# Fastaxx/Penguin.jl

Hardware: AMD Instinct MI355X
Metric: time-steps/sec + SpMV GB/s (% HBM roofline), 3D mono diffusion 512^3 (higher is better)
Workload: dtype f64

## Files before the change

include/penguin_hip.h:

```cpp
#ifndef PENGUIN_HIP_H
#define PENGUIN_HIP_H

#include <stddef.h>
#include <stdint.h>

#ifdef __cplusplus
extern "C" {
#endif

typedef struct pg_mesh pg_mesh;
typedef struct pg_capacity pg_capacity;
typedef struct pg_diffops pg_diffops;
typedef struct pg_solver pg_solver;
typedef struct pg_streamvort pg_streamvort;

enum { PG_BODY_BALL = 1, PG_BODY_MULTIBALL = 2, PG_BODY_HALFSPACE = 3, PG_BODY_ELLIPSOID = 4, PG_BODY_PLANE = 5 };
enum { PG_FLAG_COMPLEMENT = 1, PG_FLAG_NO_CENTROIDS = 2 };
enum { PG_CAP_V = 0, PG_CAP_GAMMA = 1, PG_CAP_CELL_TYPES = 2, PG_CAP_A = 3, PG_CAP_B = 4,
       PG_CAP_W = 5, PG_CAP_C_OMEGA = 6, PG_CAP_C_GAMMA = 7,
       PG_CAP_ST_V0 = 8, PG_CAP_ST_V1 = 9, PG_CAP_ST_CT_OMEGA = 10, PG_CAP_ST_CT_GAMMA = 11 };
enum { PG_OP_G = 0, PG_OP_H = 1, PG_OP_WINV = 2,
       PG_OP_C0 = 3 , PG_OP_K0 = 6  };
enum { PG_BC_NONE = 0, PG_BC_DIRICHLET = 1, PG_BC_NEUMANN = 2, PG_BC_ROBIN = 3, PG_BC_PERIODIC = 4 };
enum { PG_KEY_LEFT = 0 , PG_KEY_RIGHT = 1 , PG_KEY_BOTTOM = 2 ,
// ... 38 lines not shown
enum { PG_PRECOND_MG_CELL = -3 };
enum { PG_PRECOND_POLY_EST = -4 };
#define PG_SPECEST_MARGIN 0.0205

typedef struct {
  int32_t steps;
  int32_t admitted;
  int32_t gershgorin_admits;
  int32_t reserved;
  double g_ritz;
  double g_used;
  double margin;
  double gershgorin;
  double ritz_re_min, ritz_re_max, ritz_im_max;
  double estimate_ms;
} pg_specest_info;

#define PG_MG_MAX_LEVELS 16
typedef struct {
  int32_t levels;
  int32_t tail_level;
  int64_t rows[PG_MG_MAX_LEVELS];
  int64_t nnz[PG_MG_MAX_LEVELS];
  double setup_ms;
  int64_t bytes;
} pg_mg_info;

typedef struct {
  int32_t iters;
  int32_t converged;
  double resnorm;
  double bnorm;
  double extremum;
  double time;
} pg_step_info;

typedef struct {
  int64_t steps;
  int64_t total_iters;
  double t_final;
  double extremum;
  double solve_ms;
  double spmv_ms_total;
  int64_t spmv_launches;
  int64_t unconverged_steps;
  double worst_relres;
  double spmv_lean_ms_total;
  int64_t spmv_lean_launches;
  int64_t poly_degree;
  int64_t half_exits;
  int64_t poly_xspace;
  int64_t products;
  int64_t guess_states_read;
} pg_run_info;

typedef struct {
  int64_t n_own;
  int64_t nnz;
  int64_t n_ghost;
  int64_t n_omega;
  int64_t n_gamma;
  int64_t M_global;
  int64_t spmv_bytes;
  int64_t spmv_slices;
  int64_t rows_uniform;
  int64_t rows_pattern;
  int64_t rows_irregular;
  int64_t neumann_ok;
  double gershgorin;
  int64_t spmv_units;
  int64_t rows_marched;
  int64_t rows_matrix;
  int64_t n_ghost_loop;
  int64_t loop_is_compact;
  int64_t rows_edge;
} pg_system_info;

typedef struct {
  int64_t steps;
  int64_t psi_iters;
  int64_t omega_iters;
  int64_t psi_products;
  int64_t omega_products;
  int64_t unconverged;
  double worst_relres;
  double t_final;
  double total_ms;
  double psi_ms;
  double velocity_ms;
  double build_ms;
  double omega_ms;
} pg_streamvort_run_info;

int32_t pg_last_error(char* buf, size_t n);
int32_t pg_init(int32_t device_id);
int32_t pg_get_unique_id(void* out128);
int32_t pg_init_distributed(int32_t device_id, int32_t rank, int32_t nranks, const void* unique_id128);
int32_t pg_finalize(void);
int32_t pg_device_synchronize(void);
int32_t pg_set_profiling(int32_t on);
int32_t pg_device_name(char* buf, size_t n);
int32_t pg_config_string(char* buf, size_t n);

int32_t pg_mesh_create(int32_t N, const int64_t* n, const double* L, const double* x0, pg_mesh** out);
int32_t pg_mesh_destroy(pg_mesh* m);
int32_t pg_mesh_get_centers(const pg_mesh* m, int32_t d, double* out, int64_t len);
// ... 76 lines not shown

int32_t pg_streamvort_create(pg_capacity* c, pg_diffops* o, const double* nu, double dt, const pg_bc_desc* bc_stream,
                             const pg_bc_desc* bc_vorticity, const pg_border_desc* borders_stream, int32_t nborders_stream,
                             const pg_border_desc* borders_vorticity, int32_t nborders_vorticity, const double* psi0,
                             const double* omega0, pg_streamvort** out);
int32_t pg_streamvort_destroy(pg_streamvort* sv);
int32_t pg_streamvort_set_omega(pg_streamvort* sv, const double* omega);
int32_t pg_streamvort_set_source(pg_streamvort* sv, const double* f_n , const double* f_np1 );
int32_t pg_streamvort_set_interface_values(pg_streamvort* sv, int32_t which, const double* g_n , const double* g_np1 );
int32_t pg_streamvort_set_border_values(pg_streamvort* sv, int32_t which, const double* values );
int32_t pg_streamvort_solve_stream(pg_streamvort* sv, const pg_krylov_opts* opts, pg_step_info* info);
int32_t pg_streamvort_step(pg_streamvort* sv, int32_t scheme, const pg_krylov_opts* opts, pg_step_info* info_psi,
                           pg_step_info* info_omega);
int32_t pg_streamvort_run(pg_streamvort* sv, int64_t steps, int32_t scheme, const pg_krylov_opts* opts, int32_t save_every,
                          pg_streamvort_run_info* info);
int32_t pg_streamvort_get(const pg_streamvort* sv, int32_t field, int64_t state_index, double* out, int64_t len);
int32_t pg_streamvort_num_states(const pg_streamvort* sv, int64_t* out);
int32_t pg_streamvort_time(const pg_streamvort* sv, int64_t state_index, double* out);
int32_t pg_streamvort_solver(pg_streamvort* sv, int32_t which, pg_solver** borrowed);

int32_t pg_solver_set_source(pg_solver* s, int32_t phase, const double* f_n , const double* f_np1 );
int32_t pg_solver_set_interface_value(pg_solver* s, const double* g_n , const double* g_np1 );
int32_t pg_solver_set_border_values(pg_solver* s, const double* values );

int32_t pg_solver_initial_solve(pg_solver* s, const pg_krylov_opts* opts, pg_step_info* info);
int32_t pg_solver_step(pg_solver* s, int32_t scheme, const pg_krylov_opts* opts, pg_step_info* info);
int32_t pg_solver_run(pg_solver* s, double Tend, int32_t scheme, const pg_krylov_opts* opts, int32_t do_initial,
                      int64_t max_steps, int32_t save_every, pg_run_info* info);
int32_t pg_solver_num_states(const pg_solver* s, int64_t* out);
int32_t pg_solver_get_state(const pg_solver* s, int64_t state_index, double* x, int64_t len);
int32_t pg_solver_system_info(const pg_solver* s, int32_t which, pg_system_info* out);
int32_t pg_solver_get_system_csr(const pg_solver* s, int32_t which, int64_t* rowptr, int64_t* col, double* val,
                                 double* b, int64_t* idx);
int32_t pg_solver_get_row_scaling(const pg_solver* s, int32_t which, double* ds);
int32_t pg_solver_mg_info(const pg_solver* s, pg_mg_info* out);
int32_t pg_solver_mg_info_for(const pg_solver* s, int32_t precond, pg_mg_info* out);
int32_t pg_solver_spectral_estimate(pg_solver* s, int32_t which, pg_specest_info* out);
int32_t pg_solver_time_spmv(pg_solver* s, int32_t which, int32_t reps, double* avg_ms);

int32_t pg_partition_planes(const int64_t* weight, int64_t nplanes, int32_t nranks, int64_t* bounds);
int32_t pg_slab_numbering_host(int32_t K, int64_t plane, int64_t nplanes, int64_t p0, int64_t p1, const uint8_t* active,
                               int64_t* out);

int32_t pg_debug_spmv_compare(pg_solver* s, int32_t which, int32_t variant_a, int32_t variant_b, double* max_abs_diff,
                              double* max_abs);
int32_t pg_debug_spmv_mode_compare(pg_solver* s, int32_t which, int32_t mode, double* max_abs_diff, double* max_abs,
                                   double* max_dot_rel);
int32_t pg_debug_spmv_sizes(pg_solver* s, int32_t which, int64_t* n, int64_t* n_vec, int64_t* nnz, int32_t* grid);
#define PG_DEBUG_SPMV_SENTINEL 0x7FF8C0DE5EED0BADull
int32_t pg_debug_spmv_apply(pg_solver* s, int32_t which, int32_t variant, int32_t mode, const double* x, const double* aux,
                            const double* dotx, const double* base, double pc0, double pc1, double pc2, int32_t fold,
                            int32_t done, int32_t repeat, double* y, double* partials, double* slot_sums, double* folded,
                            int64_t* ticket);
int32_t pg_debug_read_probe(int64_t bytes, int32_t elem_bytes, int32_t nt, int32_t blocks, int32_t reps, double* gbs);
int32_t pg_debug_run_virtual_ranks(int32_t nranks, int32_t N, const int64_t* n, const double* L, int32_t body_kind,
                                   const double* params, int32_t nparams, double interface_value, double border_value,
                                   int32_t nkeys, const int32_t* keys, double dt, int32_t scheme_ctor, int32_t scheme_run,
                                   int64_t steps, double* x_out, int64_t* n_own_out, int64_t* nnz_out,
                                   int64_t* n_ghost_out, int64_t* iters_out);
int32_t pg_debug_set_virtual_rank_method(int32_t method, int32_t restart);
int32_t pg_debug_set_virtual_rank_precond(int32_t precond);
int32_t pg_debug_set_virtual_rank_ramp(double ramp);
int32_t pg_debug_set_virtual_rank_kick(int64_t step, double factor);
int32_t pg_debug_virtual_rank_info(int32_t rank, int64_t* full_rows, int64_t* loop_rows, int64_t* loop_bytes,
                                   int64_t* loop_ghosts);
int32_t pg_debug_scale_diagonal_rows(pg_solver* s, double factor);
int32_t pg_debug_set_poly_give_up(int32_t iterations);

int32_t pg_debug_mg_aggregates(pg_solver* s, int32_t level, int64_t* n, int32_t* agg);
int32_t pg_debug_mg_level_csr(pg_solver* s, int32_t level, int64_t* n, int64_t* nnz, int64_t* rowptr, int64_t* col, double* val);
int32_t pg_debug_mg_apply(pg_solver* s, const double* r, double* z);
int32_t pg_debug_mg_aggregates_for(pg_solver* s, int32_t precond, int32_t level, int64_t* n, int32_t* agg);
int32_t pg_debug_mg_level_csr_for(pg_solver* s, int32_t precond, int32_t level, int64_t* n, int64_t* nnz, int64_t* rowptr, int64_t* col,
                                  double* val);
int32_t pg_debug_mg_apply_for(pg_solver* s, int32_t precond, const double* r, double* z);

int32_t pg_debug_specest_hessenberg(pg_solver* s, int32_t which, int32_t* steps, double* H);

int32_t pg_solver_guess_info(pg_solver* s, int32_t* kept, int32_t* nstates, int32_t* offsets , double* coef ,
                             double* rr_plain, double* rr_taken);

#ifdef __cplusplus
}
#endif
#endif
```

penguin/jl_amd/_lib.py:

```python
from __future__ import annotations

import ctypes as C
import os
import re
from pathlib import Path

import numpy as np

_HERE = Path(__file__).resolve().parent
LIB_PATH = Path(os.environ["PG_LIB_PATH"]) if os.environ.get("PG_LIB_PATH") else _HERE / "lib" / "libpenguin_hip.so"
HEADER_PATH = _HERE.parent.parent / "include" / "penguin_hip.h"


class PenguinHipError(RuntimeError):
    pass


PG_BODY_BALL, PG_BODY_MULTIBALL, PG_BODY_HALFSPACE, PG_BODY_ELLIPSOID, PG_BODY_PLANE = 1, 2, 3, 4, 5
PG_FLAG_COMPLEMENT, PG_FLAG_NO_CENTROIDS = 1, 2
PG_CAP_V, PG_CAP_GAMMA, PG_CAP_CELL_TYPES, PG_CAP_A, PG_CAP_B, PG_CAP_W, PG_CAP_C_OMEGA, PG_CAP_C_GAMMA = range(8)
PG_CAP_ST_V0, PG_CAP_ST_V1, PG_CAP_ST_CT_OMEGA, PG_CAP_ST_CT_GAMMA = 8, 9, 10, 11
PG_OP_G, PG_OP_H, PG_OP_WINV = 0, 1, 2
PG_OP_C0, PG_OP_K0 = 3, 6
PG_BC_NONE, PG_BC_DIRICHLET, PG_BC_NEUMANN, PG_BC_ROBIN, PG_BC_PERIODIC = 0, 1, 2, 3, 4
PG_KEY = {"left": 0, "right": 1, "bottom": 2, "top": 3, "backward": 4, "forward": 5}
PG_SCHEME = {"BE": 0, "CN": 1, "STEADY": 2}
PG_METHOD = {"bicgstab": 0, "cg": 1, "gmres": 2, "bicgstabl": 3}
PG_SV_PSI, PG_SV_OMEGA, PG_SV_U, PG_SV_V = 0, 1, 2, 3
PG_PRECOND_MG = -2
PG_PRECOND_MG_CELL = -3
PG_PRECOND_POLY_EST = -4
PG_SPECEST_MARGIN = 0.0205
PG_MG_MAX_LEVELS = 16

c_double_p = C.POINTER(C.c_double)
c_i64_p = C.POINTER(C.c_int64)
c_i32_p = C.POINTER(C.c_int32)


class pg_bc_desc(C.Structure):
    _fields_ = [("kind", C.c_int32), ("alpha", C.c_double), ("beta", C.c_double), ("value", C.c_double),
                ("value_array", c_double_p)]


class pg_border_desc(C.Structure):
    _fields_ = [("key", C.c_int32), ("kind", C.c_int32), ("value", C.c_double)]


class pg_jump_desc(C.Structure):
    _fields_ = [("alpha1", C.c_double), ("alpha2", C.c_double), ("g", C.c_double), ("beta1", C.c_double),
                ("beta2", C.c_double), ("h", C.c_double), ("g_array", c_double_p), ("h_array", c_double_p)]


class pg_motion_desc(C.Structure):
    _fields_ = [("body_kind", C.c_int32), ("flags", C.c_int32), ("axis", C.c_int32), ("nq", C.c_int32), ("sign", C.c_double),
                ("t0", C.c_double), ("t1", C.c_double), ("nodes", c_double_p), ("body0", C.c_double * 4),
                ("body1", C.c_double * 4)]


class pg_krylov_opts(C.Structure):
    _fields_ = [("method", C.c_int32), ("reltol", C.c_double), ("abstol", C.c_double), ("maxiter", C.c_int32),
                ("check_every", C.c_int32), ("warm_start", C.c_int32), ("restart", C.c_int32), ("precond", C.c_int32)]


class pg_step_info(C.Structure):
    _fields_ = [("iters", C.c_int32), ("converged", C.c_int32), ("resnorm", C.c_double), ("bnorm", C.c_double),
                ("extremum", C.c_double), ("time", C.c_double)]


class pg_run_info(C.Structure):
    _fields_ = [("steps", C.c_int64), ("total_iters", C.c_int64), ("t_final", C.c_double), ("extremum", C.c_double),
                ("solve_ms", C.c_double), ("spmv_ms_total", C.c_double), ("spmv_launches", C.c_int64),
                ("unconverged_steps", C.c_int64), ("worst_relres", C.c_double), ("spmv_lean_ms_total", C.c_double),
                ("spmv_lean_launches", C.c_int64), ("poly_degree", C.c_int64), ("half_exits", C.c_int64),
                ("poly_xspace", C.c_int64), ("products", C.c_int64), ("guess_states_read", C.c_int64)]


class pg_system_info(C.Structure):
    _fields_ = [("n_own", C.c_int64), ("nnz", C.c_int64), ("n_ghost", C.c_int64), ("n_omega", C.c_int64),
                ("n_gamma", C.c_int64), ("M_global", C.c_int64), ("spmv_bytes", C.c_int64), ("spmv_slices", C.c_int64),
                ("rows_uniform", C.c_int64), ("rows_pattern", C.c_int64), ("rows_irregular", C.c_int64),
                ("neumann_ok", C.c_int64), ("gershgorin", C.c_double), ("spmv_units", C.c_int64),
                ("rows_marched", C.c_int64), ("rows_matrix", C.c_int64), ("n_ghost_loop", C.c_int64),
                ("loop_is_compact", C.c_int64), ("rows_edge", C.c_int64)]


class pg_streamvort_run_info(C.Structure):
    _fields_ = [("steps", C.c_int64), ("psi_iters", C.c_int64), ("omega_iters", C.c_int64), ("psi_products", C.c_int64),
                ("omega_products", C.c_int64), ("unconverged", C.c_int64), ("worst_relres", C.c_double), ("t_final", C.c_double),
                ("total_ms", C.c_double), ("psi_ms", C.c_double), ("velocity_ms", C.c_double), ("build_ms", C.c_double),
                ("omega_ms", C.c_double)]


class pg_mg_info(C.Structure):
    _fields_ = [("levels", C.c_int32), ("tail_level", C.c_int32), ("rows", C.c_int64 * PG_MG_MAX_LEVELS),
                ("nnz", C.c_int64 * PG_MG_MAX_LEVELS), ("setup_ms", C.c_double), ("bytes", C.c_int64)]


class pg_specest_info(C.Structure):
    _fields_ = [("steps", C.c_int32), ("admitted", C.c_int32), ("gershgorin_admits", C.c_int32), ("reserved", C.c_int32),
                ("g_ritz", C.c_double), ("g_used", C.c_double), ("margin", C.c_double), ("gershgorin", C.c_double),
                ("ritz_re_min", C.c_double), ("ritz_re_max", C.c_double), ("ritz_im_max", C.c_double), ("estimate_ms", C.c_double)]


def declared_symbols() -> list[str]:
    txt = HEADER_PATH.read_text()
    return sorted(set(re.findall(r"\bint32_t\s+(pg_[a-z0-9_]+)\s*\(", txt)))


_lib = None
hip_runtime_source = "system"


def _share_the_hip_runtime_with_torch() -> None:
    global hip_runtime_source
    import sys

    if "torch" in sys.modules:
        hip_runtime_source = "already mapped by torch"
        return
    if os.environ.get("PG_HIP_RUNTIME", "auto") == "system":
        return
    import importlib.util

    try:
        spec = importlib.util.find_spec("torch")
    except (ImportError, ValueError):
        spec = None
# ... 123 lines not shown
    return {k: getattr(info, k) for k, _ in pg_specest_info._fields_ if k != "reserved"}


def debug_specest_hessenberg(handle, which: int = 0, run: bool = True) -> np.ndarray:
    w = C.c_int32(which | (0 if run else 4))
    k = C.c_int32(0)
    check(lib().pg_debug_specest_hessenberg(handle, w, C.byref(k), None))
    H = np.zeros((k.value + 1) * max(k.value, 1))
    check(lib().pg_debug_specest_hessenberg(handle, w, C.byref(k), dptr(H)))
    return H[: (k.value + 1) * k.value].reshape((k.value + 1, k.value), order="F")


DEBUG_SPMV_SENTINEL = 0x7FF8C0DE5EED0BAD
DEBUG_SPMV_GUARD = 64


def debug_spmv_sizes(handle, which: int) -> tuple[int, int, int, int]:
    n, nv, nnz, grid = C.c_int64(0), C.c_int64(0), C.c_int64(0), C.c_int32(0)
    check(lib().pg_debug_spmv_sizes(handle, C.c_int32(which), C.byref(n), C.byref(nv), C.byref(nnz), C.byref(grid)))
    return n.value, nv.value, nnz.value, grid.value


def loop_system_csr(handle, which: int):
    n, _, nnz, _ = debug_spmv_sizes(handle, which)
    rowptr, col, val = np.zeros(n + 1, dtype=np.int64), np.zeros(max(nnz, 1), dtype=np.int64), np.zeros(max(nnz, 1))
    check(lib().pg_solver_get_system_csr(handle, C.c_int32(which), iptr(rowptr), iptr(col), dptr(val), None, None))
    return rowptr, col[:nnz], val[:nnz]


def debug_spmv_apply(handle, which: int, variant: int, mode: int, x, aux=None, dotx=None, base=None, pc=(0.0, 0.0, 0.0),
                     fold: int = 0, done: int = 0, repeat: int = 1) -> dict:
    n, nv, _, grid = debug_spmv_sizes(handle, which)

    def arr(a, length, name):
        if a is None:
            return None, None
        a = np.ascontiguousarray(a, dtype=np.float64)
        if a.size != length:
            raise ValueError(f"debug_spmv_apply: {name} has {a.size} entries, the matrix needs {length}")
        return a, dptr(a)

    xs, xp = arr(x, nv, "x")
    auxs, auxp = arr(aux, n, "aux")
    dots, dotp = arr(dotx, n, "dotx")
    bases, basep = arr(base, n, "base")
    y = np.zeros(n + DEBUG_SPMV_GUARD)
    partials = np.zeros((5, grid))
    sums, folded = np.zeros(5), np.zeros(5)
    ticket = C.c_int64(-1)
    check(lib().pg_debug_spmv_apply(handle, C.c_int32(which), C.c_int32(variant), C.c_int32(mode), xp, auxp, dotp, basep,
                                    C.c_double(pc[0]), C.c_double(pc[1]), C.c_double(pc[2]), C.c_int32(fold), C.c_int32(done),
                                    C.c_int32(repeat), dptr(y), dptr(partials), dptr(sums), dptr(folded), C.byref(ticket)))
    return {"y": y, "partials": partials, "slot_sums": sums, "folded": folded, "ticket": ticket.value, "grid": grid, "n": n}
```

penguin/jl_amd/csrc/pg_common.h:

```cpp
#pragma once
#include <hip/hip_runtime.h>
#include "pg_rccl.h"

#include <chrono>
#include <cstdint>
#include <cstdio>
#include <cstring>
#include <stdexcept>
#include <string>
#include <vector>

#include "../../../include/penguin_hip.h"

namespace pg {

using i64 = int64_t;
using i32 = int32_t;

struct Error : std::runtime_error {
  using std::runtime_error::runtime_error;
};

void set_last_error(const std::string& msg);

#define PG_HIP(expr)                                                                              \
  do {                                                                                            \
    hipError_t _e = (expr);                                                                       \
    if (_e != hipSuccess)                                                                         \
      throw pg::Error(std::string("HIP error: ") + hipGetErrorString(_e) + " at " + __FILE__ + ":" + \
                      std::to_string(__LINE__) + " (" #expr ")");                                 \
  } while (0)

#define PG_NCCL(expr)                                                                             \
  do {                                                                                            \
    ncclResult_t _e = (expr);                                                                     \
    if (_e != ncclSuccess)                                                                        \
      throw pg::Error(std::string("RCCL error: ") + pg::rccl::api().GetErrorString(_e) + " at " + __FILE__ + ":" + \
                      std::to_string(__LINE__) + " (" #expr ")");                                 \
  } while (0)

#define PG_REQUIRE(cond, msg)                                   \
  do {                                                          \
    if (!(cond)) throw pg::Error(std::string(msg));             \
  } while (0)

#define PG_API_BEGIN try {
#define PG_API_END                                  \
  return 0;                                         \
  }                                                 \
  catch (const std::exception& e) {                 \
    pg::set_last_error(e.what());                   \
    return 1;                                       \
  }                                                 \
  catch (...) {                                     \
    pg::set_last_error("unknown exception");        \
    return 2;                                       \
  }

struct Config {
  bool debug = false;
  int alloc_poison = 0;
  int async_alloc = 0;
  int alloc_guard = 0;
  long long pool_limit_mb = 0;
  bool poly = true;
  int poly_degree = 6;
  bool poly_adapt = true;
  double poly_margin = 1.0;
  double poly_slack = -1.0;
  int poly_hist = 3;
  bool poly_trend = true;
  int poly_maxdeg = 0;
  int poly_mindeg = 4;
  int profile_sample = 3;
  bool gamma_elim = true;
  bool diag_elim = true;
  double diag_elim_frac = 0.0005;
  int spmv_variant = 70;
  int spmv_xcd = 1;
  int spmv_strip = 16;
  int spmv_march_k = 0;
  int spmv_minrun = 24;
  bool spmv_march = true;
  bool spmv_edges = true;
  int spmv_tile_units = 0;
  int spmv_blocks_per_cu = 0;
  bool halo_overlap = true;
  int guess_n = 4;
  int guess_depth = 7;
  bool guess_defer = true;
  bool guess_always = false;
  int guess_monitor = 256;
  double guess_pass_cost = 0.34;
  double guess_gain = 0.8;
  bool speculate_product = true;
  int mg_tail_rows = 2048;
  int unit_order = 0;
};
const Config& config();

struct LocalComm;

struct Context {
  bool inited = false;
  LocalComm* local = nullptr;
  int device = 0;
  hipStream_t stream = nullptr;
  hipStream_t comm_stream = nullptr;
  hipEvent_t ev_fork = nullptr, ev_join = nullptr;
  int rank = 0, nranks = 1;
  ncclComm_t comm = nullptr;
  ncclComm_t comm_halo = nullptr;
  bool profiling = false;
  std::string device_name;
};
Context& ctx();
void require_init();
void set_thread_context(Context* c);
Context* thread_context();
LocalComm* local_comm_create(int nranks);
void local_comm_destroy(LocalComm* c);
void comm_allreduce_sum_f64(double* dev, int count, hipStream_t st);
void comm_allreduce_max_f64(double* dev, int count, hipStream_t st);
void comm_allreduce_sum_u64(unsigned long long* dev, i64 count, hipStream_t st);

void* dev_alloc(size_t bytes);
// ... 150 lines not shown
```

penguin/jl_amd/csrc/pg_context.hip:

```cpp
#include "pg_common.h"

#include <cxxabi.h>
#include <execinfo.h>

#include <atomic>
#include <map>
#include <mutex>
#include <unordered_map>
#include <unordered_set>
#include "pg_host_algos.h"

#include <algorithm>
#include <array>
#include <memory>
#include <set>

namespace pg {

static thread_local std::string g_last_error;
void set_last_error(const std::string& msg) { g_last_error = msg; }

Context& ctx() {
  static Context c;
  Context* t = thread_context();
  return t ? *t : c;
}

const Config& config() {
  static const Config c = [] {
    Config k;
    auto geti = [](const char* name, long long dflt) { const char* v = getenv(name); return v ? atoll(v) : dflt; };
    auto getd = [](const char* name, double dflt) { const char* v = getenv(name); return v ? atof(v) : dflt; };
    k.debug = getenv("PG_DEBUG") != nullptr;
    k.alloc_poison = (int)geti("PG_ALLOC_POISON", 0);
    k.async_alloc = (int)geti("PG_ASYNC_ALLOC", 0);
    k.alloc_guard = (int)geti("PG_ALLOC_GUARD", 0);
    k.pool_limit_mb = geti("PG_POOL_LIMIT_MB", 0);
    k.poly = geti("PG_POLY", 1) != 0;
    k.poly_degree = (int)geti("PG_POLY_DEGREE", 6);
    k.poly_adapt = geti("PG_POLY_ADAPT", getenv("PG_POLY_DEGREE") ? 0 : 1) != 0;
    k.poly_margin = getd("PG_POLY_MARGIN", 1.0);
    k.poly_slack = getd("PG_POLY_SLACK", -1.0);
    k.poly_hist = (int)std::max<long long>(1, std::min<long long>(3, geti("PG_POLY_HIST", 3)));
    k.poly_maxdeg = (int)geti("PG_POLY_MAXDEG", 0);
    k.poly_mindeg = (int)std::max<long long>(2, std::min<long long>(8, geti("PG_POLY_MINDEG", 4)));
    k.poly_trend = geti("PG_POLY_TREND", 1) != 0;
    k.profile_sample = (int)std::max<long long>(1, geti("PG_PROFILE_SAMPLE", 3));
    k.gamma_elim = geti("PG_GAMMA_ELIM", 1) != 0;
    k.diag_elim = geti("PG_DIAG_ELIM", 1) != 0;
    k.diag_elim_frac = getd("PG_DIAG_ELIM_FRAC", 0.0005);
    k.spmv_variant = (int)geti("PG_SPMV_VARIANT", 70);
    k.spmv_xcd = (int)geti("PG_SPMV_XCD", 1);
    k.spmv_strip = (int)geti("PG_SPMV_STRIP", 16);
    k.spmv_march_k = (int)geti("PG_SPMV_MARCH_K", 0);
    k.spmv_minrun = (int)geti("PG_SPMV_MINRUN", 24);
    k.spmv_march = geti("PG_SPMV_MARCH", 1) != 0;
    k.spmv_edges = geti("PG_SPMV_EDGES", 1) != 0;
    k.spmv_tile_units = (int)geti("PG_SPMV_TILE_UNITS", 0);
    k.spmv_blocks_per_cu = (int)geti("PG_SPMV_BLOCKS_PER_CU", 0);
    k.halo_overlap = geti("PG_HALO_OVERLAP", 1) != 0;
    k.speculate_product = geti("PG_SPECULATE", 1) != 0;
    k.guess_n = (int)std::max<long long>(0, std::min<long long>(4, geti("PG_GUESS_STATES", 4)));
    k.guess_depth = (int)std::max<long long>(1, std::min<long long>(7, geti("PG_GUESS_DEPTH", 7)));
    k.mg_tail_rows = (int)std::max<long long>(0, geti("PG_MG_TAIL_ROWS", 2048));
    k.guess_monitor = (int)std::max<long long>(1, geti("PG_GUESS_MONITOR", 256));
    k.guess_pass_cost = getd("PG_GUESS_PASS_COST", 0.34);
    k.guess_always = geti("PG_GUESS_ALWAYS", 0) != 0;
    k.guess_defer = geti("PG_GUESS_DEFER", 1) != 0;
    k.guess_gain = getd("PG_GUESS_GAIN", 0.8);
    k.unit_order = (int)geti("PG_SPMV_UNIT_ORDER", 0);
    return k;
  }();
  return c;
}

void require_init() {
  if (!ctx().inited)
    throw Error("penguin_hip: not initialised (call pg_init / pg_init_distributed first)");
}

static void init_device(int device_id) {
  Context& c = ctx();
  int ndev = 0;
  hipError_t e = hipGetDeviceCount(&ndev);
  if (e != hipSuccess || ndev <= 0)
    throw Error("penguin_hip: no HIP device visible -- this library has no CPU fallback");
  PG_REQUIRE(device_id >= 0 && device_id < ndev, "penguin_hip: device id out of range");
  PG_HIP(hipSetDevice(device_id));
  hipDeviceProp_t prop;
  PG_HIP(hipGetDeviceProperties(&prop, device_id));
  c.device = device_id;
  c.device_name = std::string(prop.name) + " (" + prop.gcnArchName + ")";
  if (!c.stream) PG_HIP(hipStreamCreateWithFlags(&c.stream, hipStreamNonBlocking));
  if (!c.comm_stream) PG_HIP(hipStreamCreateWithFlags(&c.comm_stream, hipStreamNonBlocking));
  c.inited = true;
}

}

// ... 215 lines not shown
      split_ok = R.CommSplit(c.comm, 0, rank, &c.comm_halo, nullptr) == ncclSuccess && c.comm_halo != nullptr;
      if (!split_ok) c.comm_halo = nullptr;
    }
    if (!split_ok) {
      ncclUniqueId id2;
      if (rank == 0) PG_NCCL(R.GetUniqueId(&id2));
      DevBuf<char> buf((i64)sizeof(id2));
      if (rank == 0) buf.upload(reinterpret_cast<const char*>(&id2), (i64)sizeof(id2));
      PG_NCCL(R.Broadcast(buf.p, buf.p, sizeof(id2), ncclChar, 0, c.comm, c.stream));
      buf.download(reinterpret_cast<char*>(&id2), (i64)sizeof(id2));
      PG_NCCL(R.CommInitRank(&c.comm_halo, nranks, id2, rank));
    }
  }
  PG_API_END
}

int32_t pg_finalize(void) {
  PG_API_BEGIN
  Context& c = ctx();
  if (c.inited) {
    (void)hipDeviceSynchronize();
    if (c.comm_halo) { (void)rccl::api().CommDestroy(c.comm_halo); c.comm_halo = nullptr; }
    if (c.comm) { (void)rccl::api().CommDestroy(c.comm); c.comm = nullptr; }
    dev_cache_release();
    if (c.stream) { (void)hipStreamDestroy(c.stream); c.stream = nullptr; }
    if (c.comm_stream) { (void)hipStreamDestroy(c.comm_stream); c.comm_stream = nullptr; }
    if (c.ev_fork) { (void)hipEventDestroy(c.ev_fork); c.ev_fork = nullptr; }
    if (c.ev_join) { (void)hipEventDestroy(c.ev_join); c.ev_join = nullptr; }
    c.inited = false;
  }
  PG_API_END
}

int32_t pg_device_synchronize(void) {
  PG_API_BEGIN
  require_init();
  PG_HIP(hipDeviceSynchronize());
  PG_API_END
}

int32_t pg_set_profiling(int32_t on) {
  PG_API_BEGIN
  ctx().profiling = on != 0;
  PG_API_END
}

int32_t pg_config_string(char* buf, size_t n) {
  PG_API_BEGIN
  const Config& k = config();
  char tmp[1024];
  snprintf(tmp, sizeof(tmp),
           "spmv_variant=%d spmv_xcd=%d spmv_strip=%d spmv_unit_order=%d spmv_march=%d spmv_edges=%d spmv_march_k=%d spmv_minrun=%d spmv_tile_units=%d "
           "spmv_blocks_per_cu=%d halo_overlap=%d speculate=%d poly=%d poly_degree=%d poly_adapt=%d "
           "poly_margin=%g poly_slack=%g poly_hist=%d poly_trend=%d poly_maxdeg=%d gamma_elim=%d diag_elim=%d "
           "guess_states=%d guess_depth=%d guess_defer=%d async_alloc=%d cache_limit_mb=%lld alloc_poison=%d alloc_guard=%d profile_sample=%d debug=%d",
           k.spmv_variant, k.spmv_xcd, k.spmv_strip, k.unit_order, (int)k.spmv_march, (int)k.spmv_edges, k.spmv_march_k, k.spmv_minrun, k.spmv_tile_units,
           k.spmv_blocks_per_cu, (int)k.halo_overlap, (int)k.speculate_product, (int)k.poly, k.poly_degree, (int)k.poly_adapt,
           k.poly_margin, k.poly_slack, k.poly_hist, (int)k.poly_trend, k.poly_maxdeg,
           (int)k.gamma_elim, (int)k.diag_elim, k.guess_n, k.guess_depth, (int)k.guess_defer, k.async_alloc, k.pool_limit_mb, k.alloc_poison, k.alloc_guard, k.profile_sample, (int)k.debug);
  if (buf && n > 0) {
    std::strncpy(buf, tmp, n - 1);
    buf[n - 1] = 0;
  }
  PG_API_END
}

int32_t pg_device_name(char* buf, size_t n) {
  PG_API_BEGIN
  require_init();
  if (buf && n > 0) {
    std::strncpy(buf, ctx().device_name.c_str(), n - 1);
    buf[n - 1] = 0;
  }
  PG_API_END
}

int32_t pg_mesh_create(int32_t N, const int64_t* n, const double* L, const double* x0, pg_mesh** out) {
  PG_API_BEGIN
  PG_REQUIRE(N >= 1 && N <= 3, "pg_mesh_create: N must be 1, 2 or 3");
  PG_REQUIRE(out != nullptr, "pg_mesh_create: out is NULL");
  PG_REQUIRE(n != nullptr && L != nullptr, "pg_mesh_create: n / L is NULL");
  std::unique_ptr<pg_mesh> guard(new pg_mesh());
  pg_mesh* m = guard.get();
  m->N = N;
  for (int d = 0; d < N; ++d) {
    PG_REQUIRE(n[d] >= 1, "pg_mesh_create: n_d must be >= 1");
    m->n[d] = n[d];
    m->L[d] = L[d];
    m->x0[d] = x0 ? x0[d] : 0.0;
    const double h = L[d] / static_cast<double>(n[d]);
    m->centers[d].resize(n[d]);
    m->nodes[d].resize(n[d] + 1);
    for (i64 j = 0; j < n[d]; ++j) m->centers[d][j] = m->x0[d] + static_cast<double>(j) * h;
    for (i64 j = 0; j <= n[d]; ++j) m->nodes[d][j] = m->x0[d] + (static_cast<double>(j) + 0.5) * h;
  }
  if (ctx().inited) {
    for (int d = 0; d < N; ++d) {
      m->d_nodes[d].alloc(n[d] + 1);
      m->d_nodes[d].upload(m->nodes[d].data(), n[d] + 1);
    }
  }
  *out = guard.release();
  PG_API_END
}

int32_t pg_mesh_destroy(pg_mesh* m) {
  PG_API_BEGIN
  delete m;
  PG_API_END
}

// ... 133 lines not shown
```

penguin/jl_amd/csrc/pg_host_algos.h:

```cpp
#pragma once
#include <algorithm>
#include <cmath>
#include <cstdint>
#include <vector>

namespace pghost {

inline void partition_planes(const int64_t* weight, int64_t nplanes, int nranks, int64_t* bounds) {
  std::vector<double> cum(nplanes + 1, 0.0);
  for (int64_t k = 0; k < nplanes; ++k) cum[k + 1] = cum[k] + static_cast<double>(weight[k]) + 1.0;
  const double total = cum[nplanes];
  bounds[0] = 0;
  for (int r = 1; r < nranks; ++r) {
    const double target = total * r / nranks;
    int64_t k = std::lower_bound(cum.begin(), cum.end(), target) - cum.begin();
    if (k > 0 && (target - cum[k - 1]) < (cum[k] - target)) --k;
    const int64_t lo = bounds[r - 1] + 1;
    const int64_t hi = nplanes - (nranks - r);
    bounds[r] = std::min(std::max(k, lo), hi);
  }
  bounds[nranks] = nplanes;
}

constexpr int SLAB_MAX_KINDS = 4;
// ... 498 lines not shown

PGHOST_HD inline int bicgstabl_small_solve(const double* G, int l, double* gamma) {
  for (int i = 0; i <= BL_MAX_L; ++i) gamma[i] = 0.0;
  if (l < 1 || l > BL_MAX_L) return 0;
  double M[BL_MAX_L][BL_MAX_L], c[BL_MAX_L], d0[BL_MAX_L], y[BL_MAX_L];
  int perm[BL_MAX_L];
  for (int k = l; k >= 1; --k) {
    for (int i = 0; i < k; ++i) {
      for (int j = 0; j < k; ++j) M[i][j] = G[(i + 1) * BL_LD + (j + 1)];
      c[i] = G[(i + 1) * BL_LD];
      d0[i] = M[i][i];
      perm[i] = i;
    }
    bool ok = true;
    for (int s = 0; s < k && ok; ++s) {
      int p = s;
      for (int q = s + 1; q < k; ++q)
        if (M[q][q] > M[p][p]) p = q;
      if (p != s) {
        for (int j = 0; j < k; ++j) { const double t = M[s][j]; M[s][j] = M[p][j]; M[p][j] = t; }
        for (int i = 0; i < k; ++i) { const double t = M[i][s]; M[i][s] = M[i][p]; M[i][p] = t; }
        { const double t = c[s]; c[s] = c[p]; c[p] = t; }
        { const double t = d0[s]; d0[s] = d0[p]; d0[p] = t; }
        { const int t = perm[s]; perm[s] = perm[p]; perm[p] = t; }
      }
      const double piv = M[s][s];
      if (!(piv > BL_PIV_TOL * d0[s]) || !bl_finite(piv)) { ok = false; break; }
      const double root = sqrt(piv);
      M[s][s] = root;
      c[s] = c[s] / root;
      for (int q = s + 1; q < k; ++q) M[q][s] = M[q][s] / root;
      for (int q = s + 1; q < k; ++q) {
        for (int t = s + 1; t <= q; ++t) {
          M[q][t] -= M[q][s] * M[t][s];
          M[t][q] = M[q][t];
        }
        c[q] -= M[q][s] * c[s];
      }
    }
    if (!ok) continue;
    for (int s = k - 1; s >= 0; --s) {
      double v = c[s];
      for (int q = s + 1; q < k; ++q) v -= M[q][s] * y[q];
      y[s] = v / M[s][s];
      if (!bl_finite(y[s])) ok = false;
    }
    if (!ok) continue;
    for (int s = 0; s < k; ++s) gamma[1 + perm[s]] = y[s];
    return k;
  }
  return 0;
}

}
```

penguin/jl_amd/csrc/pg_krylov.h:

```cpp
#pragma once
#include <functional>

#include "pg_system.h"

namespace pg {

struct MgHierarchy;

struct XGuess {
  const double* zbase = nullptr;
  const double* zr[8] = {nullptr, nullptr, nullptr, nullptr, nullptr, nullptr, nullptr, nullptr};
  const double* coef = nullptr;
};

struct KrylovWork {
  i64 n = 0, nvec = 0;
  DevBuf<double> r, rhat, p, v, t;
  DevBuf<double> partials;
  DevBuf<double> sc;
  double* h_sc = nullptr;
  int grid = 1;
  DevBuf<unsigned> ticket;
  double last_rate2 = 0.0;
  int last_iters = 0;
  const void* adapt_matrix = nullptr;
  int adapt_m = 0, adapt_h = 0;
  const void* need_matrix = nullptr;
  double need_hist[3] = {0.0, 0.0, 0.0};
  const void* fail_matrix = nullptr;
  int fail_deg = 0, good_deg = 0;
  double fail_L = 0.0;
  int fail_wait = 0, fail_backoff = 1;
  const int* scatter = nullptr;
  MgHierarchy* mg = nullptr;
  XGuess xguess;
  bool p_in_rhat = false;
  bool start_folded = false;
  const int* moved_flag = nullptr;
  int moved_stamp = 0;
  DevBuf<double> ya, yb, wa, wb;
  DevBuf<double> gm_basis, gm, gm_partials;
  int gm_m = -1;
  DevBuf<double> bl_vecs, bl, bl_partials;
  int bl_l = -1;
  i64 bl_stride = 0;
  std::function<void()> after_first_batch;
  hipEvent_t ev_poll = nullptr;
  void init(i64 n_own, i64 n_vec);
  ~KrylovWork();
};

struct SolveStats {
  int iters = 0;
  int converged = 0;
  double resnorm = 0.0, bnorm = 0.0;
  double spmv_ms = 0.0, spmv_lean_ms = 0.0;
  i64 spmv_launches = 0, spmv_lean_launches = 0;
  int poly_degree = 0;
  int half_exit = 0;
  int poly_xspace = 0;
  i64 products = 0;
  int polls = 0;
};

void halo_exchange(const Numbering& nb, const Slab& slab, double* vec, hipStream_t st);
void halo_begin(const Numbering& nb, const Slab& slab, double* vec, hipStream_t st);
void halo_end(hipStream_t st);
void spmv(const CsrMatrix& A, const double* x, double* y, hipStream_t st);
void spmv_halo(const CsrMatrix& A, const Numbering& nb, const Slab& slab, double* x, double* y, hipStream_t st);
void krylov_solve(const CsrMatrix& A, const Numbering& nb, const Slab& slab, const double* b, double* x,
                  KrylovWork& w, const pg_krylov_opts& opts, SolveStats& stats, const double* x0 = nullptr,
                  const double* Ax0 = nullptr, bool preinit = false);

bool krylov_uses_polynomial(const CsrMatrix& A, const pg_krylov_opts& opts);

extern int g_poly_give_up;

void gmres_solve(const CsrMatrix& A, const Numbering& nb, const Slab& slab, const double* b, double* x, KrylovWork& w,
                 const pg_krylov_opts& opts, SolveStats& stats);

void bicgstabl_solve(const CsrMatrix& A, const Numbering& nb, const Slab& slab, const double* b, double* x, KrylovWork& w,
                     const pg_krylov_opts& opts, SolveStats& stats);
const char* krylov_method_refusal(int method);

}
```

penguin/jl_amd/csrc/pg_krylov.hip:

```cpp
#include "pg_krylov.h"
#include "pg_multigrid.h"
#include "pg_spmv.h"
#include "pg_specest.h"

using namespace pg;

namespace pg { extern double g_host_wait_us; }

namespace {


__global__ __launch_bounds__(BLOCK) void k_bicg_init(i64 n, i64 nvec, const double* __restrict__ b,
                                                     const double* x0, const double* __restrict__ Ax0,
                                                     double* x, double* __restrict__ r,
                                                     double* __restrict__ rhat, double* __restrict__ p,
                                                     double* __restrict__ v, double* __restrict__ partials,
                                                     const double* __restrict__ ds) {
  __shared__ double s_red[BLOCK / 64];
  double acc = 0.0, accb = 0.0, accw = 0.0;
  for (i64 i = blockIdx.x * (i64)BLOCK + threadIdx.x; i < nvec; i += (i64)gridDim.x * BLOCK) {
    if (i < n) {
      const double bi = b[i];
      const double ri = x0 ? bi - Ax0[i] : bi;
      const double d = ds ? ds[i] : 1.0;
      x[i] = x0 ? x0[i] : 0.0;
      r[i] = ri; rhat[i] = ri; p[i] = ri; v[i] = 0.0;
      acc += ri * ri;
      accb += (d * bi) * (d * bi);
      accw += (d * ri) * (d * ri);
    } else {
      x[i] = 0.0; p[i] = 0.0;
    }
  }
  const double t = block_sum(acc, s_red);
  if (threadIdx.x == 0) partials[blockIdx.x] = t;
  const double tb = block_sum(accb, s_red);
  if (threadIdx.x == 0) partials[gridDim.x + blockIdx.x] = tb;
  const double tw = block_sum(accw, s_red);
  if (threadIdx.x == 0) partials[2 * (size_t)gridDim.x + blockIdx.x] = tw;
}

__global__ __launch_bounds__(BLOCK) void k_bicg_s(i64 n, double* __restrict__ sc, const double* __restrict__ v,
                                                  const double* __restrict__ rhat, double* __restrict__ r,
                                                  double* __restrict__ partials, const double* __restrict__ ds,
                                                  unsigned* __restrict__ ticket, int r_in_rhat) {
  __shared__ double s_red[BLOCK / 64];
  if (sc[S_DONE] != 0.0) return;
  const double alpha = sc[S_ALPHA];
  const bool rrhat = r_in_rhat != 0 && sc[S_ITERS] == 0.0;
  double a0 = 0.0, a1 = 0.0, aw = 0.0;
  for (i64 i = blockIdx.x * (i64)BLOCK + threadIdx.x; i < n; i += (i64)gridDim.x * BLOCK) {
    const double rh = rhat[i];
// ... 254 lines not shown
  if (threadIdx.x == 0) derive(phase, sc);
}

__global__ void k_derive(int phase, double* sc, int check_done) {
  if (check_done && sc[S_DONE] != 0.0) return;
  derive(phase, sc);
}

__global__ __launch_bounds__(BLOCK) void k_start_sums_moved(int grid, const double* __restrict__ partials, double* __restrict__ sc,
                                                            const int* __restrict__ flag, int stamp) {
  __shared__ double s_red[BLOCK / 64];
  for (int s = 0; s < 3; ++s) {
    double a = 0.0;
    for (int i = threadIdx.x; i < grid; i += BLOCK) a += partials[(size_t)s * grid + i];
    const double t = block_sum(a, s_red);
    if (threadIdx.x == 0) sc[S_RED0 + s] = t;
  }
  if (threadIdx.x == 0) sc[S_RED0 + 3] = __hip_atomic_load(flag, __ATOMIC_RELAXED, __HIP_MEMORY_SCOPE_AGENT) == stamp ? 1.0 : 0.0;
}

__global__ void k_derive_start_moved(double* sc) {
  derive(PH_INIT, sc);
  sc[S_MOVED] = sc[S_RED0 + 3] != 0.0 ? 1.0 : 0.0;
}

void finalize_folded(int phase, int nslots, KrylovWork& w, hipStream_t st) {
  Context& cx = ctx();
  if (cx.nranks == 1 && !cx.comm) return;
  comm_allreduce_sum_f64(w.sc.p + S_RED0, nslots, st);
  hipLaunchKernelGGL(k_derive, dim3(1), dim3(1), 0, st, phase, w.sc.p, 1);
}

void finalize(int phase, int nslots, KrylovWork& w, hipStream_t st, bool check_done, int slot0 = 0) {
  Context& cx = ctx();
  if (cx.nranks == 1 && !cx.comm) {
    hipLaunchKernelGGL(k_finalize, dim3(1), dim3(BLOCK), 0, st, phase, slot0, nslots, w.grid, w.partials.p, w.sc.p, 1,
                       check_done ? 1 : 0);
  } else {
    hipLaunchKernelGGL(k_finalize, dim3(1), dim3(BLOCK), 0, st, phase, slot0, nslots, w.grid, w.partials.p, w.sc.p, 0,
                       check_done ? 1 : 0);
    comm_allreduce_sum_f64(w.sc.p + S_RED0 + slot0, nslots, st);
    hipLaunchKernelGGL(k_derive, dim3(1), dim3(1), 0, st, phase, w.sc.p, check_done ? 1 : 0);
  }
}

struct SpmvTimer {
  bool on;
  hipEvent_t e0 = nullptr, e1 = nullptr;
  std::vector<std::pair<hipEvent_t, hipEvent_t>> pairs;
  std::vector<int> iter_of;
  std::vector<char> lean_of;
  std::vector<char> second_of;
  std::vector<int> count_of;
  int cur = 0, cur_count = 1;
  bool cur_lean = false, cur_second = false;
  bool armed = false;
  explicit SpmvTimer(bool on_) : on(on_) {}
  static std::vector<hipEvent_t>& pool() {
    static thread_local std::vector<hipEvent_t> p;
    return p;
  }
  static hipEvent_t take() {
    auto& p = pool();
    if (!p.empty()) {
      hipEvent_t e = p.back();
      p.pop_back();
      return e;
    }
    hipEvent_t e;
    PG_HIP(hipEventCreate(&e));
    return e;
  }
  void begin(hipStream_t st, int iteration, bool lean = false, bool second = false, int count = 1) {
    cur = iteration;
    cur_lean = lean;
    cur_second = second;
    cur_count = count;
    const int sample = config().profile_sample;
    static thread_local unsigned long long counter = 0;
    armed = on && (counter++ % sample == 0);
    if (!armed) return;
    e0 = take();
    e1 = take();
    PG_HIP(hipEventRecord(e0, st));
  }
  void end(hipStream_t st) {
    if (!armed) return;
    PG_HIP(hipEventRecord(e1, st));
    pairs.emplace_back(e0, e1);
    iter_of.push_back(cur);
    lean_of.push_back(cur_lean ? 1 : 0);
    second_of.push_back(cur_second ? 1 : 0);
    count_of.push_back(cur_count);
  }
  void collect(SolveStats& s, int iters_done, bool half_exit) {
    for (size_t q = 0; q < pairs.size(); ++q) {
      auto& pr = pairs[q];
      float ms = 0.f;
      (void)hipEventSynchronize(pr.second);
      const bool ran = iter_of[q] < iters_done && !(half_exit && iter_of[q] == iters_done - 1 && second_of[q]);
      if (ran && hipEventElapsedTime(&ms, pr.first, pr.second) == hipSuccess) {
        if (lean_of[q]) { s.spmv_lean_ms += ms; s.spmv_lean_launches += count_of[q]; }
        else { s.spmv_ms += ms; s.spmv_launches += 1; }
      }
      pool().push_back(pr.first);
      pool().push_back(pr.second);
    }
    pairs.clear();
    iter_of.clear();
    lean_of.clear();
    second_of.clear();
    count_of.clear();
  }
};

}

namespace pg {

double g_host_wait_us = 0.0;
int g_poly_give_up = 0;

void KrylovWork::init(i64 n_own, i64 n_vec) {
  n = n_own;
  nvec = n_vec;
  const i64 a = n_vec > 0 ? n_vec : 1;
  r.alloc(a); rhat.alloc(a); p.alloc(a); v.alloc(a); t.alloc(a);
  grid = spmv_default_grid(n_own);
  partials.alloc(5 * (i64)grid);
  sc.alloc(S_COUNT);
  sc.zero();
  ticket.alloc(1);
  ticket.zero();
  if (!h_sc) PG_HIP(hipHostMalloc(reinterpret_cast<void**>(&h_sc), sizeof(double) * S_COUNT));
}

KrylovWork::~KrylovWork() {
  if (h_sc) (void)hipHostFree(h_sc);
  if (ev_poll) (void)hipEventDestroy(ev_poll);
}

void spmv_halo(const CsrMatrix& A, const Numbering& nb, const Slab& slab, double* x, double* y, hipStream_t st) {
  spmv_with_halo(0, A, nb, slab, x, y, nullptr, nullptr, nullptr, spmv_default_grid(A.n), st);
  PG_HIP(hipGetLastError());
}

void spmv(const CsrMatrix& A, const double* x, double* y, hipStream_t st) {
  if (A.n == 0) return;
  launch_spmv(0, A, x, y, nullptr, nullptr, nullptr, spmv_default_grid(A.n), st);
  PG_HIP(hipGetLastError());
}

const char* krylov_method_refusal(int method) {
  return method == PG_METHOD_CG ? "the method is CG (BiCGStab only)"
         : method == PG_METHOD_BICGSTABL ? "the method is BiCGStab(l) (BiCGStab only)" : "the method is GMRES (BiCGStab only)";
}

bool krylov_uses_polynomial(const CsrMatrix& A, const pg_krylov_opts& opts) {
  const bool poly_env = config().poly;
  const int degree_env = config().poly_degree;
  const int precond = opts.precond == PG_PRECOND_POLY_EST ? 0 : opts.precond;
  if (!(poly_env && precond >= 0 && opts.method == PG_METHOD_BICGSTAB && A.poly_ok && spmv_supports_preconditioner_product() && A.n > 0))
    return false;
  return (precond > 0 ? precond : degree_env) >= 2;
}

constexpr int MAX_POLY_DEGREE = 40;

namespace {

void choose_next_degree(const CsrMatrix& A, const SolveStats& stats, int m, bool adaptive, KrylovWork& w) {
  const Config& cfg = config();
  const bool keep_degree = adaptive && stats.converged && stats.iters == 0 && w.adapt_m >= 2;
  w.adapt_matrix = nullptr;
  if (keep_degree) { w.adapt_matrix = &A; w.adapt_m = cfg.poly_mindeg; w.adapt_h = 1; }
  if (!(adaptive && stats.converged && stats.iters > 0)) return;
  const double rr0 = w.h_sc[S_RR0], rr = w.h_sc[S_HALF] != 0.0 ? w.h_sc[S_RED4] : w.h_sc[S_RR], tol2 = w.h_sc[S_TOL2];
  const double P = (2.0 * stats.iters - stats.half_exit) * m;
  if (!(rr0 > tol2 && rr > 0.0 && rr < rr0 && tol2 > 0.0)) return;
  w.last_rate2 = std::log(rr0 / rr) / P;
  const double margin = cfg.poly_margin;
  const double slack_env = cfg.poly_slack;
  const double slack = slack_env >= 0.0 ? slack_env : 0.3;
  const double need_now = std::min(P, P * std::log(tol2 / rr0) / std::log(rr / rr0)) * margin + slack;
  const int hist_n = cfg.poly_hist;
  if (w.need_matrix != &A) { w.need_matrix = &A; w.need_hist[0] = w.need_hist[1] = w.need_hist[2] = 0.0; }
  w.need_hist[2] = w.need_hist[1]; w.need_hist[1] = w.need_hist[0]; w.need_hist[0] = need_now;
  double need = need_now;
  double trend = 0.0;
  if (cfg.poly_trend && hist_n >= 3 && w.need_hist[2] > 0.0) trend = std::max(-0.5, std::min(0.2, 0.5 * (need_now - w.need_hist[2])));
  for (int q = 1; q < hist_n; ++q)
    if (w.need_hist[q] > 0.0) need = std::max(need, std::min(w.need_hist[q] + q * trend, need_now + 0.6));
  need += trend;
  double best = 1e300;
  for (int h = 1; h <= 16; ++h) {
    const int mm = std::max(cfg.poly_mindeg, (int)std::ceil(need / h));
    const int maxdeg = cfg.poly_maxdeg > 0 ? std::min(MAX_POLY_DEGREE, std::max(4, cfg.poly_maxdeg)) : 32;
    if (mm > maxdeg) continue;
    const double cost = h * (1.0 + 1.18 * (mm - 2) + 3.6);
    if (cost < best) { best = cost; w.adapt_m = mm; w.adapt_h = h; }
  }
  if (best < 1e300) w.adapt_matrix = &A;
  if (stats.iters == 1) {
    const double Lnow = std::log(rr0 / tol2);
    if (w.fail_matrix != &A) { w.fail_matrix = &A; w.fail_deg = 0; w.good_deg = 0; w.fail_wait = 0; w.fail_backoff = 1; }
    if (w.fail_wait > 0) --w.fail_wait;
    if (stats.half_exit) w.good_deg = m;
    else {
      w.fail_backoff = (m == w.fail_deg) ? std::min(w.fail_backoff * 2, 64) : 1;
      w.fail_deg = m; w.fail_L = Lnow;
      w.fail_wait = 2 * w.fail_backoff * (m + 3);
    }
    if (best < 1e300 && w.adapt_h == 1) {
      if (!stats.half_exit && w.good_deg > m) w.adapt_m = std::max(m + 1, std::min(w.adapt_m, w.good_deg));
      const double per_product = std::max(1.0, w.last_rate2);
      if (w.fail_deg > 0 && w.fail_wait > 0 && w.adapt_m <= w.fail_deg &&
          Lnow > w.fail_L - per_product * (w.fail_deg - w.adapt_m + 1))
        w.adapt_m = w.fail_deg + 1;
    }
  }
  if (cfg.debug) fprintf(stderr, "[pg_krylov] degree %d used %g products, needed %.1f -> next: %d applications of degree %d\n", m, P, need, w.adapt_h, w.adapt_m);
}

}

void krylov_solve(const CsrMatrix& A, const Numbering& nb, const Slab& slab, const double* b, double* x, KrylovWork& w,
                  const pg_krylov_opts& opts, SolveStats& stats, const double* x0, const double* Ax0, bool preinit) {
  Context& cx = ctx();
  hipStream_t st = cx.stream;
  const i64 n = A.n, nvec = nb.n_vec();
  PG_REQUIRE(w.n >= n && w.nvec >= nvec, "krylov workspace too small");
  PG_REQUIRE(opts.method == PG_METHOD_BICGSTAB || opts.method == PG_METHOD_CG || opts.method == PG_METHOD_GMRES ||
                 opts.method == PG_METHOD_BICGSTABL,
             "unknown Krylov method");
  const bool est_opt = opts.precond == PG_PRECOND_POLY_EST;
  if (est_opt) {
    PG_REQUIRE(opts.method == PG_METHOD_BICGSTAB,
               std::string("estimated polynomial preconditioner (precond = PG_PRECOND_POLY_EST) refused: ") +
                   krylov_method_refusal(opts.method));
    specest_require_one_rank();
    PG_REQUIRE(A.poly_ok || A.est.tried || A.poly_gave_up, "estimated polynomial preconditioner (precond = PG_PRECOND_POLY_EST): no spectral estimate "
               "has run on this matrix (specest_run before krylov_solve)");
  }
  const int precond = est_opt ? 0 : opts.precond;
  if (opts.method == PG_METHOD_GMRES) {
    PG_REQUIRE(!preinit && !x0, "GMRES starts from zero (IterativeSolvers' default)");
    gmres_solve(A, nb, slab, b, x, w, opts, stats);
    return;
  }
  if (opts.method == PG_METHOD_BICGSTABL) {
    PG_REQUIRE(!preinit && !x0, "BiCGStab(l) starts from zero (IterativeSolvers' default)");
    PG_REQUIRE(!mg_is_precond(opts.precond), std::string("multigrid preconditioner (precond = ") + mg_precond_name(mg_rule_of(opts.precond)) +
// ... 21 lines not shown
  w.xguess = XGuess();
  const bool start_folded = w.start_folded && preinit && opts.method == PG_METHOD_BICGSTAB;
  w.start_folded = false;
  const int* moved_flag = w.moved_flag;
  const int moved_stamp = w.moved_stamp;
  w.moved_flag = nullptr;
  const bool fused_start = !start_folded && preinit && opts.method == PG_METHOD_BICGSTAB && cx.nranks == 1 && !cx.comm;
  if (!fused_start && !start_folded)
    hipLaunchKernelGGL(k_sc_reset, dim3(1), dim3(S_COUNT), 0, st, w.sc.p, opts.reltol * opts.reltol, opts.abstol * opts.abstol);
  SpmvTimer timer(cx.profiling);

  const bool cg = opts.method == PG_METHOD_CG;
  const Config& cfg = config();
  const bool poly_env = cfg.poly;
  const int degree_env = cfg.poly_degree;
  int m = 0;
  const bool by_estimate = est_opt && !A.poly_ok && !A.poly_gave_up && A.est.tried && A.est.admitted;
  if (poly_env && precond >= 0 && !cg && (A.poly_ok || by_estimate) && spmv_supports_preconditioner_product() && n > 0)
    m = std::min(precond > 0 ? precond : degree_env, MAX_POLY_DEGREE);
  const bool adapt_env = cfg.poly_adapt;
  const bool adaptive = adapt_env && m >= 2 && precond == 0 && preinit;
  int expect_halves = 0;
  if (adaptive && w.adapt_matrix == &A && w.adapt_m >= 2) { m = w.adapt_m; expect_halves = w.adapt_h; }
  if (m < 2) m = 0;
  const bool poly = m > 0;
  MgHierarchy* const mgh = w.mg;
  w.mg = nullptr;
  const bool mg = mg_is_precond(opts.precond);
  if (mg) {
    PG_REQUIRE(!cg, "multigrid preconditioner refused: the method must be BiCGStab");
    PG_REQUIRE(spmv_supports_preconditioner_product(), "multigrid preconditioner refused: the x-space loop needs the slice kernel (PG_SPMV_VARIANT)");
    mg_require_one_rank(mg_rule_of(opts.precond));
    PG_REQUIRE(mgh && !w.scatter && !xg.zbase && n > 0, "multigrid preconditioner refused: this solve has no hierarchy (steady monophasic "
               "diffusion systems and the stream-function solve only)");
    PG_REQUIRE(mgh->rule == mg_rule_of(opts.precond),
               std::string("multigrid preconditioner: the hierarchy handed over was not built for precond = ") +
                   mg_precond_name(mg_rule_of(opts.precond)));
  }
  const bool pre = poly || mg;
  stats.poly_degree = m;
  stats.poly_xspace = poly ? 1 : 0;
  PG_REQUIRE(!w.scatter || (poly && preinit), "a compact system needs the polynomial path and a prepared start");
  double tau[MAX_POLY_DEGREE];
  if (poly) {
    const double g = std::min(std::max(by_estimate ? A.est.g_used : A.gersh, 0.05), 0.95);
    double lam[MAX_POLY_DEGREE];
    for (int k = 0; k < m; ++k) lam[k] = 1.0 + g * std::cos(M_PI * (2.0 * k + 1.0) / (2.0 * m));
    for (int k = 0, lo = 0, hi = m - 1; k < m; ++k) tau[k] = 1.0 / ((k & 1) ? lam[hi--] : lam[lo++]);
  }
  if (pre && w.ya.n < nvec) {
    w.ya.alloc(nvec); w.wa.alloc(nvec); w.wb.alloc(nvec); w.yb.alloc(nvec);
    w.ya.zero(); w.wa.zero(); w.wb.zero(); w.yb.zero();
  }
  const bool half_test = m >= 3 || mg;
  PG_REQUIRE(!xg.zbase || (poly && p_in_rhat && w.scatter), "an unformed extrapolated state needs the polynomial loop on a compact system");
  PG_REQUIRE(!preinit || !cg, "preinit is a BiCGStab path");
  if (!cg) {
    if (!preinit)
      hipLaunchKernelGGL(k_bicg_init, dim3(G), dim3(BLOCK), 0, st, n, nvec, b, x0, Ax0, x, w.r.p, w.rhat.p, w.p.p, w.v.p,
                       w.partials.p, (const double*)A.ds.p);
    static_assert(S_COUNT <= BLOCK, "k_start resets the scalar block with one thread per scalar");
    if (start_folded) {
    } else if (fused_start)
      hipLaunchKernelGGL(k_start, dim3(1), dim3(BLOCK), 0, st, (int)PH_INIT, 3, w.grid, (const double*)w.partials.p, w.sc.p,
                         opts.reltol * opts.reltol, opts.abstol * opts.abstol);
    else if (moved_flag && preinit && !(cx.nranks == 1 && !cx.comm)) {
      hipLaunchKernelGGL(k_start_sums_moved, dim3(1), dim3(BLOCK), 0, st, w.grid, (const double*)w.partials.p, w.sc.p, moved_flag,
                         moved_stamp);
      comm_allreduce_sum_f64(w.sc.p + S_RED0, 4, st);
      hipLaunchKernelGGL(k_derive_start_moved, dim3(1), dim3(1), 0, st, w.sc.p);
    } else
      finalize(PH_INIT, 3, w, st, false);
  } else {
    hipLaunchKernelGGL(k_cg_init, dim3(G), dim3(BLOCK), 0, st, n, nvec, b, x, w.r.p, w.p.p, w.partials.p, (const double*)A.ds.p);
    finalize(PH_CG_INIT, 2, w, st, false);
  }
  PG_HIP(hipGetLastError());

  int launched = 0, polls = 0;
  bool mid = false;
  bool done = false, poly_failed = false;
  const int poly_give_up = g_poly_give_up > 0 ? g_poly_give_up : 40 + 400 / std::max(m, 1);
  const int derive_here = (cx.nranks == 1 && !cx.comm) ? 1 : 0;
  auto apply = [&](double* in, double* out, int phase, int nslots, int itn) {
    const bool second = phase == PH_BICG_2;
    double* src = in;
    if (poly) {
      double* hat = second ? w.yb.p : w.ya.p;
      timer.begin(st, itn, true, second, m - 1);
      for (int k = m - 2; k >= 0; --k) {
        double* dst = k == 0 ? hat : ((k & 1) ? w.wb.p : w.wa.p);
        FinArgs f{nullptr, nullptr, PH_NONE, 0, 0, nullptr};
        const double lead = k == m - 2 ? tau[m - 1] : 1.0;
        f.pc0 = lead; f.pc1 = -lead * tau[k]; f.pc2 = tau[k]; f.base = in;
        spmv_with_halo(8, A, nb, slab, src, dst, nullptr, nullptr, w.sc.p, G, st, &f);
        src = dst;
      }
      timer.end(st);
    } else if (mg) {
      double* hat = second ? w.yb.p : w.ya.p;
      timer.begin(st, itn, true, second, 1);
      mg_apply(*mgh, A, nb, slab, in, hat, w.sc.p, st);
      timer.end(st);
      src = hat;
    }
    FinArgs f{w.ticket.p, w.sc.p, phase, nslots, derive_here, pre ? in : nullptr};
    timer.begin(st, itn, false, second);
    const bool folded = spmv_with_halo(phase == PH_BICG_1 ? 1 : 3, A, nb, slab, src, out, w.rhat.p, w.partials.p, w.sc.p, G, st, &f);
    timer.end(st);
    if (folded) finalize_folded(phase, nslots, w, st); else finalize(phase, nslots, w, st, true);
  };
  auto first_half = [&](int itn, bool test) {
    double* pvec = (p_in_rhat && itn == 0) ? w.rhat.p : w.p.p;
    apply(pvec, w.v.p, PH_BICG_1, 3, itn);
    unsigned* tk = (test && derive_here) ? w.ticket.p : nullptr;
    if (pre)
      hipLaunchKernelGGL(k_bicg_s_x, dim3(G), dim3(BLOCK), 0, st, n, w.sc.p, w.v.p, w.rhat.p, w.r.p, w.partials.p, (const double*)A.ds.p, tk,
                         p_in_rhat ? 1 : 0, (const double*)w.ya.p, x, w.scatter, xg, itn == 0 ? 1 : 0);
    else
      hipLaunchKernelGGL(k_bicg_s, dim3(G), dim3(BLOCK), 0, st, n, w.sc.p, w.v.p, w.rhat.p, w.r.p, w.partials.p, (const double*)A.ds.p, tk,
                         p_in_rhat ? 1 : 0);
    if (test && !tk) finalize(PH_BICG_S, 1, w, st, true, 4);
  };
  auto second_half = [&](int itn) {
    apply(w.r.p, w.t.p, PH_BICG_2, 5, itn);
    hipLaunchKernelGGL(k_bicg_xrp, dim3(G), dim3(BLOCK), 0, st, n, w.sc.p, w.t.p, w.v.p, x, w.r.p, w.p.p, w.rhat.p, w.partials.p,
                       (const double*)A.ds.p, p_in_rhat ? 1 : 0, pre ? (const double*)w.yb.p : nullptr, w.scatter);
  };
  while (!done) {
    int want = check_every;
    if (w.last_iters > 1) want = polls == 0 ? w.last_iters - 1 : (polls <= 4 ? 1 : check_every);
    if (expect_halves > 0) want = polls == 0 ? (expect_halves + 1) / 2 : (polls <= 4 ? 1 : check_every);
    const int batch = std::max(1, std::min(want, maxiter - launched));
    int halves = 2 * batch;
    if (half_test && expect_halves > 0 && polls == 0) halves = std::max(1, std::min(expect_halves, 2 * (maxiter - launched)));
    ++polls;
    if (!cg) {
      const bool predicted = half_test && expect_halves > 0 && polls == 1;
      for (int h = 0; h < halves; ++h) {
        if (!mid) {
          if (launched >= maxiter) break;
          first_half(launched, half_test && (!predicted || h + 2 >= halves));
          ++launched;
          mid = true;
        } else {
          second_half(launched - 1);
          mid = false;
        }
      }
    } else {
      for (int it = 0; it < batch; ++it) {
// ... 14 lines not shown
    struct WaitClock {
      std::chrono::steady_clock::time_point t0;
      ~WaitClock() { g_host_wait_us += std::chrono::duration<double, std::micro>(std::chrono::steady_clock::now() - t0).count(); }
    } wait_clock{t_wait0};
    if (w.after_first_batch && polls == 1) {
      if (!w.ev_poll) PG_HIP(hipEventCreateWithFlags(&w.ev_poll, hipEventDisableTiming));
      PG_HIP(hipEventRecord(w.ev_poll, st));
      std::function<void()> hook;
      hook.swap(w.after_first_batch);
      hook();
      PG_HIP(hipEventSynchronize(w.ev_poll));
    } else {
      PG_HIP(hipStreamSynchronize(st));
    }
    if (w.h_sc[S_DONE] != 0.0 || (launched >= maxiter && !mid)) done = true;
    if (!done && poly && launched >= poly_give_up) { poly_failed = true; done = true; }
  }
  if (poly_failed) {
    const_cast<CsrMatrix&>(A).poly_ok = false;
    const_cast<CsrMatrix&>(A).est.admitted = false;
    const_cast<CsrMatrix&>(A).poly_gave_up = true;
    timer.collect(stats, launched, false);
    if (w.scatter) {
      stats.iters = launched;
      stats.converged = 0;
      stats.poly_degree = -1;
      return;
    }
    if (cfg.debug) fprintf(stderr, "[pg_krylov] polynomial preconditioner (m = %d) stagnated after %d iterations: plain iteration\n", m, launched);
    spmv_with_halo(0, A, nb, slab, x, w.t.p, nullptr, nullptr, nullptr, G, st);
    SolveStats rest;
    krylov_solve(A, nb, slab, b, x, w, opts, rest, x, w.t.p, false);
    stats = rest;
    stats.iters += launched;
    return;
  }
  if (cfg.debug)
    fprintf(stderr, "[pg_krylov] done=%g iters=%g rr0=%g rr=%g tol2=%g rho=%g rho_old=%g alpha=%g omega=%g beta=%g red0=%g red1=%g\n",
            w.h_sc[S_DONE], w.h_sc[S_ITERS], w.h_sc[S_RR0], w.h_sc[S_RR], w.h_sc[S_TOL2], w.h_sc[S_RHO], w.h_sc[S_RHO_OLD], w.h_sc[S_ALPHA],
            w.h_sc[S_OMEGA], w.h_sc[S_BETA], w.h_sc[S_RED0], w.h_sc[S_RED1]);
  stats.iters = (int)w.h_sc[S_ITERS];
  stats.polls = polls;
  w.last_iters = stats.iters;
  stats.converged = w.h_sc[S_DONE] == 1.0 ? 1 : 0;
  stats.half_exit = w.h_sc[S_HALF] != 0.0 ? 1 : 0;
  stats.resnorm = std::sqrt(cg ? w.h_sc[S_RRW] : w.h_sc[S_RR]);
  stats.bnorm = std::sqrt(w.h_sc[S_BB]);
  timer.collect(stats, stats.iters, w.h_sc[S_HALF] != 0.0);
  stats.products = (i64)(2 * stats.iters - stats.half_exit) * (m >= 2 ? m : 1);
  if (!cg && stats.converged && stats.products > 0) {
    const double rr0 = w.h_sc[S_RR0], rr = w.h_sc[S_HALF] != 0.0 ? w.h_sc[S_RED4] : w.h_sc[S_RR];
    if (rr0 > 0.0 && rr > 0.0 && rr < rr0) w.last_rate2 = std::log(rr0 / rr) / (double)stats.products;
  }
  choose_next_degree(A, stats, m, adaptive, w);
}

}
```

penguin/jl_amd/csrc/pg_solver.hip:

```cpp
#include <algorithm>
#include <cmath>
#include <memory>

#include "pg_krylov.h"
#include "pg_reduce.h"
#include "pg_multigrid.h"
#include "pg_solver_internal.h"
#include "pg_spmv.h"
#include "pg_specest.h"

using namespace pg;

namespace pg { extern double g_host_wait_us; }

struct pg_solver {
  int nphase = 1;
  pg_capacity* cap[2] = {nullptr, nullptr};
  pg_diffops* ops[2] = {nullptr, nullptr};
  Slab slab;
  int K = 2;
  i64 Mloc = 0, M = 0;
  double dt = 0.0, t = 0.0;
  int scheme_ctor = PG_SCHEME_BE;
  pg_bc_desc bc_i{};
// ... 1809 lines not shown
                     dv.p, s->slab.first_cell(), s->Mloc, s->nphase, s->nb.red.p, s->nb.n_own, s->bcv.p);
  PG_HIP(hipGetLastError());
  PG_HIP(hipStreamSynchronize(ctx().stream));
  s->bconst_dirty = true;
  if (!s->initial_done) build_first_rhs(s);
  PG_API_END
}

int32_t pg_solver_initial_solve(pg_solver* s, const pg_krylov_opts* opts, pg_step_info* info) {
  PG_API_BEGIN
  require_init();
  PG_REQUIRE(s, "Solver is not initialized. Call a solver constructor first.");
  SolveStats st;
  std::unique_ptr<AsyncAllocScope> pool(s->moving ? new AsyncAllocScope() : nullptr);
  do_initial(s, opts, st);
  fill_info(s, st, info);
  PG_API_END
}

int32_t pg_solver_step(pg_solver* s, int32_t scheme, const pg_krylov_opts* opts, pg_step_info* info) {
  PG_API_BEGIN
  require_init();
  PG_REQUIRE(s, "Solver is not initialized. Call a solver constructor first.");
  PG_REQUIRE(scheme == PG_SCHEME_BE || scheme == PG_SCHEME_CN, "scheme must be BE or CN");
  SolveStats st;
  do_step(s, scheme, opts, st);
  fill_info(s, st, info);
  PG_API_END
}

int32_t pg_solver_run(pg_solver* s, double Tend, int32_t scheme, const pg_krylov_opts* opts, int32_t do_initial_flag,
                      int64_t max_steps, int32_t save_every, pg_run_info* info) {
  PG_API_BEGIN
  require_init();
  PG_REQUIRE(s, "Solver is not initialized. Call a solver constructor first.");
  PG_REQUIRE(scheme == PG_SCHEME_BE || scheme == PG_SCHEME_CN, "scheme must be BE or CN");
  hipStream_t stream = ctx().stream;
  EventPair ev;
  const auto t_run0 = std::chrono::steady_clock::now();
  const double wait0 = pg::g_host_wait_us;
  PG_HIP(hipEventRecord(ev.e0, stream));
  double used0 = 0.0;
  if (s->guess_coef.n >= 16) s->guess_coef.download(&used0, 1, 13);
  SolveStats tot;
  i64 steps = 0, iters = 0, unconverged = 0;
  double worst = 0.0;
  auto account = [&](const SolveStats& st) {
    iters += st.iters; tot.spmv_ms += st.spmv_ms; tot.spmv_launches += st.spmv_launches;
    tot.spmv_lean_ms += st.spmv_lean_ms; tot.spmv_lean_launches += st.spmv_lean_launches;
    tot.poly_degree = st.poly_degree;
    tot.poly_xspace = st.poly_xspace;
    tot.half_exit += st.half_exit;
    tot.products += st.products;
    if (!st.converged) ++unconverged;
    if (st.bnorm > 0.0) worst = std::max(worst, st.resnorm / st.bnorm);
  };
  if (do_initial_flag) {
    SolveStats st;
    do_initial(s, opts, st);
    account(st);
    if (save_every > 0) keep_state(s);
  }
  while (s->t < Tend) {
    if (max_steps >= 0 && steps >= max_steps) break;
    SolveStats st;
    s->hint_more_steps = (s->t + s->dt < Tend) && (max_steps < 0 || steps + 1 < max_steps);
    struct HintReset { pg_solver* s; ~HintReset() { s->hint_more_steps = false; } } hint_reset{s};
    do_step(s, scheme, opts, st);
    account(st);
    ++steps;
    if (save_every > 0 && steps % save_every == 0) keep_state(s);
  }
  PG_HIP(hipEventRecord(ev.e1, stream));
  PG_HIP(hipEventSynchronize(ev.e1));
  float ms = 0.f;
  PG_HIP(hipEventElapsedTime(&ms, ev.e0, ev.e1));
  if (config().debug && steps > 0) {
    const double wall_us = std::chrono::duration<double, std::micro>(std::chrono::steady_clock::now() - t_run0).count();
    fprintf(stderr, "[pg_solver_run] %lld steps: wall %.1f us per step, of which the host waited %.1f us for the device (the rest: queueing "
            "launches and bookkeeping); device time by events %.1f us per step\n", (long long)steps, wall_us / steps,
            (pg::g_host_wait_us - wait0) / steps, ms * 1e3 / steps);
  }
  if (info) {
    info->steps = steps;
    info->total_iters = iters;
    info->t_final = s->t;
    info->extremum = max_abs(s);
    info->solve_ms = ms;
    info->spmv_ms_total = tot.spmv_ms;
    info->spmv_launches = tot.spmv_launches;
    info->unconverged_steps = unconverged;
    info->worst_relres = worst;
    info->spmv_lean_ms_total = tot.spmv_lean_ms;
    info->spmv_lean_launches = tot.spmv_lean_launches;
    info->poly_degree = tot.poly_degree;
    info->poly_xspace = tot.poly_xspace;
    info->half_exits = tot.half_exit;
    info->products = tot.products;
    info->guess_states_read = 0;
    if (s->guess_coef.n >= 16) {
      double hc[16];
      s->guess_coef.download(hc, 16);
      info->guess_states_read = (int64_t)(hc[13] - used0);
    }
  }
  PG_API_END
}

int32_t pg_solver_num_states(const pg_solver* s, int64_t* out) {
  PG_API_BEGIN
  PG_REQUIRE(s && out, "pg_solver_num_states: NULL argument");
  *out = (int64_t)s->states.size();
  PG_API_END
}

int32_t pg_solver_get_state(const pg_solver* s, int64_t state_index, double* x, int64_t len) {
  PG_API_BEGIN
  require_init();
  PG_REQUIRE(s && x, "pg_solver_get_state: NULL argument");
  PG_REQUIRE(len == (i64)s->K * s->M, "pg_solver_get_state: len must be 2M (mono) or 4M (diph)");
  if (state_index < 0) materialize_x(const_cast<pg_solver*>(s));
  const double* src = s->x.p;
  if (state_index >= 0) {
    PG_REQUIRE(state_index < (i64)s->states.size(), "pg_solver_get_state: state index out of range");
    src = s->states[state_index].p;
  }
  hipStream_t st = ctx().stream;
  DevBuf<double> pad((i64)s->K * s->Mloc);
  pad.zero();
  if (s->nb.n_own > 0) {
    hipLaunchKernelGGL(k_scatter_active, dim3(grid_for(s->nb.n_own, BLOCK)), dim3(BLOCK), 0, st, make_segs(s->nb),
                       s->nb.n_own, s->Mloc, s->nb.row_cell.p, src, pad.p);
    PG_HIP(hipGetLastError());
  }
  const i64 own_lo = (s->slab.p0 - s->slab.s0) * s->slab.plane, own_n = (s->slab.p1 - s->slab.p0) * s->slab.plane;
  for (int k = 0; k < s->K; ++k)
    pad.download(x + (i64)k * s->M + s->slab.p0 * s->slab.plane, own_n, (i64)k * s->Mloc + own_lo);
  PG_API_END
}

int32_t pg_solver_system_info(const pg_solver* s, int32_t which, pg_system_info* out) {
  PG_API_BEGIN
  PG_REQUIRE(s && out, "pg_solver_system_info: NULL argument");
  const CsrMatrix& Af = ((which & 1) == 0 || !s->have_run) ? s->A_ctor : run_matrix(s);
  const GammaElim& E = (&Af == &s->A_ctor) ? s->elim_ctor : s->elim_run;
  const DiagElim& DE = (&Af == &s->A_ctor) ? s->diag_ctor : s->diag_run;
  const CsrMatrix& A = ((which & 4) && DE.active) ? DE.A : (((which & 4) && E.active) ? E.A : Af);
  out->n_own = s->nb.n_own;
  out->nnz = (which & 6) ? A.nnz : A.nnz_raw;
  out->n_ghost = s->nb.n_ghost;
  i64 nw = 0, ng = 0;
// ... 376 lines not shown
  PG_REQUIRE(n > 0, "pg_debug_spmv_apply: the matrix has no rows");
  PG_REQUIRE(!slices || A.srec.p, "pg_debug_spmv_apply: the matrix has no slice image");
  nv = std::max(nv, n);
  hipStream_t st = ctx().stream;
  const int grid = spmv_default_grid(n);
  constexpr i64 GUARD = 64;
  double sentinel;
  const unsigned long long sbits = PG_DEBUG_SPMV_SENTINEL;
  std::memcpy(&sentinel, &sbits, sizeof(double));
  DevBuf<double> dx(nv), daux(nv), ddot(nv), dbase(nv), dy(n + GUARD), dpart(5 * (i64)grid), dsc(S_COUNT);
  DevBuf<unsigned> dticket(1);
  daux.zero(); ddot.zero(); dbase.zero(); dsc.zero(); dticket.zero();
  dx.upload(x, nv);
  if (aux) daux.upload(aux, n);
  if (dotx) ddot.upload(dotx, n);
  if (base) dbase.upload(base, n);
  {
    std::vector<double> fill((size_t)std::max<i64>(n + GUARD, 5 * (i64)grid), sentinel);
    dy.upload(fill.data(), n + GUARD);
    if (fold && mode == 3) std::fill(fill.begin() + 2 * (size_t)grid, fill.begin() + 4 * (size_t)grid, 0.0);
    dpart.upload(fill.data(), 5 * (i64)grid);
    std::vector<double> hsc(S_COUNT, 0.0);
    for (int k = 0; k < 5; ++k) hsc[S_RED0 + k] = sentinel;
    hsc[S_DONE] = (double)done;
    dsc.upload(hsc.data(), S_COUNT);
  }
  FinArgs f{fold ? dticket.p : nullptr, fold ? dsc.p : nullptr, PH_NONE, fold ? (mode == 1 ? 1 : (mode == 2 ? 2 : 5)) : 0, 0,
            dotx ? ddot.p : nullptr};
  if (mode == 8) { f.pc0 = pc0; f.pc1 = pc1; f.pc2 = pc2; f.base = base ? dbase.p : dx.p; }
  const bool with_fin = mode == 8 || fold || dotx;
  for (int r = 0; r < repeat; ++r) {
    const bool folded_here = launch_spmv_as(variant, mode, A, dx.p, dy.p, aux ? daux.p : nullptr, mode >= 1 && mode <= 3 ? dpart.p : nullptr,
                                            dsc.p, grid, st, with_fin ? &f : nullptr);
    PG_REQUIRE(folded_here == (fold != 0), "pg_debug_spmv_apply: the launch did not report the scalar phase as asked");
  }
  PG_HIP(hipGetLastError());
  dy.download(y, n + GUARD);
  std::vector<double> hp(5 * (size_t)grid), hsc(S_COUNT);
  dpart.download(hp.data(), 5 * (i64)grid);
  dsc.download(hsc.data(), S_COUNT);
  if (partials) std::memcpy(partials, hp.data(), sizeof(double) * hp.size());
  for (int k = 0; k < 5; ++k) {
    double a = 0.0;
    for (int i = 0; i < grid; ++i) a += hp[(size_t)k * grid + i];
    slot_sums[k] = a;
    folded[k] = hsc[S_RED0 + k];
  }
  unsigned ht = 0;
  dticket.download(&ht, 1);
  *ticket = (int64_t)ht;
  PG_API_END
}

__global__ void k_scale_rows(i64 n_e, const int* __restrict__ elist, double factor, double* __restrict__ z) {
  for (i64 q = blockIdx.x * (i64)blockDim.x + threadIdx.x; q < n_e; q += (i64)gridDim.x * blockDim.x) z[elist[q]] *= factor;
}

int32_t pg_debug_scale_diagonal_rows(pg_solver* s, double factor) {
  PG_API_BEGIN
  require_init();
  PG_REQUIRE(s && s->have_run, "pg_debug_scale_diagonal_rows: no run matrix yet");
  const CsrMatrix& A = run_matrix(s);
  DiagElim& DE = (&A == &s->A_ctor) ? s->diag_ctor : s->diag_run;
  PG_REQUIRE(DE.active && DE.n_e > 0, "pg_debug_scale_diagonal_rows: the loop of this solver is not the compact one");
  hipLaunchKernelGGL(k_scale_rows, dim3(grid_for(DE.n_e, BLOCK)), dim3(BLOCK), 0, ctx().stream, DE.n_e, (const int*)DE.elist.p, factor,
                     s->z.p);
  PG_HIP(hipGetLastError());
  PG_HIP(hipStreamSynchronize(ctx().stream));
  s->x_valid = false;
  s->spec_y_valid = false;
  PG_API_END
}

int32_t pg_solver_guess_info(pg_solver* s, int32_t* kept, int32_t* nstates, int32_t* offsets, double* coef, double* rr_plain,
                             double* rr_taken) {
  PG_API_BEGIN
  require_init();
  PG_REQUIRE(s && kept && nstates && offsets && coef && rr_plain && rr_taken, "pg_solver_guess_info: NULL argument");
  *kept = s->hist_cnt;
  *nstates = 0;
  *rr_plain = *rr_taken = 0.0;
  for (int j = 0; j < 4; ++j) { offsets[j] = 0; coef[j] = 0.0; }
  if (s->guess_coef.n >= 16 && s->hist_cnt > 0) {
    double hc[16];
    s->guess_coef.download(hc, 16);
    *nstates = (int32_t)hc[4];
    for (int j = 0; j < *nstates && j < 4; ++j) { offsets[j] = (int32_t)hc[5 + j] + 1; coef[j] = hc[j]; }
    *rr_plain = hc[9];
    *rr_taken = hc[10];
  }
  PG_API_END
}

int32_t pg_solver_time_spmv(pg_solver* s, int32_t which, int32_t reps, double* avg_ms) {
  PG_API_BEGIN
  require_init();
  PG_REQUIRE(s && avg_ms && reps > 0, "pg_solver_time_spmv: bad arguments");
  const int sel = which & 1, mode = (which & 2048) ? 8 : ((which >> 4) & 7);
  PG_REQUIRE(mode <= 3 || mode == 8, "pg_solver_time_spmv: unknown launch mode");
  if (sel == 1) PG_REQUIRE(s->have_run, "run matrix not assembled yet");
  const CsrMatrix& Afull = sel == 0 ? s->A_ctor : run_matrix(s);
  GammaElim& E = (&Afull == &s->A_ctor) ? s->elim_ctor : s->elim_run;
  if ((which & 512) && !E.tried) build_gamma_elim(Afull, s->nb, E);
  DiagElim& DE = (&Afull == &s->A_ctor) ? s->diag_ctor : s->diag_run;
  if ((which & 4096) && !DE.tried) build_diag_elim(Afull, s->nb, s->slab, DE);
  const CsrMatrix& A = ((which & 4096) && DE.active) ? DE.A : (((which & 512) && E.active) ? E.A : Afull);
// ... 165 lines not shown
```

penguin/jl_amd/csrc/pg_spmv.h:

```cpp
#pragma once
#include "pg_system.h"

namespace pg {

enum { S_RHO = 0, S_RHO_OLD, S_ALPHA, S_OMEGA, S_BETA, S_RR, S_BB, S_TOL2, S_DONE, S_ITERS, S_RELTOL2, S_ABSTOL2,
       S_RESTART, S_RHAT2, S_FORCE, S_PENDING3, S_RRW, S_HALF, S_RR0 ,
       S_MOVED ,
       S_RED0, S_RED1, S_RED2, S_RED3, S_RED4, S_COUNT };

constexpr int BLOCK = 256;

__device__ inline double wave_sum(double v) {
#pragma unroll
  for (int off = 32; off > 0; off >>= 1) v += __shfl_down(v, off, 64);
  return v;
}

__device__ inline double block_sum(double v, double* sh ) {
  v = wave_sum(v);
  const int lane = threadIdx.x & 63, wave = threadIdx.x >> 6;
  __syncthreads();
  if (lane == 0) sh[wave] = v;
  __syncthreads();
  double s = 0.0;
// ... 77 lines not shown
      break;
    case PH_CG_1:
      if (r0 == 0.0) sc[S_DONE] = 2.0; else sc[S_ALPHA] = sc[S_RR] / r0;
      break;
    case PH_CG_2: {
      const double rr_old = sc[S_RR];
      sc[S_RR] = r0;
      sc[S_RRW] = r1;
      sc[S_ITERS] += 1.0;
      if (r1 <= sc[S_TOL2]) sc[S_DONE] = 1.0;
      else sc[S_BETA] = r0 / rr_old;
      break;
    }
  }
}


__device__ inline void store_partial(double* p, double v) {
  __hip_atomic_store(reinterpret_cast<unsigned long long*>(p), (unsigned long long)__double_as_longlong(v), __ATOMIC_RELAXED,
                     __HIP_MEMORY_SCOPE_AGENT);
}
__device__ inline double load_partial(const double* p) {
  return __longlong_as_double((long long)__hip_atomic_load(reinterpret_cast<const unsigned long long*>(p), __ATOMIC_RELAXED,
                                                            __HIP_MEMORY_SCOPE_AGENT));
}

__device__ inline void put_partial(double* p, double v, int accum) { store_partial(p, accum ? v + load_partial(p) : v); }

__device__ inline bool last_block_arrives(unsigned* ticket, unsigned nblocks, double* sh ) {
  asm volatile("s_waitcnt vmcnt(0)" ::: "memory");
  __syncthreads();
  if (threadIdx.x == 0) {
    const unsigned t = __hip_atomic_fetch_add(ticket, 1u, __ATOMIC_RELAXED, __HIP_MEMORY_SCOPE_AGENT);
    const bool last = t == nblocks - 1;
    if (last) __hip_atomic_store(ticket, 0u, __ATOMIC_RELAXED, __HIP_MEMORY_SCOPE_AGENT);
    sh[0] = last ? 1.0 : 0.0;
  }
  __syncthreads();
  const bool last = sh[0] != 0.0;
  __syncthreads();
  return last;
}

struct FinArgs {
  unsigned* ticket;
  double* sc;
  int phase;
  int nslots;
  int do_derive;
  const double* dotx;
  double pc0 = 0.0, pc1 = 0.0;
  const double* base = nullptr;
  double pc2 = 0.0;
};

__device__ inline void fold_scalar_phase(const FinArgs& fin, const double* __restrict__ partials, double* s_red, int nparts) {
  if (!fin.ticket) return;
  if (!last_block_arrives(fin.ticket, gridDim.x, s_red)) return;
  for (int sl = 0; sl < fin.nslots; ++sl) {
    double a = 0.0;
    for (int i = threadIdx.x; i < nparts; i += BLOCK) a += load_partial(partials + (size_t)sl * nparts + i);
    const double t = block_sum(a, s_red);
    if (threadIdx.x == 0) fin.sc[S_RED0 + sl] = t;
  }
  if (threadIdx.x == 0 && fin.do_derive) derive(fin.phase, fin.sc);
}

bool launch_spmv(int mode, const CsrMatrix& A, const double* x, double* y, const double* aux, double* partials,
                 const double* sc, int grid, hipStream_t st, const FinArgs* fin = nullptr);
bool launch_spmv_as(int variant, int mode, const CsrMatrix& A, const double* x, double* y, const double* aux, double* partials,
                    const double* sc, int grid, hipStream_t st, const FinArgs* fin = nullptr);
bool spmv_with_halo(int mode, const CsrMatrix& A, const Numbering& nb, const Slab& slab, double* x, double* y, const double* aux,
                    double* partials, const double* sc, int grid, hipStream_t st, const FinArgs* fin = nullptr);
void launch_spmv_variant(int variant, const CsrMatrix& A, const double* x, double* y, hipStream_t st);
void spmv_mode_compare(const CsrMatrix& A, i64 nv, int mode, double* max_abs_diff, double* max_abs, double* max_dot_rel);
int spmv_default_grid(i64 n);
bool spmv_supports_preconditioner_product();

}
```

penguin/jl_amd/csrc/pg_spmv.hip:

```cpp
#include <algorithm>
#include <cstdlib>
#include <thread>
#include <vector>

#include "pg_host_algos.h"
#include "pg_krylov.h"
#include "pg_spmv.h"

namespace pg {
namespace {

constexpr int SPMV_ROWS = 256;
constexpr int SPMV_LDS_ENTRIES = 3584;

template <int MODE>
__global__ __launch_bounds__(BLOCK) void k_spmv(i64 n, const int* __restrict__ rowptr, const int* __restrict__ col,
                                                const double* __restrict__ val, const double* __restrict__ x,
                                                double* __restrict__ y, const double* __restrict__ aux,
                                                double* __restrict__ partials, const double* __restrict__ sc) {
  __shared__ double s_val[SPMV_LDS_ENTRIES];
  __shared__ int s_col[SPMV_LDS_ENTRIES];
  __shared__ double s_red[BLOCK / 64];
  if (sc && sc[S_DONE] != 0.0) return;
  double acc0 = 0.0, acc1 = 0.0, acc2 = 0.0;
  const i64 nchunks = (n + SPMV_ROWS - 1) / SPMV_ROWS;
  for (i64 chunk = blockIdx.x; chunk < nchunks; chunk += gridDim.x) {
    const i64 r0 = chunk * SPMV_ROWS;
    const i64 r1 = r0 + SPMV_ROWS < n ? r0 + SPMV_ROWS : n;
    const int base = rowptr[r0];
    const int cnt = rowptr[r1] - base;
    const i64 r = r0 + threadIdx.x;
    int a = 0, b = 0;
    if (r < r1) {
      a = rowptr[r] - base;
      b = rowptr[r + 1] - base;
    }
    double sum = 0.0;
    if (cnt <= SPMV_LDS_ENTRIES) {
      for (int k = threadIdx.x; k < cnt; k += BLOCK) {
        s_val[k] = val[base + k];
        s_col[k] = col[base + k];
      }
      __syncthreads();
      for (int k = a; k < b; ++k) sum += s_val[k] * x[s_col[k]];
      __syncthreads();
    } else {
      for (int k = a; k < b; ++k) sum += val[base + k] * x[col[base + k]];
    }
    if (r < r1) {
      y[r] = sum;
      if (MODE == 1) acc0 += aux[r] * sum;
      if (MODE >= 2) {
        acc0 += sum * x[r];
        acc1 += sum * sum;
      }
// ... 115 lines not shown
    const Desc dnext2 = load_desc(chunk_desc, c2 < nchunks ? c2 : lastc);
    double sum = 0.0;
#pragma unroll
    for (int j = 0; j < WUNR; ++j) sum += vv[j] * xv[j];
    if (__builtin_expect(len > WUNR, 0))
      for (int k = WUNR; k < len; ++k) sum += sv[av + k] * x[scl[ac + k]];
    __builtin_amdgcn_wave_barrier();
    if (live) {
      y[r] = sum;
      if (MODE == 1) acc0 += aux[r] * sum;
      if (MODE >= 2) {
        acc0 += sum * x[r];
        acc1 += sum * sum;
      }
      if (MODE == 3) acc2 += aux[r] * sum;
    }
    dcur = dnext;
    dnext = dnext2;
  }
  if (MODE >= 1) {
    const double t0 = block_sum(acc0, s_red);
    if (threadIdx.x == 0) partials[blockIdx.x] = t0;
  }
  if (MODE >= 2) {
    const double t1 = block_sum(acc1, s_red);
    if (threadIdx.x == 0) partials[gridDim.x + blockIdx.x] = t1;
  }
  if (MODE == 3) {
    const double t2 = block_sum(acc2, s_red);
    if (threadIdx.x == 0) partials[4 * (size_t)gridDim.x + blockIdx.x] = t2;
  }
}

enum { SL_U = 0, SL_P = 1, SL_G = 2 };
constexpr int SL_MAXROWS_U = 254, SL_MAXROWS_P = 128, SL_MAXCNT = 8, SL_REC = 32;

struct SDesc {
  int r0, meta, base, aux;
};

__device__ inline int rlane(int v, int l) { return __builtin_amdgcn_readlane(v, l); }

typedef double d2u_t __attribute__((ext_vector_type(2), aligned(8)));

template <bool NT>
__device__ inline d2_t load_pair(const double* p) {
  const d2u_t* q = reinterpret_cast<const d2u_t*>(p);
  d2u_t v = NT ? __builtin_nontemporal_load(q) : *q;
  d2_t r;
  r.x = v.x; r.y = v.y;
  return r;
}

template <int MODE>
struct ModeInfo {
  static constexpr bool OWN = MODE == 8;
  static constexpr bool HAS_A = MODE == 1 || MODE == 2 || MODE == 3;
  static constexpr bool HAS_B = MODE == 3 || MODE == 8;
  static constexpr bool DOT0 = MODE == 1 || MODE == 2 || MODE == 3;
  static constexpr bool DOT1 = MODE == 2 || MODE == 3;
  static constexpr bool DOT2 = MODE == 3;
};

template <int MODE>
__device__ __forceinline__ double mode_out(double s, double own, double b, double pc0, double pc1, double pc2) {
  if (MODE == 8) return __builtin_fma(pc2, b, __builtin_fma(pc0, own, pc1 * s));
  return s;
}

template <int CNT, int NB, bool PSL, int MODE, bool NT>
__device__ __forceinline__ void slice_rows(const SDesc& d, int nrows, int rec, const double* __restrict__ pval,
                                  const double* __restrict__ x, double* __restrict__ y, const double* __restrict__ pa,
                                  const double* __restrict__ pb, int lane, double& acc0, double& acc1, double& acc2, int dbg,
                                  double pc0, double pc1, double pc2) {
  using MI = ModeInfo<MODE>;
  int o[CNT];
#pragma unroll
  for (int j = 0; j < CNT; ++j) o[j] = (dbg & 4) ? 0 : rlane(rec, 4 + j);
  int l0[NB];
  bool live0[NB], live1[NB];
  d2_t xv[NB][CNT];
#pragma unroll
  for (int b = 0; b < NB; ++b) {
    const int l = 128 * b + 2 * lane;
    live0[b] = l < nrows;
    live1[b] = l + 1 < nrows;
    l0[b] = live0[b] ? l : 0;
#pragma unroll
    for (int j = 0; j < CNT; ++j) xv[b][j] = load_pair<false>(x + d.r0 + l0[b] + o[j]);
  }
  d2_t sum[NB];
#pragma unroll
  for (int b = 0; b < NB; ++b) { sum[b].x = 0.0; sum[b].y = 0.0; }
  if (!PSL) {
#pragma unroll
    for (int j = 0; j < CNT; ++j) {
      const double c = __hiloint2double(rlane(rec, 13 + 2 * j), rlane(rec, 12 + 2 * j));
#pragma unroll
      for (int b = 0; b < NB; ++b) {
        sum[b].x += c * xv[b][j].x;
        sum[b].y += c * xv[b][j].y;
      }
    }
  } else {
#pragma unroll
    for (int b = 0; b < NB; ++b) {
      const double* __restrict__ pv = pval + d.base + l0[b];
      d2_t vv[CNT];
#pragma unroll
      for (int j = 0; j < CNT; ++j) vv[j] = load_pair<NT>(pv + j * nrows);
#pragma unroll
      for (int j = 0; j < CNT; ++j) {
        sum[b].x += vv[j].x * xv[b][j].x;
        sum[b].y += vv[j].y * xv[b][j].y;
      }
    }
  }
  d2_t own[NB], ax[NB], ax2[NB];
#pragma unroll
  for (int b = 0; b < NB; ++b) {
    own[b].x = own[b].y = ax[b].x = ax[b].y = ax2[b].x = ax2[b].y = 0.0;
    if (MI::OWN) own[b] = load_pair<false>(x + d.r0 + l0[b]);
    if (MI::HAS_A) ax[b] = load_pair<false>(pa + d.r0 + l0[b]);
    if (MI::HAS_B) ax2[b] = load_pair<false>(pb + d.r0 + l0[b]);
  }
#pragma unroll
  for (int b = 0; b < NB; ++b) {
    sum[b].x = mode_out<MODE>(sum[b].x, own[b].x, ax2[b].x, pc0, pc1, pc2);
    sum[b].y = mode_out<MODE>(sum[b].y, own[b].y, ax2[b].y, pc0, pc1, pc2);
    const bool st = !(dbg & 8) || sum[b].x == 1.2345e-300;
    double* yp = y + d.r0 + l0[b];
    if (live1[b]) {
      if (st) {
        d2u_t out;
        out.x = sum[b].x; out.y = sum[b].y;
        if (!(dbg & 2048)) __builtin_nontemporal_store(out, reinterpret_cast<d2u_t*>(yp));
        else *reinterpret_cast<d2u_t*>(yp) = out;
      }
      if (MI::DOT0) acc0 += ax[b].x * sum[b].x + ax[b].y * sum[b].y;
      if (MI::DOT1) acc1 += sum[b].x * sum[b].x + sum[b].y * sum[b].y;
      if (MI::DOT2) acc2 += ax2[b].x * sum[b].x + ax2[b].y * sum[b].y;
    } else if (live0[b]) {
      if (st) *yp = sum[b].x;
      if (MI::DOT0) acc0 += ax[b].x * sum[b].x;
      if (MI::DOT1) acc1 += sum[b].x * sum[b].x;
      if (MI::DOT2) acc2 += ax2[b].x * sum[b].x;
    }
  }
}

template <int CNT, bool PSL, int MODE, bool NT>
__device__ __forceinline__ void slice_nb(const SDesc& d, int nrows, int rec, const double* __restrict__ pval,
                                const double* __restrict__ x, double* __restrict__ y, const double* __restrict__ pa,
                                const double* __restrict__ pb, int lane, double& acc0, double& acc1, double& acc2, int dbg,
                                double pc0, double pc1, double pc2) {
  if (!PSL && nrows > 128) slice_rows<CNT, 2, PSL, MODE, NT>(d, nrows, rec, pval, x, y, pa, pb, lane, acc0, acc1, acc2, dbg, pc0, pc1, pc2);
  else slice_rows<CNT, 1, PSL, MODE, NT>(d, nrows, rec, pval, x, y, pa, pb, lane, acc0, acc1, acc2, dbg, pc0, pc1, pc2);
}

template <bool PSL, int MODE, bool NT>
__device__ __forceinline__ void slice_dispatch(int cnt, const SDesc& d, int nrows, int rec, const double* __restrict__ pval,
                                      const double* __restrict__ x, double* __restrict__ y,
                                      const double* __restrict__ pa, const double* __restrict__ pb, int lane, double& acc0,
                                      double& acc1, double& acc2, int dbg, double pc0, double pc1, double pc2) {
  switch (cnt) {
    case 1: slice_nb<1, PSL, MODE, NT>(d, nrows, rec, pval, x, y, pa, pb, lane, acc0, acc1, acc2, dbg, pc0, pc1, pc2); break;
    case 3: slice_nb<3, PSL, MODE, NT>(d, nrows, rec, pval, x, y, pa, pb, lane, acc0, acc1, acc2, dbg, pc0, pc1, pc2); break;
    case 5: slice_nb<5, PSL, MODE, NT>(d, nrows, rec, pval, x, y, pa, pb, lane, acc0, acc1, acc2, dbg, pc0, pc1, pc2); break;
    case 7: slice_nb<7, PSL, MODE, NT>(d, nrows, rec, pval, x, y, pa, pb, lane, acc0, acc1, acc2, dbg, pc0, pc1, pc2); break;
    case 2: slice_nb<2, PSL, MODE, NT>(d, nrows, rec, pval, x, y, pa, pb, lane, acc0, acc1, acc2, dbg, pc0, pc1, pc2); break;
    case 4: slice_nb<4, PSL, MODE, NT>(d, nrows, rec, pval, x, y, pa, pb, lane, acc0, acc1, acc2, dbg, pc0, pc1, pc2); break;
    case 6: slice_nb<6, PSL, MODE, NT>(d, nrows, rec, pval, x, y, pa, pb, lane, acc0, acc1, acc2, dbg, pc0, pc1, pc2); break;
    default: slice_nb<8, PSL, MODE, NT>(d, nrows, rec, pval, x, y, pa, pb, lane, acc0, acc1, acc2, dbg, pc0, pc1, pc2); break;
  }
}


#ifndef PG_MARCH_K
#define PG_MARCH_K 4
#endif
#ifndef PG_MARCH_SPLIT
#define PG_MARCH_SPLIT 1
#endif
constexpr int MARCH_K = PG_MARCH_K, MARCH_KS = 2, MARCH_REC = 64, MARCH_W = 126;
constexpr int MARCH_EDGE = pghost::EDGE_REC, MARCH_ESLOTS = pghost::EDGE_SLOTS;
static_assert(MARCH_K > MARCH_KS && 18 + 4 * MARCH_K <= MARCH_EDGE && MARCH_EDGE + 2 + MARCH_K <= MARCH_REC, "unit record layout");

__device__ inline double lane_up(double v) {
  return __shfl_down(v, 1, 64);
}

struct MarchSide {
  d2_t ym, yp, ax, ax2;
};

template <int CNT, int MODE, bool EDGE>
__device__ __forceinline__ double march_plane(const double (&c)[CNT], int rng, int l2, double* __restrict__ yrow, const d2_t& xm,
                                              double xm_n, const d2_t& xc, const d2_t& xp, const MarchSide& sd, double pc0,
                                              double pc1, double pc2, double& acc0, double& acc1, double& acc2, int dbg,
                                              int einfo, int e_first, const d2_t* el, const d2_t* cl) {
  using MI = ModeInfo<MODE>;
  constexpr bool Y = CNT == 7;
  const double xc_nx = lane_up(xc.x), xc_ny = lane_up(xc.y), xp_n = lane_up(xp.x);
  double a1[CNT], a2[CNT];
  {
    int j = 0;
    a1[j] = xc_nx; a2[j] = xc_ny; ++j;
    a1[j] = xc.x;  a2[j] = xc.y;  ++j;
    if (Y) {
      a1[j] = sd.yp.x; a2[j] = sd.yp.y; ++j;
      a1[j] = sd.ym.x; a2[j] = sd.ym.y; ++j;
    }
    a1[j] = xp.y;  a2[j] = xp_n;  ++j;
    a1[j] = xm.y;  a2[j] = xm_n;  ++j;
    a1[j] = xc.y;  a2[j] = xc_nx;
  }
  double s1 = 0.0, s2 = 0.0;
  int lo = rng & 255, hi = rng >> 8;
  if (EDGE) {
    const int nlo = einfo & 255, nhi = (einfo >> 8) & 255, e0 = (einfo >> 16) - e_first;
    const int elo = lo - nlo, ehi = hi + nhi, p1 = l2 + 1, p2 = l2 + 2;
    const bool g1 = p1 >= elo && p1 < ehi && !(p1 >= lo && p1 < hi), g2 = p2 >= elo && p2 < ehi && !(p2 >= lo && p2 < hi);
    const d2_t* q1 = g1 ? el + (e0 + (p1 - elo) - (p1 >= hi ? hi - lo : 0)) : cl;
    const d2_t* q2 = g2 ? el + (e0 + (p2 - elo) - (p2 >= hi ? hi - lo : 0)) : cl;
#pragma unroll
    for (int jp = 0; jp < (CNT + 1) / 2; ++jp) {
      const d2_t w1 = q1[64 * jp], w2 = q2[64 * jp];
      s1 += w1.x * a1[2 * jp];
      s2 += w2.x * a2[2 * jp];
      if (2 * jp + 1 < CNT) {
        s1 += w1.y * a1[2 * jp + 1];
        s2 += w2.y * a2[2 * jp + 1];
      }
    }
    lo = elo;
    hi = ehi;
  } else {
#pragma unroll
    for (int j = 0; j < CNT; ++j) { s1 += c[j] * a1[j]; s2 += c[j] * a2[j]; }
  }
  s1 = mode_out<MODE>(s1, xc.y, sd.ax2.x, pc0, pc1, pc2);
  s2 = mode_out<MODE>(s2, xc_nx, sd.ax2.y, pc0, pc1, pc2);
  const bool nost = (dbg & 32) && s1 != 1.2345e-300;
  const bool allst = (dbg & 512) != 0;
  const bool v1 = ((l2 + 1 >= lo && l2 + 1 < hi) || allst) && !nost, v2 = ((l2 + 2 >= lo && l2 + 2 < hi) || allst) && !nost;
  if (v1 && v2) {
    d2u_t out;
    out.x = s1; out.y = s2;
    if (!(dbg & 2048)) __builtin_nontemporal_store(out, reinterpret_cast<d2u_t*>(yrow));
    else *reinterpret_cast<d2u_t*>(yrow) = out;
  } else if (v1) {
    yrow[0] = s1;
  } else if (v2) {
    yrow[1] = s2;
  }
  if (MI::DOT0) {
    const double w1 = v1 ? s1 : 0.0, w2 = v2 ? s2 : 0.0;
    acc0 += (v1 ? sd.ax.x : 0.0) * w1 + (v2 ? sd.ax.y : 0.0) * w2;
    if (MI::DOT1) acc1 += w1 * w1 + w2 * w2;
    if (MI::DOT2) acc2 += (v1 ? sd.ax2.x : 0.0) * w1 + (v2 ? sd.ax2.y : 0.0) * w2;
  }
  return xc_nx;
}

template <int CNT, int MODE, bool EDGE, int KK, int Q0 = 0, int KTOT = KK>
__device__ __forceinline__ void march_unit(int rec, int lane, const double* __restrict__ x, double* __restrict__ y,
                                  const double* __restrict__ pa, const double* __restrict__ pb, double pc0, double pc1,
                                  double pc2, double& acc0, double& acc1, double& acc2, int dbg,
                                  const double* __restrict__ e_val, double* sv, double* sx) {
  using MI = ModeInfo<MODE>;
  constexpr bool Y = CNT == 7;
  const int amask = (dbg & 128) ? ~1 : ~0;
  const int one = (dbg & 128) ? 0 : 1;
  const bool nolat = (dbg & 64) != 0;
  double c[CNT];
#pragma unroll
  for (int j = 0; j < CNT; ++j) c[j] = __hiloint2double(rlane(rec, 3 + 2 * j), rlane(rec, 2 + 2 * j));
  const int l2 = 2 * lane;
  int rb[KK];
  d2_t ln[KK + 2];
  MarchSide sd[KK];
  const bool act = lane < (rlane(rec, 0) >> 16);
  d2_t zero;
  zero.x = zero.y = 0.0;
#pragma unroll
  for (int q = 0; q < KK + 2; ++q) ln[q] = zero;
#pragma unroll
  for (int q = 0; q < KK; ++q) {
    rb[q] = rlane(rec, 18 + 4 * (Q0 + q)) & amask;
    sd[q].ym = sd[q].yp = sd[q].ax = sd[q].ax2 = zero;
  }
  if (act) {
    ln[0] = load_pair<false>(x + (rlane(rec, Q0 == 0 ? 16 : 18 + 4 * (Q0 - 1)) & amask) + l2);
#pragma unroll
    for (int q = 0; q < KK; ++q) ln[q + 1] = load_pair<false>(x + rb[q] + l2);
    ln[KK + 1] = load_pair<false>(x + (rlane(rec, Q0 + KK == KTOT ? 17 : 18 + 4 * (Q0 + KK)) & amask) + l2);
#pragma unroll
    for (int q = 0; q < KK; ++q) {
      if (Y && !nolat) {
        sd[q].ym = load_pair<false>(x + rb[q] + (rlane(rec, 19 + 4 * (Q0 + q)) & amask) + l2 + one);
        sd[q].yp = load_pair<false>(x + rb[q] + (rlane(rec, 20 + 4 * (Q0 + q)) & amask) + l2 + one);
      }
      if (MI::HAS_A) sd[q].ax = load_pair<false>(pa + rb[q] + l2 + one);
      if (MI::HAS_B) sd[q].ax2 = load_pair<false>(pb + rb[q] + l2 + one);
    }
  }
  const int e_first = rlane(rec, MARCH_EDGE + 2 + Q0) >> 16;
  const int e_cnt = (Q0 + KK == KTOT ? rlane(rec, MARCH_EDGE + 1) : rlane(rec, MARCH_EDGE + 2 + Q0 + KK) >> 16) - e_first;
  int elane = lane;
  if (EDGE) asm volatile("" : "+v"(elane));
  if (EDGE && e_cnt > 0) {
    const int e_all = rlane(rec, MARCH_EDGE + 1);
    const double* ep = e_val + (i64)MARCH_ESLOTS * rlane(rec, MARCH_EDGE) + 2 * (e_first + elane);
    asm volatile("s_waitcnt lgkmcnt(0)" ::: "memory");
    if (elane < e_cnt) {
#pragma unroll
      for (int jp = 0; jp < (CNT + 1) / 2; ++jp)
        __builtin_amdgcn_global_load_lds((const __attribute__((address_space(1))) void*)(ep + 2 * jp * e_all),
                                         (__attribute__((address_space(3))) void*)(sv + 128 * jp), 16, 0, 0);
    }
    asm volatile("s_waitcnt vmcnt(0)" ::: "memory");
  }
  if (EDGE) {
    const int k = elane - 2;
    if (k >= 0 && k < 2 * CNT) reinterpret_cast<int*>(sx)[256 * (k >> 2) + (k & 3)] = rec;
  }
  const d2_t* el = reinterpret_cast<const d2_t*>(sv);
  const d2_t* cl = reinterpret_cast<const d2_t*>(sx);
  double xm_n = lane_up(ln[0].x);
#pragma unroll
  for (int q = 0; q < KK; ++q)
    xm_n = march_plane<CNT, MODE, EDGE>(c, rlane(rec, 21 + 4 * (Q0 + q)), l2, y + rb[q] + l2 + one, ln[q], xm_n, ln[q + 1], ln[q + 2], sd[q], pc0,
                                  pc1, pc2, acc0, acc1, acc2, dbg, rlane(rec, MARCH_EDGE + 2 + Q0 + q), e_first, el, cl);
}

template <int CNT, int MODE, bool EDGE>
__device__ __forceinline__ void march_dispatch(int rec, int lane, const double* __restrict__ x, double* __restrict__ y,
                                      const double* __restrict__ pa, const double* __restrict__ pb, double pc0, double pc1,
                                      double pc2, double& acc0, double& acc1, double& acc2, int dbg,
                                      const double* __restrict__ e_val, double* sv, double* sx) {
  constexpr bool SPLIT = MODE == 3 && MARCH_K == 2 * MARCH_KS && PG_MARCH_SPLIT;
  if ((rlane(rec, 0) & 255) == MARCH_K) {
    if (SPLIT) {
      march_unit<CNT, MODE, EDGE, MARCH_KS, 0, MARCH_K>(rec, lane, x, y, pa, pb, pc0, pc1, pc2, acc0, acc1, acc2, dbg, e_val, sv, sx);
      march_unit<CNT, MODE, EDGE, MARCH_KS, MARCH_KS, MARCH_K>(rec, lane, x, y, pa, pb, pc0, pc1, pc2, acc0, acc1, acc2, dbg, e_val, sv, sx);
    } else {
      march_unit<CNT, MODE, EDGE, MARCH_K>(rec, lane, x, y, pa, pb, pc0, pc1, pc2, acc0, acc1, acc2, dbg, e_val, sv, sx);
    }
  } else {
    march_unit<CNT, MODE, EDGE, MARCH_KS>(rec, lane, x, y, pa, pb, pc0, pc1, pc2, acc0, acc1, acc2, dbg, e_val, sv, sx);
  }
}

template <int MODE, bool NT, bool DIAG>
__global__ __launch_bounds__(BLOCK, 4) void k_spmv_s(i64 nslices, const int* __restrict__ srec,
                                                  const double* __restrict__ pval, const int* __restrict__ g_rowid,
                                                  const int* __restrict__ g_rowptr, const int* __restrict__ g_col,
                                                  const double* __restrict__ g_val, const double* __restrict__ x,
                                                  double* __restrict__ y, const double* __restrict__ aux,
                                                  double* __restrict__ partials, const double* __restrict__ sc, int xcd,
                                                  FinArgs fin, int pstride, int accum, const int* __restrict__ mrec,
                                                  i64 nunits, const int* __restrict__ tiles, int tpx,
                                                  const double* __restrict__ e_val) {
  __shared__ __attribute__((aligned(16))) double s_val[BLOCK / 64][512];
  __shared__ __attribute__((aligned(16))) double s_x[BLOCK / 64][512];
  __shared__ double s_red[BLOCK / 64];
  if (sc && sc[S_DONE] != 0.0) return;
  using MI = ModeInfo<MODE>;
  constexpr bool DOTS = MI::DOT0;
  const double* __restrict__ dx = fin.dotx ? fin.dotx : x;
  const double* __restrict__ pa = MODE == 1 ? aux : ((MODE == 2 || MODE == 3) ? dx : nullptr);
  const double* __restrict__ pb = MODE == 3 ? aux : (MODE == 8 ? fin.base : nullptr);
  const int lane = threadIdx.x & 63;
  const int wave = __builtin_amdgcn_readfirstlane(threadIdx.x >> 6);
  double* __restrict__ sv = s_val[wave];
  double* __restrict__ sx = s_x[wave];
  d2_t* sv2 = reinterpret_cast<d2_t*>(sv);
  d2_t* sx2 = reinterpret_cast<d2_t*>(sx);
  double acc0 = 0.0, acc1 = 0.0, acc2 = 0.0;
  const int dbg = DIAG ? (xcd >> 8) : 0;
  xcd &= 255;
  xcd &= 1;
  const bool xsplit = xcd && gridDim.x >= 8;
  const int xid = xsplit ? (blockIdx.x & 7) : 0;
  const int woff = xsplit ? (int)(blockIdx.x >> 3) * (BLOCK / 64) + wave : (int)blockIdx.x * (BLOCK / 64) + wave;
  const int wstr = xsplit ? (int)(((i64)gridDim.x + 7 - xid) >> 3) * (BLOCK / 64) : (int)gridDim.x * (BLOCK / 64);
  const int* __restrict__ tb = tiles ? tiles + 2 * (tpx + 1) * xid : nullptr;
  const int ntile = tiles ? tpx : 1;
  const int l31 = lane & 31;
  for (int tile = 0; tile < ntile; ++tile) {
  i64 ulo, uhi, slo, shi, ubase, sbase;
  if (tiles) {
    ubase = tb[0]; sbase = tb[1];
    ulo = tb[2 * tile]; slo = tb[2 * tile + 1]; uhi = tb[2 * tile + 2]; shi = tb[2 * tile + 3];
  } else if (xsplit) {
    ubase = ulo = nunits * xid / 8; uhi = nunits * (xid + 1) / 8;
    sbase = slo = nslices * xid / 8; shi = nslices * (xid + 1) / 8;
  } else {
    ubase = ulo = 0; uhi = nunits;
    sbase = slo = 0; shi = nslices;
  }
  auto run_units = [&]() __attribute__((always_inline)) {
  if (nunits > 0) {
    int d = (woff - (int)(ulo - ubase)) % wstr;
    d = d < 0 ? d + wstr : d;
    i64 ucur = ulo + d;
    const i64 ustride = wstr;
    int urec = ucur < uhi ? mrec[(unsigned)(MARCH_REC * (int)ucur + lane)] : 0;
    for (; ucur < uhi; ucur += ustride) {
      const i64 un = ucur + ustride;
      const int urec_n = mrec[(unsigned)(MARCH_REC * (int)(un < uhi ? un : ucur) + lane)];
      if (!(dbg & 16)) {
        const bool edge = rlane(urec, MARCH_EDGE + 1) > 0;
        if (((rlane(urec, 0) >> 8) & 255) == 7) {
          if (edge) march_dispatch<7, MODE, true>(urec, lane, x, y, pa, pb, fin.pc0, fin.pc1, fin.pc2, acc0, acc1, acc2, dbg, e_val, sv, sx);
          else march_dispatch<7, MODE, false>(urec, lane, x, y, pa, pb, fin.pc0, fin.pc1, fin.pc2, acc0, acc1, acc2, dbg, e_val, sv, sx);
        } else {
          if (edge) march_dispatch<5, MODE, true>(urec, lane, x, y, pa, pb, fin.pc0, fin.pc1, fin.pc2, acc0, acc1, acc2, dbg, e_val, sv, sx);
          else march_dispatch<5, MODE, false>(urec, lane, x, y, pa, pb, fin.pc0, fin.pc1, fin.pc2, acc0, acc1, acc2, dbg, e_val, sv, sx);
        }
      }
      urec = urec_n;
    }
  }
  };
  auto run_slices = [&]() __attribute__((always_inline)) {
  int ds_ = (woff - (int)(slo - sbase)) % wstr;
  ds_ = ds_ < 0 ? ds_ + wstr : ds_;
  const i64 first = slo + ds_, wstride = wstr, hi = shi;
  const i64 lastc = hi - 1;
  int rec = first < hi ? srec[(unsigned)(SL_REC * (int)first + l31)] : 0;
  int rec_n = srec[(unsigned)(SL_REC * (int)(first + wstride < hi ? first + wstride : (first < hi ? lastc : 0)) + l31)];
  for (i64 chunk = first; chunk < hi; chunk += wstride) {
    const i64 cnn = chunk + 2 * wstride;
    const int rec_nn = srec[(unsigned)(SL_REC * (int)(cnn < hi ? cnn : lastc) + l31)];
    SDesc d;
    d.r0 = rlane(rec, 0); d.meta = rlane(rec, 1); d.base = rlane(rec, 2); d.aux = rlane(rec, 3);
    const int nrows = d.meta & 255, type = (d.meta >> 8) & 3, cnt = d.meta >> 16;
    const bool skip = ((dbg & 1) && type == SL_G) || ((dbg & 2) && type != SL_G);
    if (skip) {
    } else if (type == SL_U) {
      slice_dispatch<false, MODE, NT>(cnt, d, nrows, rec, pval, x, y, pa, pb, lane, acc0, acc1, acc2, dbg, fin.pc0, fin.pc1, fin.pc2);
    } else if (type == SL_P) {
      slice_dispatch<true, MODE, NT>(cnt, d, nrows, rec, pval, x, y, pa, pb, lane, acc0, acc1, acc2, dbg, fin.pc0, fin.pc1, fin.pc2);
    } else {
      Desc dd;
      dd.r0 = d.r0; dd.base = d.base; dd.r1 = d.r0 + nrows; dd.end = d.aux;
      StreamW q;
      stream_issue_w<NT>(q, dd, g_rowptr, g_col, g_val, lane);
      const bool live = lane < nrows;
      const int rid = g_rowid[d.r0 + (live ? lane : 0)];
      const int basev = dd.base & ~1, basec = dd.base & ~3;
      const int av = q.ra - basev, ac = q.ra - basec, len = q.rb - q.ra;
#pragma unroll
      for (int j = 0; j < XV_IT; ++j) sv2[lane + 64 * j] = q.v[j];
      const double opa = MI::HAS_A ? pa[rid] : 0.0, opb = MI::HAS_B ? pb[rid] : 0.0;
      const double xown = MI::OWN ? x[rid] : 0.0;
      double xg[XC_IT][4];
#pragma unroll
      for (int j = 0; j < XC_IT; ++j) {
        xg[j][0] = x[q.c[j].x]; xg[j][1] = x[q.c[j].y]; xg[j][2] = x[q.c[j].z]; xg[j][3] = x[q.c[j].w];
      }
#pragma unroll
      for (int j = 0; j < XC_IT; ++j) {
        d2_t lo2, hi2;
        lo2.x = xg[j][0]; lo2.y = xg[j][1]; hi2.x = xg[j][2]; hi2.y = xg[j][3];
        sx2[2 * (lane + 64 * j)] = lo2;
        sx2[2 * (lane + 64 * j) + 1] = hi2;
      }
      __builtin_amdgcn_wave_barrier();
      double sum = 0.0;
      int maxlen = len;
#pragma unroll
      for (int off = 32; off > 0; off >>= 1) {
        const int other = __shfl_xor(maxlen, off, 64);
        maxlen = other > maxlen ? other : maxlen;
      }
      maxlen = __builtin_amdgcn_readfirstlane(maxlen);
      for (int j0 = 0; j0 < maxlen; j0 += GUNR) {
        double vv[GUNR], xv[GUNR];
#pragma unroll
        for (int j = 0; j < GUNR; ++j) {
          const int k = j0 + j < len ? j0 + j : 0;
          vv[j] = sv[av + k];
          xv[j] = sx[ac + k];
        }
#pragma unroll
        for (int j = 0; j < GUNR; ++j)
          if (j0 + j < len) sum += vv[j] * xv[j];
      }
      __builtin_amdgcn_wave_barrier();
      if (live) {
        sum = mode_out<MODE>(sum, xown, opb, fin.pc0, fin.pc1, fin.pc2);
        y[rid] = sum;
        if (MI::DOT0) acc0 += opa * sum;
        if (MI::DOT1) acc1 += sum * sum;
        if (MI::DOT2) acc2 += opb * sum;
      }
    }
    rec = rec_n;
    rec_n = rec_nn;
  }
  };
  if (DIAG && (dbg & 4096)) { run_slices(); run_units(); }
  else { run_units(); run_slices(); }
  }
  if (DOTS) {
    const double t0 = block_sum(acc0, s_red);
    if (threadIdx.x == 0) put_partial(partials + blockIdx.x, t0, accum);
  }
  if (MI::DOT1) {
    const double t1 = block_sum(acc1, s_red);
    if (threadIdx.x == 0) put_partial(partials + pstride + blockIdx.x, t1, accum);
  }
  if (MI::DOT2) {
    const double t2 = block_sum(acc2, s_red);
    if (threadIdx.x == 0) put_partial(partials + 4 * (size_t)pstride + blockIdx.x, t2, accum);
  }
  if (DOTS) fold_scalar_phase(fin, partials, s_red, pstride);
}

__global__ void k_row_same(i64 n, const int* __restrict__ rowptr, const int* __restrict__ col,
                           const double* __restrict__ val, unsigned char* __restrict__ flags) {
  for (i64 r = blockIdx.x * (i64)blockDim.x + threadIdx.x; r < n; r += (i64)gridDim.x * blockDim.x) {
    unsigned char f = 0;
    bool ghost = false;
    for (int k = rowptr[r]; k < rowptr[r + 1]; ++k) ghost = ghost || col[k] >= n;
    if (r > 0) {
      const int a = rowptr[r], b = rowptr[r + 1], pa = rowptr[r - 1];
      if (b - a == a - pa) {
        bool same = true, vsame = true;
        for (int k = 0; k < b - a; ++k) {
          same = same && (col[a + k] - 1 == col[pa + k]);
          vsame = vsame && (__double_as_longlong(val[a + k]) == __double_as_longlong(val[pa + k]));
        }
        f = same ? (vsame ? 3 : 1) : 0;
      }
    }
    flags[r] = f | (ghost ? 4 : 0);
  }
}

__global__ void k_pval_fill(i64 nslices, const int* __restrict__ srec, const int* __restrict__ rowptr,
                            const double* __restrict__ val, double* __restrict__ pval) {
  for (i64 sidx = blockIdx.x; sidx < nslices; sidx += gridDim.x) {
    const int r0 = srec[SL_REC * sidx], meta = srec[SL_REC * sidx + 1], base = srec[SL_REC * sidx + 2];
    if (((meta >> 8) & 3) != SL_P) continue;
// ... 43 lines not shown

}
void ensure_csr_chunks(const CsrMatrix& A);
namespace {

#define PG_LAUNCH_C_ARGS(KERNEL, X, Y, AUX, PART)                                                               \
  hipLaunchKernelGGL(HIP_KERNEL_NAME(KERNEL), dim3(grid), dim3(BLOCK), 0, st, A.n, A.nchunks, A.chunk_desc.p, \
                     A.rowptr.p, A.col.p, A.val.p, X, Y, AUX, PART, (const double*)nullptr)
#define PG_LAUNCH_C(KERNEL)                                                                                    \
  hipLaunchKernelGGL(HIP_KERNEL_NAME(KERNEL), dim3(grid), dim3(BLOCK), 0, st, A.n, A.nchunks, A.chunk_desc.p, \
                     A.rowptr.p, A.col.p, A.val.p, x, y, aux, partials, sc)

template <int MODE>
bool launch_slices(int v, const CsrMatrix& A, i64 s0, i64 ns, const double* x, double* y, const double* aux, double* partials,
                   const double* sc, int grid, int pstride, int accum, hipStream_t st, const FinArgs* fin, bool units = true) {
  FinArgs fa{nullptr, nullptr, PH_NONE, 0, 0, nullptr};
  if (fin && MODE >= 1) fa = *fin;
  const int* rec = A.srec.p + SL_REC * s0;
  const i64 nu = units ? A.nunits : 0;
  const bool tiled = units && A.tiles_per_xcd > 0 && s0 == 0 && ns == A.tile_ns && (xcd_map() & 1) && grid >= 8;
  const int* tiles = tiled ? (const int*)A.tiles.p : nullptr;
  const int tpx = tiled ? A.tiles_per_xcd : 0;
  if (xcd_map() >= 256)
    hipLaunchKernelGGL(HIP_KERNEL_NAME(k_spmv_s<MODE, true, true>), dim3(grid), dim3(BLOCK), 0, st, ns, rec, A.pval.p,
                       A.g_rowid.p, A.g_rowptr.p, A.g_col.p, A.g_val.p, x, y, aux, partials, sc, xcd_map(), fa, pstride, accum,
                       (const int*)A.mrec.p, nu, tiles, tpx, (const double*)A.e_val.p);
  else if (v & 4)
    hipLaunchKernelGGL(HIP_KERNEL_NAME(k_spmv_s<MODE, true, false>), dim3(grid), dim3(BLOCK), 0, st, ns, rec, A.pval.p,
                       A.g_rowid.p, A.g_rowptr.p, A.g_col.p, A.g_val.p, x, y, aux, partials, sc, xcd_map(), fa, pstride, accum,
                       (const int*)A.mrec.p, nu, tiles, tpx, (const double*)A.e_val.p);
  else
    hipLaunchKernelGGL(HIP_KERNEL_NAME(k_spmv_s<MODE, false, false>), dim3(grid), dim3(BLOCK), 0, st, ns, rec, A.pval.p,
                       A.g_rowid.p, A.g_rowptr.p, A.g_col.p, A.g_val.p, x, y, aux, partials, sc, xcd_map(), fa, pstride, accum,
                       (const int*)A.mrec.p, nu, tiles, tpx, (const double*)A.e_val.p);
  return fa.ticket != nullptr;
}

template <int MODE>
bool launch_mode(int v, const CsrMatrix& A, const double* x, double* y, const double* aux, double* partials,
                 const double* sc, int grid, hipStream_t st, const FinArgs* fin) {
  if (v & 64) return launch_slices<MODE>(v, A, 0, A.nslices, x, y, aux, partials, sc, grid, grid, 0, st, fin);
  PG_REQUIRE(MODE != 8 && !(fin && fin->dotx), "the preconditioner products and separate dot operands need the slice kernel");
  if (v != 1) ensure_csr_chunks(A);
  if (v == 1) {
    hipLaunchKernelGGL(HIP_KERNEL_NAME(k_spmv<MODE>), dim3(grid), dim3(BLOCK), 0, st, A.n, A.rowptr.p, A.col.p, A.val.p, x, y,
                       aux, partials, sc);
    return false;
  }
  if (v & 4) PG_LAUNCH_C((k_spmv_cw<MODE, true>));
  else PG_LAUNCH_C((k_spmv_cw<MODE, false>));
  return false;
}

}


namespace {

struct Slice {
  int r0, meta, base, aux;
  int key;
  int bnd;
  i64 okey = 0;
};

using pghost::MRun;

constexpr int RUN_INFO = 25;

__global__ void k_run_info(i64 nruns, const int* __restrict__ run_r0, const int* __restrict__ rowptr,
                           const int* __restrict__ col, const double* __restrict__ val, const int* __restrict__ cell,
                           const int* __restrict__ map, int* __restrict__ out) {
  for (i64 q = blockIdx.x * (i64)blockDim.x + threadIdx.x; q < nruns; q += (i64)gridDim.x * blockDim.x) {
    const int r = run_r0[q], a = rowptr[r], len = rowptr[r + 1] - a;
    out[RUN_INFO * q + 24] = cell ? cell[map ? map[r] : r] : -1;
    for (int k = 0; k < 8; ++k) {
      out[RUN_INFO * q + k] = k < len ? col[a + k] - r : 0;
      const double v = k < len ? val[a + k] : 0.0;
      out[RUN_INFO * q + 8 + 2 * k] = __double2loint(v);
      out[RUN_INFO * q + 9 + 2 * k] = __double2hiint(v);
    }
  }
}

__global__ void k_fill_units(i64 nunits, int* __restrict__ mrec, const int* __restrict__ rowptr,
                             const double* __restrict__ val) {
  for (i64 q = blockIdx.x * (i64)blockDim.x + threadIdx.x; q < nunits; q += (i64)gridDim.x * blockDim.x) {
    int* rec = mrec + MARCH_REC * q;
    const int cnt = (rec[0] >> 8) & 255, a = rowptr[rec[1]];
    for (int k = 0; k < cnt; ++k) {
      rec[2 + 2 * k] = __double2loint(val[a + k]);
      rec[3 + 2 * k] = __double2hiint(val[a + k]);
    }
  }
}

__global__ void k_fill_edges(i64 ne, const int* __restrict__ meta, const int* __restrict__ rowptr, const double* __restrict__ val,
                             double* __restrict__ e_val) {
  for (i64 q = blockIdx.x * (i64)blockDim.x + threadIdx.x; q < ne; q += (i64)gridDim.x * blockDim.x) {
    const int r = meta[4 * q], dst = meta[4 * q + 1], dist = meta[4 * q + 2], sm = meta[4 * q + 3];
    const int a = rowptr[r], len = sm >> 24;
    for (int j = 0; j < MARCH_ESLOTS; ++j) e_val[dst + (i64)(j >> 1) * dist + (j & 1)] = 0.0;
    for (int k = 0; k < len; ++k) {
      const int j = (sm >> (3 * k)) & 7;
      e_val[dst + (i64)(j >> 1) * dist + (j & 1)] = val[a + k];
    }
// ... 638 lines not shown
```

Baseline: 1310.

## Run the early Chebyshev polynomial preconditioner products in fp32 with an f64 tail

Adds a mixed-precision schedule for the polynomial preconditioner. Most Horner-style SpMV products in the chain read and write float32 vectors, and a few final factors stay in float64. Root ordering and tail length are picked from the required accuracy and the spectral bound, and the degree-selection cost model is adjusted to account for the cheaper fp32 launches. The goal is to cut vector traffic in the bandwidth-bound SpMV chain, at the cost of precision risk that the f64 tail and a safety margin are meant to absorb.

```diff
diff --git a/include/penguin_hip.h b/include/penguin_hip.h
--- a/include/penguin_hip.h
+++ b/include/penguin_hip.h
@@ -114,6 +114,11 @@
   int64_t poly_xspace;
   int64_t products;
   int64_t guess_states_read;
+  int64_t poly_f32_launches;
+  double poly_f32_ms_total;
+  int64_t poly_f32_timed;
+  int64_t poly_f32_chains;
+  int64_t poly_f32_tail_sum;
 } pg_run_info;
 
 typedef struct {
@@ -296,6 +301,9 @@
                             const double* dotx, const double* base, double pc0, double pc1, double pc2, int32_t fold,
                             int32_t done, int32_t repeat, double* y, double* partials, double* slot_sums, double* folded,
                             int64_t* ticket);
+#define PG_DEBUG_SPMV_SENTINEL_F32 0x7FC5EED0u
+int32_t pg_debug_spmv_apply_typed(pg_solver* s, int32_t which, int32_t kind, const void* x, const void* base, double pc0, double pc1,
+                                  double pc2, double sigma, int32_t done, double* y64, float* y32, float* p32);
 int32_t pg_debug_read_probe(int64_t bytes, int32_t elem_bytes, int32_t nt, int32_t blocks, int32_t reps, double* gbs);
 int32_t pg_debug_run_virtual_ranks(int32_t nranks, int32_t N, const int64_t* n, const double* L, int32_t body_kind,
                                    const double* params, int32_t nparams, double interface_value, double border_value,
diff --git a/penguin/jl_amd/_lib.py b/penguin/jl_amd/_lib.py
--- a/penguin/jl_amd/_lib.py
+++ b/penguin/jl_amd/_lib.py
@@ -73,7 +73,9 @@
                 ("solve_ms", C.c_double), ("spmv_ms_total", C.c_double), ("spmv_launches", C.c_int64),
                 ("unconverged_steps", C.c_int64), ("worst_relres", C.c_double), ("spmv_lean_ms_total", C.c_double),
                 ("spmv_lean_launches", C.c_int64), ("poly_degree", C.c_int64), ("half_exits", C.c_int64),
-                ("poly_xspace", C.c_int64), ("products", C.c_int64), ("guess_states_read", C.c_int64)]
+                ("poly_xspace", C.c_int64), ("products", C.c_int64), ("guess_states_read", C.c_int64),
+                ("poly_f32_launches", C.c_int64), ("poly_f32_ms_total", C.c_double), ("poly_f32_timed", C.c_int64),
+                ("poly_f32_chains", C.c_int64), ("poly_f32_tail_sum", C.c_int64)]
 
 
 class pg_system_info(C.Structure):
@@ -303,3 +305,32 @@
                                     C.c_double(pc[0]), C.c_double(pc[1]), C.c_double(pc[2]), C.c_int32(fold), C.c_int32(done),
                                     C.c_int32(repeat), dptr(y), dptr(partials), dptr(sums), dptr(folded), C.byref(ticket)))
     return {"y": y, "partials": partials, "slot_sums": sums, "folded": folded, "ticket": ticket.value, "grid": grid, "n": n}
+
+
+DEBUG_SPMV_SENTINEL_F32 = 0x7FC5EED0
+TYPED_FIRST, TYPED_MIDDLE, TYPED_HANDOVER = 1, 2, 3
+
+
+def debug_spmv_apply_typed(handle, which: int, kind: int, x, base=None, pc=(0.0, 0.0, 0.0), sigma: float = 1.0, done: int = 0) -> dict:
+    n, nv, _, _ = debug_spmv_sizes(handle, which)
+    want_x = np.float64 if kind == TYPED_FIRST else np.float32
+    want_b = {TYPED_FIRST: None, TYPED_MIDDLE: np.float32, TYPED_HANDOVER: np.float64}[kind]
+    x = np.ascontiguousarray(x)
+    if x.dtype != want_x or x.size != nv:
+        raise ValueError(f"debug_spmv_apply_typed: x must be {nv} x {np.dtype(want_x).name}")
+    if (base is None) != (want_b is None):
+        raise ValueError("debug_spmv_apply_typed: base goes with kinds 2 and 3, and only with them")
+    bp = None
+    if base is not None:
+        base = np.ascontiguousarray(base)
+        if base.dtype != want_b or base.size != n:
+            raise ValueError(f"debug_spmv_apply_typed: base must be {n} x {np.dtype(want_b).name}")
+        bp = base.ctypes.data_as(C.c_void_p)
+    y64 = np.zeros(n + DEBUG_SPMV_GUARD) if kind == TYPED_HANDOVER else None
+    y32 = np.zeros(n + DEBUG_SPMV_GUARD, dtype=np.float32) if kind != TYPED_HANDOVER else None
+    p32 = np.zeros(n + DEBUG_SPMV_GUARD, dtype=np.float32) if kind == TYPED_FIRST else None
+    ptr = lambda a: None if a is None else a.ctypes.data_as(C.c_void_p)
+    check(lib().pg_debug_spmv_apply_typed(handle, C.c_int32(which), C.c_int32(kind), x.ctypes.data_as(C.c_void_p), bp,
+                                          C.c_double(pc[0]), C.c_double(pc[1]), C.c_double(pc[2]), C.c_double(sigma), C.c_int32(done),
+                                          ptr(y64), ptr(y32), ptr(p32)))
+    return {"y": y64 if kind == TYPED_HANDOVER else y32, "p32": p32}
diff --git a/penguin/jl_amd/csrc/pg_common.h b/penguin/jl_amd/csrc/pg_common.h
--- a/penguin/jl_amd/csrc/pg_common.h
+++ b/penguin/jl_amd/csrc/pg_common.h
@@ -72,6 +72,8 @@
   bool poly_trend = true;
   int poly_maxdeg = 0;
   int poly_mindeg = 4;
+  bool poly_f32 = true;
+  int poly_f32_tail = -1;
   int profile_sample = 3;
   bool gamma_elim = true;
   bool diag_elim = true;
diff --git a/penguin/jl_amd/csrc/pg_context.hip b/penguin/jl_amd/csrc/pg_context.hip
--- a/penguin/jl_amd/csrc/pg_context.hip
+++ b/penguin/jl_amd/csrc/pg_context.hip
@@ -45,6 +45,8 @@
     k.poly_maxdeg = (int)geti("PG_POLY_MAXDEG", 0);
     k.poly_mindeg = (int)std::max<long long>(2, std::min<long long>(8, geti("PG_POLY_MINDEG", 4)));
     k.poly_trend = geti("PG_POLY_TREND", 1) != 0;
+    k.poly_f32 = geti("PG_POLY_F32", 1) != 0;
+    k.poly_f32_tail = (int)std::max<long long>(-1, std::min<long long>(64, geti("PG_POLY_F32_TAIL", -1)));
     k.profile_sample = (int)std::max<long long>(1, geti("PG_PROFILE_SAMPLE", 3));
     k.gamma_elim = geti("PG_GAMMA_ELIM", 1) != 0;
     k.diag_elim = geti("PG_DIAG_ELIM", 1) != 0;
@@ -366,11 +368,11 @@
   snprintf(tmp, sizeof(tmp),
            "spmv_variant=%d spmv_xcd=%d spmv_strip=%d spmv_unit_order=%d spmv_march=%d spmv_edges=%d spmv_march_k=%d spmv_minrun=%d spmv_tile_units=%d "
            "spmv_blocks_per_cu=%d halo_overlap=%d speculate=%d poly=%d poly_degree=%d poly_adapt=%d "
-           "poly_margin=%g poly_slack=%g poly_hist=%d poly_trend=%d poly_maxdeg=%d gamma_elim=%d diag_elim=%d "
+           "poly_margin=%g poly_slack=%g poly_hist=%d poly_trend=%d poly_maxdeg=%d poly_f32=%d poly_f32_tail=%d gamma_elim=%d diag_elim=%d "
            "guess_states=%d guess_depth=%d guess_defer=%d async_alloc=%d cache_limit_mb=%lld alloc_poison=%d alloc_guard=%d profile_sample=%d debug=%d",
            k.spmv_variant, k.spmv_xcd, k.spmv_strip, k.unit_order, (int)k.spmv_march, (int)k.spmv_edges, k.spmv_march_k, k.spmv_minrun, k.spmv_tile_units,
            k.spmv_blocks_per_cu, (int)k.halo_overlap, (int)k.speculate_product, (int)k.poly, k.poly_degree, (int)k.poly_adapt,
-           k.poly_margin, k.poly_slack, k.poly_hist, (int)k.poly_trend, k.poly_maxdeg,
+           k.poly_margin, k.poly_slack, k.poly_hist, (int)k.poly_trend, k.poly_maxdeg, (int)k.poly_f32, k.poly_f32_tail,
            (int)k.gamma_elim, (int)k.diag_elim, k.guess_n, k.guess_depth, (int)k.guess_defer, k.async_alloc, k.pool_limit_mb, k.alloc_poison, k.alloc_guard, k.profile_sample, (int)k.debug);
   if (buf && n > 0) {
     std::strncpy(buf, tmp, n - 1);
diff --git a/penguin/jl_amd/csrc/pg_host_algos.h b/penguin/jl_amd/csrc/pg_host_algos.h
--- a/penguin/jl_amd/csrc/pg_host_algos.h
+++ b/penguin/jl_amd/csrc/pg_host_algos.h
@@ -574,4 +574,86 @@
   return 0;
 }
 
-}
+constexpr int MIXED_MAX_DEGREE = 40;
+constexpr double MIXED_FLOOR32 = 1e-7;
+constexpr double MIXED_DAMP = 0.45;
+constexpr double MIXED_SAFETY = 0.5;
+enum { CHAIN_F64 = 0, CHAIN_FIRST = 1, CHAIN_MIDDLE = 2, CHAIN_HANDOVER = 3 };
+
+struct MixedChain {
+  int m = 0, j = 0, n32 = 0;
+  int order[MIXED_MAX_DEGREE];
+  int kind[MIXED_MAX_DEGREE];
+};
+
+inline double mixed_root(int m, double g, int k) { return 1.0 + g * std::cos(M_PI * (2.0 * k + 1.0) / (2.0 * m)); }
+inline double mixed_rho(double g) { return g / (1.0 + std::sqrt(std::max(0.0, 1.0 - g * g))); }
+
+inline void mixed_alternate(const int* idx, int n, int* out) {
+  for (int k = 0, lo = 0, hi = n - 1; k < n; ++k) out[k] = (k & 1) ? idx[hi--] : idx[lo++];
+}
+
+inline bool mixed_chain_schedule(int m, double g, int j, MixedChain& out) {
+  if (m < 2 || m > MIXED_MAX_DEGREE || j < 0) return false;
+  if (j < 1) j = 1;
+  const int n32 = m - 1 - j;
+  if (n32 < 2) return false;
+  out.m = m; out.j = j; out.n32 = n32;
+  bool taken[MIXED_MAX_DEGREE];
+  for (int k = 0; k < m; ++k) taken[k] = false;
+  int tail[MIXED_MAX_DEGREE], head[MIXED_MAX_DEGREE];
+  for (int q = 0; q < j; ++q) {
+    const double c = mixed_root(j, g, q);
+    int best = -1;
+    double dbest = 0.0;
+    for (int k = 0; k < m; ++k) {
+      if (taken[k]) continue;
+      const double d = std::fabs(mixed_root(m, g, k) - c);
+      if (best < 0 || d < dbest) { best = k; dbest = d; }
+    }
+    taken[best] = true;
+  }
+  int nt = 0, nh = 0;
+  for (int k = 0; k < m; ++k) (taken[k] ? tail[nt++] : head[nh++]) = k;
+  mixed_alternate(head, nh, out.order);
+  mixed_alternate(tail, nt, out.order + nh);
+  for (int i = 0; i < m - 1; ++i)
+    out.kind[i] = i == 0 ? CHAIN_FIRST : (i < n32 ? CHAIN_MIDDLE : (i == n32 ? CHAIN_HANDOVER : CHAIN_F64));
+  out.kind[m - 1] = CHAIN_F64;
+  return true;
+}
+
+inline int mixed_chain_tail(double needed, double g, int m) {
+  if (!(needed > 0.0) || !(needed < 1.0) || m < 2 || m > MIXED_MAX_DEGREE) return -1;
+  const double damp = std::max(MIXED_DAMP, mixed_rho(g));
+  int j = 1;
+  double left = MIXED_FLOOR32 * damp;
+  while (left > MIXED_SAFETY * needed && j < m) { left *= damp; ++j; }
+  return m - 1 - j >= 2 ? j : -1;
+}
+
+inline long double mixed_tail_max(const MixedChain& c, double g) {
+  const int j = c.j;
+  long double r[MIXED_MAX_DEGREE];
+  for (int q = 0; q < j; ++q) {
+    const int k = c.order[c.m - j + q];
+    r[q] = 1.0L + (long double)g * cosl(3.141592653589793238462643383279502884L * (2.0L * k + 1.0L) / (2.0L * c.m));
+  }
+  std::sort(r, r + j);
+  auto P = [&](long double x) { long double p = 1.0L; for (int q = 0; q < j; ++q) p *= 1.0L - x / r[q]; return fabsl(p); };
+  long double best = std::max(P(1.0L - (long double)g), P(1.0L + (long double)g));
+  for (int q = 0; q + 1 < j; ++q) {
+    long double a = r[q], b = r[q + 1];
+    for (int it = 0; it < 200; ++it) {
+      const long double x = 0.5L * (a + b);
+      if (!(x > a && x < b)) break;
+      long double d = 0.0L;
+      for (int t = 0; t < j; ++t) d += 1.0L / (x - r[t]);
+      if (d > 0.0L) a = x; else b = x;
+    }
+    best = std::max(best, P(0.5L * (a + b)));
+  }
+  return best;
+}
+
+}
diff --git a/penguin/jl_amd/csrc/pg_krylov.h b/penguin/jl_amd/csrc/pg_krylov.h
--- a/penguin/jl_amd/csrc/pg_krylov.h
+++ b/penguin/jl_amd/csrc/pg_krylov.h
@@ -39,6 +39,10 @@
   const int* moved_flag = nullptr;
   int moved_stamp = 0;
   DevBuf<double> ya, yb, wa, wb;
+  DevBuf<float> fa, fb, p32;
+  const void* mix_matrix = nullptr;
+  double mix_sigma = 0.0, mix_need = 0.0;
+  int mix_wait = 0;
   DevBuf<double> gm_basis, gm, gm_partials;
   int gm_m = -1;
   DevBuf<double> bl_vecs, bl, bl_partials;
@@ -61,6 +65,8 @@
   int poly_xspace = 0;
   i64 products = 0;
   int polls = 0;
+  i64 f32_launches = 0, f32_timed = 0, f32_chains = 0, f32_tail_sum = 0;
+  double f32_ms = 0.0;
 };
 
 void halo_exchange(const Numbering& nb, const Slab& slab, double* vec, hipStream_t st);
diff --git a/penguin/jl_amd/csrc/pg_krylov.hip b/penguin/jl_amd/csrc/pg_krylov.hip
--- a/penguin/jl_amd/csrc/pg_krylov.hip
+++ b/penguin/jl_amd/csrc/pg_krylov.hip
@@ -1,3 +1,4 @@
+#include "pg_host_algos.h"
 #include "pg_krylov.h"
 #include "pg_multigrid.h"
 #include "pg_spmv.h"
@@ -358,8 +359,9 @@
   std::vector<char> lean_of;
   std::vector<char> second_of;
   std::vector<int> count_of;
+  std::vector<char> f32_of;
   int cur = 0, cur_count = 1;
-  bool cur_lean = false, cur_second = false;
+  bool cur_lean = false, cur_second = false, cur_f32 = false;
   bool armed = false;
   explicit SpmvTimer(bool on_) : on(on_) {}
   static std::vector<hipEvent_t>& pool() {
@@ -377,14 +379,15 @@
     PG_HIP(hipEventCreate(&e));
     return e;
   }
-  void begin(hipStream_t st, int iteration, bool lean = false, bool second = false, int count = 1) {
+  void begin(hipStream_t st, int iteration, bool lean = false, bool second = false, int count = 1, bool f32 = false) {
     cur = iteration;
     cur_lean = lean;
     cur_second = second;
     cur_count = count;
+    cur_f32 = f32;
     const int sample = config().profile_sample;
-    static thread_local unsigned long long counter = 0;
-    armed = on && (counter++ % sample == 0);
+    static thread_local unsigned long long counter = 0, counter_f32 = 0;
+    armed = on && ((f32 ? counter_f32++ : counter++) % sample == 0);
     if (!armed) return;
     e0 = take();
     e1 = take();
@@ -398,6 +401,7 @@
     lean_of.push_back(cur_lean ? 1 : 0);
     second_of.push_back(cur_second ? 1 : 0);
     count_of.push_back(cur_count);
+    f32_of.push_back(cur_f32 ? 1 : 0);
   }
   void collect(SolveStats& s, int iters_done, bool half_exit) {
     for (size_t q = 0; q < pairs.size(); ++q) {
@@ -406,7 +410,8 @@
       (void)hipEventSynchronize(pr.second);
       const bool ran = iter_of[q] < iters_done && !(half_exit && iter_of[q] == iters_done - 1 && second_of[q]);
       if (ran && hipEventElapsedTime(&ms, pr.first, pr.second) == hipSuccess) {
-        if (lean_of[q]) { s.spmv_lean_ms += ms; s.spmv_lean_launches += count_of[q]; }
+        if (f32_of[q]) { s.f32_ms += ms; s.f32_timed += count_of[q]; }
+        else if (lean_of[q]) { s.spmv_lean_ms += ms; s.spmv_lean_launches += count_of[q]; }
         else { s.spmv_ms += ms; s.spmv_launches += 1; }
       }
       pool().push_back(pr.first);
@@ -417,6 +422,7 @@
     lean_of.clear();
     second_of.clear();
     count_of.clear();
+    f32_of.clear();
   }
 };
 
@@ -475,7 +481,9 @@
 
 namespace {
 
-void choose_next_degree(const CsrMatrix& A, const SolveStats& stats, int m, bool adaptive, KrylovWork& w) {
+constexpr double F32_LAUNCH_WEIGHT = 0.87;
+
+void choose_next_degree(const CsrMatrix& A, const SolveStats& stats, int m, bool adaptive, KrylovWork& w, double mixed_g) {
   const Config& cfg = config();
   const bool keep_degree = adaptive && stats.converged && stats.iters == 0 && w.adapt_m >= 2;
   w.adapt_matrix = nullptr;
@@ -503,7 +511,11 @@
     const int mm = std::max(cfg.poly_mindeg, (int)std::ceil(need / h));
     const int maxdeg = cfg.poly_maxdeg > 0 ? std::min(MAX_POLY_DEGREE, std::max(4, cfg.poly_maxdeg)) : 32;
     if (mm > maxdeg) continue;
-    const double cost = h * (1.0 + 1.18 * (mm - 2) + 3.6);
+    double cost = h * (1.0 + 1.18 * (mm - 2) + 3.6);
+    if (mixed_g > 0.0) {
+      const int jt = pghost::mixed_chain_tail(std::pow(std::sqrt(tol2 / rr0), 1.0 / h), mixed_g, mm);
+      if (jt >= 0) cost -= (1.0 - F32_LAUNCH_WEIGHT) * 1.18 * (mm - jt - 2);
+    }
     if (cost < best) { best = cost; w.adapt_m = mm; w.adapt_h = h; }
   }
   if (best < 1e300) w.adapt_matrix = &A;
@@ -631,6 +643,27 @@
     w.ya.alloc(nvec); w.wa.alloc(nvec); w.wb.alloc(nvec); w.yb.alloc(nvec);
     w.ya.zero(); w.wa.zero(); w.wb.zero(); w.yb.zero();
   }
+  pghost::MixedChain mc;
+  bool mixed = false;
+  double mix_sigma = 1.0;
+  double mtau[MAX_POLY_DEGREE];
+  if (poly && cfg.poly_f32 && cx.nranks == 1 && !cx.comm && !A.halo_needed && spmv_supports_typed_chain() && w.mix_matrix == &A &&
+      w.mix_sigma > 0.0) {
+    const double g = std::min(std::max(by_estimate ? A.est.g_used : A.gersh, 0.05), 0.95);
+    int j = cfg.poly_f32_tail >= 0 ? cfg.poly_f32_tail : pghost::mixed_chain_tail(w.mix_need, g, m);
+    if (j >= 0 && w.mix_wait > 0 && cfg.poly_f32_tail < 0) j += 2;
+    if (w.mix_wait > 0) --w.mix_wait;
+    if (j >= 0 && pghost::mixed_chain_schedule(m, g, j, mc)) {
+      mixed = true;
+      mix_sigma = w.mix_sigma;
+      for (int i = 0; i < m; ++i) mtau[i] = 1.0 / pghost::mixed_root(m, g, mc.order[i]);
+      if (w.fa.n < nvec) {
+        w.fa.alloc(nvec); w.fb.alloc(nvec); w.p32.alloc(nvec);
+        w.fa.zero(); w.fb.zero(); w.p32.zero();
+      }
+    }
+  }
+  bool mixed_ran = false;
   const bool half_test = m >= 3 || mg;
   PG_REQUIRE(!xg.zbase || (poly && p_in_rhat && w.scatter), "an unformed extrapolated state needs the polynomial loop on a compact system");
   PG_REQUIRE(!preinit || !cg, "preinit is a BiCGStab path");
@@ -666,6 +699,51 @@
     double* src = in;
     if (poly) {
       double* hat = second ? w.yb.p : w.ya.p;
+      if (mixed && itn == 0 && !second) {
+        const int n32 = mc.n32, nf32 = n32 + 1, nf64 = m - 1 - nf32;
+        const void* src32 = nullptr;
+        timer.begin(st, itn, true, second, nf32, true);
+        for (int i = 0; i <= n32; ++i) {
+          const double tk = mtau[i + 1];
+          FinArgs f{nullptr, nullptr, PH_NONE, 0, 0, nullptr};
+          if (i == 0) {
+            float* dst = w.fa.p;
+            f.pc0 = mix_sigma * mtau[0]; f.pc1 = -mix_sigma * (mtau[0] * tk); f.pc2 = mix_sigma * tk;
+            f.base = in; f.p32 = w.p32.p; f.psig = mix_sigma;
+            launch_spmv_typed(TYPED_FIRST, A, in, dst, w.sc.p, G, st, f);
+            src32 = dst;
+          } else if (i < n32) {
+            float* dst = (i & 1) ? w.fb.p : w.fa.p;
+            f.pc0 = 1.0; f.pc1 = -tk; f.pc2 = tk;
+            f.base = reinterpret_cast<const double*>(w.p32.p);
+            launch_spmv_typed(TYPED_MIDDLE, A, src32, dst, w.sc.p, G, st, f);
+            src32 = dst;
+          } else {
+            double* dst = i == m - 2 ? hat : ((i & 1) ? w.wb.p : w.wa.p);
+            const double inv = 1.0 / mix_sigma;
+            f.pc0 = inv; f.pc1 = -inv * tk; f.pc2 = tk;
+            f.base = in;
+            launch_spmv_typed(TYPED_HANDOVER, A, src32, dst, w.sc.p, G, st, f);
+            src = dst;
+          }
+        }
+        timer.end(st);
+        if (nf64 > 0) {
+          timer.begin(st, itn, true, second, nf64);
+          for (int i = n32 + 1; i <= m - 2; ++i) {
+            double* dst = i == m - 2 ? hat : ((i & 1) ? w.wb.p : w.wa.p);
+            FinArgs f{nullptr, nullptr, PH_NONE, 0, 0, nullptr};
+            f.pc0 = 1.0; f.pc1 = -mtau[i + 1]; f.pc2 = mtau[i + 1]; f.base = in;
+            launch_spmv(8, A, src, dst, nullptr, nullptr, w.sc.p, G, st, &f);
+            src = dst;
+          }
+          timer.end(st);
+        }
+        mixed_ran = true;
+        stats.f32_launches += nf32;
+        stats.f32_chains += 1;
+        stats.f32_tail_sum += mc.j;
+      } else {
       timer.begin(st, itn, true, second, m - 1);
       for (int k = m - 2; k >= 0; --k) {
         double* dst = k == 0 ? hat : ((k & 1) ? w.wb.p : w.wa.p);
@@ -676,6 +754,7 @@
         src = dst;
       }
       timer.end(st);
+      }
     } else if (mg) {
       double* hat = second ? w.yb.p : w.ya.p;
       timer.begin(st, itn, true, second, 1);
@@ -796,7 +875,25 @@
     const double rr0 = w.h_sc[S_RR0], rr = w.h_sc[S_HALF] != 0.0 ? w.h_sc[S_RED4] : w.h_sc[S_RR];
     if (rr0 > 0.0 && rr > 0.0 && rr < rr0) w.last_rate2 = std::log(rr0 / rr) / (double)stats.products;
   }
-  choose_next_degree(A, stats, m, adaptive, w);
-}
-
-}
+  const bool mix_env = poly && cfg.poly_f32 && cx.nranks == 1 && !cx.comm && !A.halo_needed && spmv_supports_typed_chain();
+  choose_next_degree(A, stats, m, adaptive, w,
+                     mix_env && cfg.poly_f32_tail < 0 ? std::min(std::max(by_estimate ? A.est.g_used : A.gersh, 0.05), 0.95) : 0.0);
+  if (stats.iters == 0) stats.f32_launches = stats.f32_chains = stats.f32_tail_sum = 0;
+  if (mixed_ran && expect_halves == 1 && !(stats.iters == 1 && stats.half_exit)) w.mix_wait = 2 * (m + 3);
+  w.mix_matrix = nullptr;
+  if (mix_env && stats.converged) {
+    const double rr0 = w.h_sc[S_RR0], tol2 = w.h_sc[S_TOL2];
+    if (rr0 > 0.0 && rr0 < 1e300 && tol2 > 0.0) {
+      int e = 0;
+      (void)std::frexp(std::sqrt(rr0 / (double)n), &e);
+      const int h = (adaptive && w.adapt_matrix == &A && w.adapt_h >= 1) ? w.adapt_h : std::max(1, 2 * stats.iters - stats.half_exit);
+      if (e > -100 && e < 100) {
+        w.mix_matrix = &A;
+        w.mix_sigma = std::ldexp(1.0, -e);
+        w.mix_need = std::pow(std::sqrt(std::min(1.0, tol2 / rr0)), 1.0 / h);
+      }
+    }
+  }
+}
+
+}
diff --git a/penguin/jl_amd/csrc/pg_solver.hip b/penguin/jl_amd/csrc/pg_solver.hip
--- a/penguin/jl_amd/csrc/pg_solver.hip
+++ b/penguin/jl_amd/csrc/pg_solver.hip
@@ -1885,6 +1885,8 @@
     tot.poly_xspace = st.poly_xspace;
     tot.half_exit += st.half_exit;
     tot.products += st.products;
+    tot.f32_launches += st.f32_launches; tot.f32_ms += st.f32_ms; tot.f32_timed += st.f32_timed;
+    tot.f32_chains += st.f32_chains; tot.f32_tail_sum += st.f32_tail_sum;
     if (!st.converged) ++unconverged;
     if (st.bnorm > 0.0) worst = std::max(worst, st.resnorm / st.bnorm);
   };
@@ -1930,6 +1932,11 @@
     info->poly_xspace = tot.poly_xspace;
     info->half_exits = tot.half_exit;
     info->products = tot.products;
+    info->poly_f32_launches = tot.f32_launches;
+    info->poly_f32_ms_total = tot.f32_ms;
+    info->poly_f32_timed = tot.f32_timed;
+    info->poly_f32_chains = tot.f32_chains;
+    info->poly_f32_tail_sum = tot.f32_tail_sum;
     info->guess_states_read = 0;
     if (s->guess_coef.n >= 16) {
       double hc[16];
@@ -2412,6 +2419,67 @@
   PG_API_END
 }
 
+int32_t pg_debug_spmv_apply_typed(pg_solver* s, int32_t which, int32_t kind, const void* x, const void* base, double pc0, double pc1,
+                                  double pc2, double sigma, int32_t done, double* y64, float* y32, float* p32) {
+  PG_API_BEGIN
+  require_init();
+  PG_REQUIRE(s && x, "pg_debug_spmv_apply_typed: NULL argument");
+  PG_REQUIRE(ctx().nranks == 1 && !ctx().comm, "pg_debug_spmv_apply_typed: one rank");
+  PG_REQUIRE(kind == TYPED_FIRST || kind == TYPED_MIDDLE || kind == TYPED_HANDOVER, "pg_debug_spmv_apply_typed: kinds 1 (first), 2 (middle), 3 (hand-over)");
+  PG_REQUIRE((kind == TYPED_FIRST) == (base == nullptr), "pg_debug_spmv_apply_typed: the first launch's base is its x; the others take one");
+  PG_REQUIRE((kind == TYPED_FIRST) == (p32 != nullptr), "pg_debug_spmv_apply_typed: p32 is the first launch's output, and only its");
+  PG_REQUIRE(kind == TYPED_HANDOVER ? (y64 && !y32) : (y32 && !y64), "pg_debug_spmv_apply_typed: y32 for kinds 1 and 2, y64 for kind 3");
+  PG_REQUIRE(spmv_supports_typed_chain(), "pg_debug_spmv_apply_typed: the typed launches exist in the slice kernel with the stream hint only");
+  i64 nv = 0;
+  const CsrMatrix& A = debug_matrix(s, which, &nv);
+  const i64 n = A.n;
+  PG_REQUIRE(n > 0 && A.srec.p, "pg_debug_spmv_apply_typed: the matrix has no rows or no slice image");
+  nv = std::max(nv, n);
+  hipStream_t st = ctx().stream;
+  const int grid = spmv_default_grid(n);
+  constexpr i64 GUARD = 64;
+  double sentinel;
+  const unsigned long long sbits = PG_DEBUG_SPMV_SENTINEL;
+  std::memcpy(&sentinel, &sbits, sizeof(double));
+  float sentinel32;
+  const unsigned sbits32 = PG_DEBUG_SPMV_SENTINEL_F32;
+  std::memcpy(&sentinel32, &sbits32, sizeof(float));
+  DevBuf<double> dx64(nv), db64(nv), dy64(n + GUARD), dsc(S_COUNT);
+  DevBuf<float> dx32(nv), db32(nv), dy32(n + GUARD), dp32(n + GUARD);
+  db64.zero(); db32.zero();
+  if (kind == TYPED_FIRST) dx64.upload(static_cast<const double*>(x), nv);
+  else dx32.upload(static_cast<const float*>(x), nv);
+  if (kind == TYPED_MIDDLE) db32.upload(static_cast<const float*>(base), n);
+  if (kind == TYPED_HANDOVER) db64.upload(static_cast<const double*>(base), n);
+  {
+    std::vector<double> f64((size_t)(n + GUARD), sentinel);
+    std::vector<float> f32((size_t)(n + GUARD), sentinel32);
+    dy64.upload(f64.data(), n + GUARD);
+    dy32.upload(f32.data(), n + GUARD);
+    dp32.upload(f32.data(), n + GUARD);
+    std::vector<double> hsc(S_COUNT, 0.0);
+    hsc[S_DONE] = (double)done;
+    dsc.upload(hsc.data(), S_COUNT);
+  }
+  FinArgs f{nullptr, nullptr, PH_NONE, 0, 0, nullptr};
+  f.pc0 = pc0; f.pc1 = pc1; f.pc2 = pc2;
+  if (kind == TYPED_FIRST) {
+    f.base = dx64.p; f.p32 = dp32.p; f.psig = sigma;
+    launch_spmv_typed(kind, A, dx64.p, dy32.p, dsc.p, grid, st, f);
+  } else if (kind == TYPED_MIDDLE) {
+    f.base = reinterpret_cast<const double*>(db32.p);
+    launch_spmv_typed(kind, A, dx32.p, dy32.p, dsc.p, grid, st, f);
+  } else {
+    f.base = db64.p;
+    launch_spmv_typed(kind, A, dx32.p, dy64.p, dsc.p, grid, st, f);
+  }
+  PG_HIP(hipGetLastError());
+  if (y64) dy64.download(y64, n + GUARD);
+  if (y32) dy32.download(y32, n + GUARD);
+  if (p32) dp32.download(p32, n + GUARD);
+  PG_API_END
+}
+
 __global__ void k_scale_rows(i64 n_e, const int* __restrict__ elist, double factor, double* __restrict__ z) {
   for (i64 q = blockIdx.x * (i64)blockDim.x + threadIdx.x; q < n_e; q += (i64)gridDim.x * blockDim.x) z[elist[q]] *= factor;
 }
diff --git a/penguin/jl_amd/csrc/pg_spmv.h b/penguin/jl_amd/csrc/pg_spmv.h
--- a/penguin/jl_amd/csrc/pg_spmv.h
+++ b/penguin/jl_amd/csrc/pg_spmv.h
@@ -153,6 +153,8 @@
   double pc0 = 0.0, pc1 = 0.0;
   const double* base = nullptr;
   double pc2 = 0.0;
+  float* p32 = nullptr;
+  double psig = 0.0;
 };
 
 __device__ inline void fold_scalar_phase(const FinArgs& fin, const double* __restrict__ partials, double* s_red, int nparts) {
@@ -171,6 +173,10 @@
                  const double* sc, int grid, hipStream_t st, const FinArgs* fin = nullptr);
 bool launch_spmv_as(int variant, int mode, const CsrMatrix& A, const double* x, double* y, const double* aux, double* partials,
                     const double* sc, int grid, hipStream_t st, const FinArgs* fin = nullptr);
+enum { TYPED_FIRST = 1, TYPED_MIDDLE = 2, TYPED_HANDOVER = 3 };
+void launch_spmv_typed(int kind, const CsrMatrix& A, const void* x, void* y, const double* sc, int grid, hipStream_t st,
+                       const FinArgs& fin);
+bool spmv_supports_typed_chain();
 bool spmv_with_halo(int mode, const CsrMatrix& A, const Numbering& nb, const Slab& slab, double* x, double* y, const double* aux,
                     double* partials, const double* sc, int grid, hipStream_t st, const FinArgs* fin = nullptr);
 void launch_spmv_variant(int variant, const CsrMatrix& A, const double* x, double* y, hipStream_t st);
diff --git a/penguin/jl_amd/csrc/pg_spmv.hip b/penguin/jl_amd/csrc/pg_spmv.hip
--- a/penguin/jl_amd/csrc/pg_spmv.hip
+++ b/penguin/jl_amd/csrc/pg_spmv.hip
@@ -1,6 +1,7 @@
 #include <algorithm>
 #include <cstdlib>
 #include <thread>
+#include <type_traits>
 #include <vector>
 
 #include "pg_host_algos.h"
@@ -222,6 +223,65 @@
   return r;
 }
 
+template <class TX_, class TB_, class TY_, bool P32_>
+struct VecTypes {
+  using TX = TX_;
+  using TB = TB_;
+  using TY = TY_;
+  static constexpr bool P32 = P32_;
+};
+using VecF64 = VecTypes<double, double, double, false>;
+
+typedef float f2u_t __attribute__((ext_vector_type(2), aligned(4)));
+
+template <bool NT>
+__device__ inline d2_t load_pair_t(const double* p) { return load_pair<NT>(p); }
+template <bool NT>
+__device__ inline d2_t load_pair_t(const float* p) {
+  const f2u_t* q = reinterpret_cast<const f2u_t*>(p);
+  f2u_t v = NT ? __builtin_nontemporal_load(q) : *q;
+  d2_t r;
+  r.x = (double)v.x; r.y = (double)v.y;
+  return r;
+}
+typedef float f2_t __attribute__((ext_vector_type(2)));
+template <class T> struct PairOf { typedef d2_t type; };
+template <> struct PairOf<float> { typedef f2_t type; };
+template <bool NT>
+__device__ inline d2_t load_raw(const double* p) { return load_pair<NT>(p); }
+template <bool NT>
+__device__ inline f2_t load_raw(const float* p) {
+  const f2u_t* q = reinterpret_cast<const f2u_t*>(p);
+  f2u_t v = NT ? __builtin_nontemporal_load(q) : *q;
+  f2_t r;
+  r.x = v.x; r.y = v.y;
+  return r;
+}
+__device__ inline d2_t widen(const d2_t& v) { return v; }
+__device__ inline d2_t widen(const f2_t& v) {
+  d2_t r;
+  r.x = (double)v.x; r.y = (double)v.y;
+  return r;
+}
+__device__ inline void store_pair_t(double* p, double a, double b, bool plain) {
+  d2u_t out;
+  out.x = a; out.y = b;
+  if (!plain) __builtin_nontemporal_store(out, reinterpret_cast<d2u_t*>(p));
+  else *reinterpret_cast<d2u_t*>(p) = out;
+}
+__device__ inline float narrow(double a) {
+  const float f = (float)a;
+  return __builtin_fminf(__builtin_fmaxf(f, -3.402823466e+38f), 3.402823466e+38f);
+}
+__device__ inline void store_pair_t(float* p, double a, double b, bool plain) {
+  f2u_t out;
+  out.x = narrow(a); out.y = narrow(b);
+  if (!plain) __builtin_nontemporal_store(out, reinterpret_cast<f2u_t*>(p));
+  else *reinterpret_cast<f2u_t*>(p) = out;
+}
+__device__ inline void store_one_t(double* p, double a) { *p = a; }
+__device__ inline void store_one_t(float* p, double a) { *p = narrow(a); }
+
 template <int MODE>
 struct ModeInfo {
   static constexpr bool OWN = MODE == 8;
@@ -238,18 +298,18 @@
   return s;
 }
 
-template <int CNT, int NB, bool PSL, int MODE, bool NT>
+template <int CNT, int NB, bool PSL, int MODE, bool NT, class VT>
 __device__ __forceinline__ void slice_rows(const SDesc& d, int nrows, int rec, const double* __restrict__ pval,
-                                  const double* __restrict__ x, double* __restrict__ y, const double* __restrict__ pa,
-                                  const double* __restrict__ pb, int lane, double& acc0, double& acc1, double& acc2, int dbg,
-                                  double pc0, double pc1, double pc2) {
+                                  const typename VT::TX* __restrict__ x, typename VT::TY* __restrict__ y, const double* __restrict__ pa,
+                                  const typename VT::TB* __restrict__ pb, int lane, double& acc0, double& acc1, double& acc2, int dbg,
+                                  double pc0, double pc1, double pc2, float* __restrict__ p32, double psig) {
   using MI = ModeInfo<MODE>;
   int o[CNT];
 #pragma unroll
   for (int j = 0; j < CNT; ++j) o[j] = (dbg & 4) ? 0 : rlane(rec, 4 + j);
   int l0[NB];
   bool live0[NB], live1[NB];
-  d2_t xv[NB][CNT];
+  typename PairOf<typename VT::TX>::type xv[NB][CNT];
 #pragma unroll
   for (int b = 0; b < NB; ++b) {
     const int l = 128 * b + 2 * lane;
@@ -257,7 +317,7 @@
     live1[b] = l + 1 < nrows;
     l0[b] = live0[b] ? l : 0;
 #pragma unroll
-    for (int j = 0; j < CNT; ++j) xv[b][j] = load_pair<false>(x + d.r0 + l0[b] + o[j]);
+    for (int j = 0; j < CNT; ++j) xv[b][j] = load_raw<false>(x + d.r0 + l0[b] + o[j]);
   }
   d2_t sum[NB];
 #pragma unroll
@@ -268,8 +328,9 @@
       const double c = __hiloint2double(rlane(rec, 13 + 2 * j), rlane(rec, 12 + 2 * j));
 #pragma unroll
       for (int b = 0; b < NB; ++b) {
-        sum[b].x += c * xv[b][j].x;
-        sum[b].y += c * xv[b][j].y;
+        const d2_t xw = widen(xv[b][j]);
+        sum[b].x += c * xw.x;
+        sum[b].y += c * xw.y;
       }
     }
   } else {
@@ -281,8 +342,9 @@
       for (int j = 0; j < CNT; ++j) vv[j] = load_pair<NT>(pv + j * nrows);
 #pragma unroll
       for (int j = 0; j < CNT; ++j) {
-        sum[b].x += vv[j].x * xv[b][j].x;
-        sum[b].y += vv[j].y * xv[b][j].y;
+        const d2_t xw = widen(xv[b][j]);
+        sum[b].x += vv[j].x * xw.x;
+        sum[b].y += vv[j].y * xw.y;
       }
     }
   }
@@ -290,28 +352,29 @@
 #pragma unroll
   for (int b = 0; b < NB; ++b) {
     own[b].x = own[b].y = ax[b].x = ax[b].y = ax2[b].x = ax2[b].y = 0.0;
-    if (MI::OWN) own[b] = load_pair<false>(x + d.r0 + l0[b]);
+    if (MI::OWN) own[b] = load_pair_t<false>(x + d.r0 + l0[b]);
     if (MI::HAS_A) ax[b] = load_pair<false>(pa + d.r0 + l0[b]);
-    if (MI::HAS_B) ax2[b] = load_pair<false>(pb + d.r0 + l0[b]);
+    if (MI::HAS_B && !VT::P32) ax2[b] = load_pair_t<false>(pb + d.r0 + l0[b]);
+    if (VT::P32) ax2[b] = own[b];
   }
 #pragma unroll
   for (int b = 0; b < NB; ++b) {
     sum[b].x = mode_out<MODE>(sum[b].x, own[b].x, ax2[b].x, pc0, pc1, pc2);
     sum[b].y = mode_out<MODE>(sum[b].y, own[b].y, ax2[b].y, pc0, pc1, pc2);
     const bool st = !(dbg & 8) || sum[b].x == 1.2345e-300;
-    double* yp = y + d.r0 + l0[b];
+    typename VT::TY* yp = y + d.r0 + l0[b];
+    if (VT::P32) {
+      float* pp = p32 + d.r0 + l0[b];
+      if (live1[b]) store_pair_t(pp, psig * ax2[b].x, psig * ax2[b].y, false);
+      else if (live0[b]) store_one_t(pp, psig * ax2[b].x);
+    }
     if (live1[b]) {
-      if (st) {
-        d2u_t out;
-        out.x = sum[b].x; out.y = sum[b].y;
-        if (!(dbg & 2048)) __builtin_nontemporal_store(out, reinterpret_cast<d2u_t*>(yp));
-        else *reinterpret_cast<d2u_t*>(yp) = out;
-      }
+      if (st) store_pair_t(yp, sum[b].x, sum[b].y, (dbg & 2048) != 0);
       if (MI::DOT0) acc0 += ax[b].x * sum[b].x + ax[b].y * sum[b].y;
       if (MI::DOT1) acc1 += sum[b].x * sum[b].x + sum[b].y * sum[b].y;
       if (MI::DOT2) acc2 += ax2[b].x * sum[b].x + ax2[b].y * sum[b].y;
     } else if (live0[b]) {
-      if (st) *yp = sum[b].x;
+      if (st) store_one_t(yp, sum[b].x);
       if (MI::DOT0) acc0 += ax[b].x * sum[b].x;
       if (MI::DOT1) acc1 += sum[b].x * sum[b].x;
       if (MI::DOT2) acc2 += ax2[b].x * sum[b].x;
@@ -319,29 +382,30 @@
   }
 }
 
-template <int CNT, bool PSL, int MODE, bool NT>
+template <int CNT, bool PSL, int MODE, bool NT, class VT>
 __device__ __forceinline__ void slice_nb(const SDesc& d, int nrows, int rec, const double* __restrict__ pval,
-                                const double* __restrict__ x, double* __restrict__ y, const double* __restrict__ pa,
-                                const double* __restrict__ pb, int lane, double& acc0, double& acc1, double& acc2, int dbg,
-                                double pc0, double pc1, double pc2) {
-  if (!PSL && nrows > 128) slice_rows<CNT, 2, PSL, MODE, NT>(d, nrows, rec, pval, x, y, pa, pb, lane, acc0, acc1, acc2, dbg, pc0, pc1, pc2);
-  else slice_rows<CNT, 1, PSL, MODE, NT>(d, nrows, rec, pval, x, y, pa, pb, lane, acc0, acc1, acc2, dbg, pc0, pc1, pc2);
-}
-
-template <bool PSL, int MODE, bool NT>
+                                const typename VT::TX* __restrict__ x, typename VT::TY* __restrict__ y, const double* __restrict__ pa,
+                                const typename VT::TB* __restrict__ pb, int lane, double& acc0, double& acc1, double& acc2, int dbg,
+                                double pc0, double pc1, double pc2, float* __restrict__ p32, double psig) {
+  if (!PSL && nrows > 128) slice_rows<CNT, 2, PSL, MODE, NT, VT>(d, nrows, rec, pval, x, y, pa, pb, lane, acc0, acc1, acc2, dbg, pc0, pc1, pc2, p32, psig);
+  else slice_rows<CNT, 1, PSL, MODE, NT, VT>(d, nrows, rec, pval, x, y, pa, pb, lane, acc0, acc1, acc2, dbg, pc0, pc1, pc2, p32, psig);
+}
+
+template <bool PSL, int MODE, bool NT, class VT>
 __device__ __forceinline__ void slice_dispatch(int cnt, const SDesc& d, int nrows, int rec, const double* __restrict__ pval,
-                                      const double* __restrict__ x, double* __restrict__ y,
-                                      const double* __restrict__ pa, const double* __restrict__ pb, int lane, double& acc0,
-                                      double& acc1, double& acc2, int dbg, double pc0, double pc1, double pc2) {
+                                      const typename VT::TX* __restrict__ x, typename VT::TY* __restrict__ y,
+                                      const double* __restrict__ pa, const typename VT::TB* __restrict__ pb, int lane, double& acc0,
+                                      double& acc1, double& acc2, int dbg, double pc0, double pc1, double pc2,
+                                      float* __restrict__ p32, double psig) {
   switch (cnt) {
-    case 1: slice_nb<1, PSL, MODE, NT>(d, nrows, rec, pval, x, y, pa, pb, lane, acc0, acc1, acc2, dbg, pc0, pc1, pc2); break;
-    case 3: slice_nb<3, PSL, MODE, NT>(d, nrows, rec, pval, x, y, pa, pb, lane, acc0, acc1, acc2, dbg, pc0, pc1, pc2); break;
-    case 5: slice_nb<5, PSL, MODE, NT>(d, nrows, rec, pval, x, y, pa, pb, lane, acc0, acc1, acc2, dbg, pc0, pc1, pc2); break;
-    case 7: slice_nb<7, PSL, MODE, NT>(d, nrows, rec, pval, x, y, pa, pb, lane, acc0, acc1, acc2, dbg, pc0, pc1, pc2); break;
-    case 2: slice_nb<2, PSL, MODE, NT>(d, nrows, rec, pval, x, y, pa, pb, lane, acc0, acc1, acc2, dbg, pc0, pc1, pc2); break;
-    case 4: slice_nb<4, PSL, MODE, NT>(d, nrows, rec, pval, x, y, pa, pb, lane, acc0, acc1, acc2, dbg, pc0, pc1, pc2); break;
-    case 6: slice_nb<6, PSL, MODE, NT>(d, nrows, rec, pval, x, y, pa, pb, lane, acc0, acc1, acc2, dbg, pc0, pc1, pc2); break;
-    default: slice_nb<8, PSL, MODE, NT>(d, nrows, rec, pval, x, y, pa, pb, lane, acc0, acc1, acc2, dbg, pc0, pc1, pc2); break;
+    case 1: slice_nb<1, PSL, MODE, NT, VT>(d, nrows, rec, pval, x, y, pa, pb, lane, acc0, acc1, acc2, dbg, pc0, pc1, pc2, p32, psig); break;
+    case 3: slice_nb<3, PSL, MODE, NT, VT>(d, nrows, rec, pval, x, y, pa, pb, lane, acc0, acc1, acc2, dbg, pc0, pc1, pc2, p32, psig); break;
+    case 5: slice_nb<5, PSL, MODE, NT, VT>(d, nrows, rec, pval, x, y, pa, pb, lane, acc0, acc1, acc2, dbg, pc0, pc1, pc2, p32, psig); break;
+    case 7: slice_nb<7, PSL, MODE, NT, VT>(d, nrows, rec, pval, x, y, pa, pb, lane, acc0, acc1, acc2, dbg, pc0, pc1, pc2, p32, psig); break;
+    case 2: slice_nb<2, PSL, MODE, NT, VT>(d, nrows, rec, pval, x, y, pa, pb, lane, acc0, acc1, acc2, dbg, pc0, pc1, pc2, p32, psig); break;
+    case 4: slice_nb<4, PSL, MODE, NT, VT>(d, nrows, rec, pval, x, y, pa, pb, lane, acc0, acc1, acc2, dbg, pc0, pc1, pc2, p32, psig); break;
+    case 6: slice_nb<6, PSL, MODE, NT, VT>(d, nrows, rec, pval, x, y, pa, pb, lane, acc0, acc1, acc2, dbg, pc0, pc1, pc2, p32, psig); break;
+    default: slice_nb<8, PSL, MODE, NT, VT>(d, nrows, rec, pval, x, y, pa, pb, lane, acc0, acc1, acc2, dbg, pc0, pc1, pc2, p32, psig); break;
   }
 }
 
@@ -360,17 +424,27 @@
   return __shfl_down(v, 1, 64);
 }
 
+template <class TX, class TB>
 struct MarchSide {
-  d2_t ym, yp, ax, ax2;
+  typename PairOf<TX>::type ym, yp;
+  d2_t ax;
+  typename PairOf<TB>::type ax2;
 };
 
-template <int CNT, int MODE, bool EDGE>
-__device__ __forceinline__ double march_plane(const double (&c)[CNT], int rng, int l2, double* __restrict__ yrow, const d2_t& xm,
-                                              double xm_n, const d2_t& xc, const d2_t& xp, const MarchSide& sd, double pc0,
+template <int CNT, int MODE, bool EDGE, class VT>
+__device__ __forceinline__ double march_plane(const double (&c)[CNT], int rng, int l2, typename VT::TY* __restrict__ yrow,
+                                              const typename PairOf<typename VT::TX>::type& xm_, double xm_n,
+                                              const typename PairOf<typename VT::TX>::type& xc_,
+                                              const typename PairOf<typename VT::TX>::type& xp_,
+                                              const MarchSide<typename VT::TX, typename VT::TB>& sd_, double pc0,
                                               double pc1, double pc2, double& acc0, double& acc1, double& acc2, int dbg,
-                                              int einfo, int e_first, const d2_t* el, const d2_t* cl) {
+                                              int einfo, int e_first, const d2_t* el, const d2_t* cl, float* __restrict__ prow,
+                                              double psig) {
   using MI = ModeInfo<MODE>;
   constexpr bool Y = CNT == 7;
+  const d2_t xm = widen(xm_), xc = widen(xc_), xp = widen(xp_);
+  struct { d2_t ym, yp, ax, ax2; } sd;
+  sd.ym = widen(sd_.ym); sd.yp = widen(sd_.yp); sd.ax = sd_.ax; sd.ax2 = widen(sd_.ax2);
   const double xc_nx = lane_up(xc.x), xc_ny = lane_up(xc.y), xp_n = lane_up(xp.x);
   double a1[CNT], a2[CNT];
   {
@@ -409,20 +483,23 @@
 #pragma unroll
     for (int j = 0; j < CNT; ++j) { s1 += c[j] * a1[j]; s2 += c[j] * a2[j]; }
   }
-  s1 = mode_out<MODE>(s1, xc.y, sd.ax2.x, pc0, pc1, pc2);
-  s2 = mode_out<MODE>(s2, xc_nx, sd.ax2.y, pc0, pc1, pc2);
+  const double b1 = VT::P32 ? xc.y : sd.ax2.x, b2 = VT::P32 ? xc_nx : sd.ax2.y;
+  s1 = mode_out<MODE>(s1, xc.y, b1, pc0, pc1, pc2);
+  s2 = mode_out<MODE>(s2, xc_nx, b2, pc0, pc1, pc2);
   const bool nost = (dbg & 32) && s1 != 1.2345e-300;
   const bool allst = (dbg & 512) != 0;
   const bool v1 = ((l2 + 1 >= lo && l2 + 1 < hi) || allst) && !nost, v2 = ((l2 + 2 >= lo && l2 + 2 < hi) || allst) && !nost;
+  if (VT::P32) {
+    if (v1 && v2) store_pair_t(prow, psig * b1, psig * b2, false);
+    else if (v1) store_one_t(prow, psig * b1);
+    else if (v2) store_one_t(prow + 1, psig * b2);
+  }
   if (v1 && v2) {
-    d2u_t out;
-    out.x = s1; out.y = s2;
-    if (!(dbg & 2048)) __builtin_nontemporal_store(out, reinterpret_cast<d2u_t*>(yrow));
-    else *reinterpret_cast<d2u_t*>(yrow) = out;
+    store_pair_t(yrow, s1, s2, (dbg & 2048) != 0);
   } else if (v1) {
-    yrow[0] = s1;
+    store_one_t(yrow, s1);
   } else if (v2) {
-    yrow[1] = s2;
+    store_one_t(yrow + 1, s2);
   }
   if (MI::DOT0) {
     const double w1 = v1 ? s1 : 0.0, w2 = v2 ? s2 : 0.0;
@@ -433,11 +510,11 @@
   return xc_nx;
 }
 
-template <int CNT, int MODE, bool EDGE, int KK, int Q0 = 0, int KTOT = KK>
-__device__ __forceinline__ void march_unit(int rec, int lane, const double* __restrict__ x, double* __restrict__ y,
-                                  const double* __restrict__ pa, const double* __restrict__ pb, double pc0, double pc1,
+template <int CNT, int MODE, bool EDGE, class VT, int KK, int Q0 = 0, int KTOT = KK>
+__device__ __forceinline__ void march_unit(int rec, int lane, const typename VT::TX* __restrict__ x, typename VT::TY* __restrict__ y,
+                                  const double* __restrict__ pa, const typename VT::TB* __restrict__ pb, double pc0, double pc1,
                                   double pc2, double& acc0, double& acc1, double& acc2, int dbg,
-                                  const double* __restrict__ e_val, double* sv, double* sx) {
+                                  const double* __restrict__ e_val, double* sv, double* sx, float* __restrict__ p32, double psig) {
   using MI = ModeInfo<MODE>;
   constexpr bool Y = CNT == 7;
   const int amask = (dbg & 128) ? ~1 : ~0;
@@ -448,31 +525,39 @@
   for (int j = 0; j < CNT; ++j) c[j] = __hiloint2double(rlane(rec, 3 + 2 * j), rlane(rec, 2 + 2 * j));
   const int l2 = 2 * lane;
   int rb[KK];
-  d2_t ln[KK + 2];
-  MarchSide sd[KK];
+  typedef typename PairOf<typename VT::TX>::type xpair_t;
+  typedef typename PairOf<typename VT::TB>::type bpair_t;
+  xpair_t ln[KK + 2];
+  MarchSide<typename VT::TX, typename VT::TB> sd[KK];
   const bool act = lane < (rlane(rec, 0) >> 16);
   d2_t zero;
   zero.x = zero.y = 0.0;
-#pragma unroll
-  for (int q = 0; q < KK + 2; ++q) ln[q] = zero;
+  xpair_t xzero;
+  xzero.x = xzero.y = 0;
+  bpair_t bzero;
+  bzero.x = bzero.y = 0;
+#pragma unroll
+  for (int q = 0; q < KK + 2; ++q) ln[q] = xzero;
 #pragma unroll
   for (int q = 0; q < KK; ++q) {
     rb[q] = rlane(rec, 18 + 4 * (Q0 + q)) & amask;
-    sd[q].ym = sd[q].yp = sd[q].ax = sd[q].ax2 = zero;
+    sd[q].ym = sd[q].yp = xzero;
+    sd[q].ax = zero;
+    sd[q].ax2 = bzero;
   }
   if (act) {
-    ln[0] = load_pair<false>(x + (rlane(rec, Q0 == 0 ? 16 : 18 + 4 * (Q0 - 1)) & amask) + l2);
-#pragma unroll
-    for (int q = 0; q < KK; ++q) ln[q + 1] = load_pair<false>(x + rb[q] + l2);
-    ln[KK + 1] = load_pair<false>(x + (rlane(rec, Q0 + KK == KTOT ? 17 : 18 + 4 * (Q0 + KK)) & amask) + l2);
+    ln[0] = load_raw<false>(x + (rlane(rec, Q0 == 0 ? 16 : 18 + 4 * (Q0 - 1)) & amask) + l2);
+#pragma unroll
+    for (int q = 0; q < KK; ++q) ln[q + 1] = load_raw<false>(x + rb[q] + l2);
+    ln[KK + 1] = load_raw<false>(x + (rlane(rec, Q0 + KK == KTOT ? 17 : 18 + 4 * (Q0 + KK)) & amask) + l2);
 #pragma unroll
     for (int q = 0; q < KK; ++q) {
       if (Y && !nolat) {
-        sd[q].ym = load_pair<false>(x + rb[q] + (rlane(rec, 19 + 4 * (Q0 + q)) & amask) + l2 + one);
-        sd[q].yp = load_pair<false>(x + rb[q] + (rlane(rec, 20 + 4 * (Q0 + q)) & amask) + l2 + one);
+        sd[q].ym = load_raw<false>(x + rb[q] + (rlane(rec, 19 + 4 * (Q0 + q)) & amask) + l2 + one);
+        sd[q].yp = load_raw<false>(x + rb[q] + (rlane(rec, 20 + 4 * (Q0 + q)) & amask) + l2 + one);
       }
       if (MI::HAS_A) sd[q].ax = load_pair<false>(pa + rb[q] + l2 + one);
-      if (MI::HAS_B) sd[q].ax2 = load_pair<false>(pb + rb[q] + l2 + one);
+      if (MI::HAS_B && !VT::P32) sd[q].ax2 = load_raw<false>(pb + rb[q] + l2 + one);
     }
   }
   const int e_first = rlane(rec, MARCH_EDGE + 2 + Q0) >> 16;
@@ -497,37 +582,38 @@
   }
   const d2_t* el = reinterpret_cast<const d2_t*>(sv);
   const d2_t* cl = reinterpret_cast<const d2_t*>(sx);
-  double xm_n = lane_up(ln[0].x);
+  double xm_n = lane_up((double)ln[0].x);
 #pragma unroll
   for (int q = 0; q < KK; ++q)
-    xm_n = march_plane<CNT, MODE, EDGE>(c, rlane(rec, 21 + 4 * (Q0 + q)), l2, y + rb[q] + l2 + one, ln[q], xm_n, ln[q + 1], ln[q + 2], sd[q], pc0,
-                                  pc1, pc2, acc0, acc1, acc2, dbg, rlane(rec, MARCH_EDGE + 2 + Q0 + q), e_first, el, cl);
-}
-
-template <int CNT, int MODE, bool EDGE>
-__device__ __forceinline__ void march_dispatch(int rec, int lane, const double* __restrict__ x, double* __restrict__ y,
-                                      const double* __restrict__ pa, const double* __restrict__ pb, double pc0, double pc1,
+    xm_n = march_plane<CNT, MODE, EDGE, VT>(c, rlane(rec, 21 + 4 * (Q0 + q)), l2, y + rb[q] + l2 + one, ln[q], xm_n, ln[q + 1], ln[q + 2], sd[q], pc0,
+                                  pc1, pc2, acc0, acc1, acc2, dbg, rlane(rec, MARCH_EDGE + 2 + Q0 + q), e_first, el, cl,
+                                  VT::P32 ? p32 + rb[q] + l2 + one : nullptr, psig);
+}
+
+template <int CNT, int MODE, bool EDGE, class VT>
+__device__ __forceinline__ void march_dispatch(int rec, int lane, const typename VT::TX* __restrict__ x, typename VT::TY* __restrict__ y,
+                                      const double* __restrict__ pa, const typename VT::TB* __restrict__ pb, double pc0, double pc1,
                                       double pc2, double& acc0, double& acc1, double& acc2, int dbg,
-                                      const double* __restrict__ e_val, double* sv, double* sx) {
+                                      const double* __restrict__ e_val, double* sv, double* sx, float* __restrict__ p32, double psig) {
   constexpr bool SPLIT = MODE == 3 && MARCH_K == 2 * MARCH_KS && PG_MARCH_SPLIT;
   if ((rlane(rec, 0) & 255) == MARCH_K) {
     if (SPLIT) {
-      march_unit<CNT, MODE, EDGE, MARCH_KS, 0, MARCH_K>(rec, lane, x, y, pa, pb, pc0, pc1, pc2, acc0, acc1, acc2, dbg, e_val, sv, sx);
-      march_unit<CNT, MODE, EDGE, MARCH_KS, MARCH_KS, MARCH_K>(rec, lane, x, y, pa, pb, pc0, pc1, pc2, acc0, acc1, acc2, dbg, e_val, sv, sx);
+      march_unit<CNT, MODE, EDGE, VT, MARCH_KS, 0, MARCH_K>(rec, lane, x, y, pa, pb, pc0, pc1, pc2, acc0, acc1, acc2, dbg, e_val, sv, sx, p32, psig);
+      march_unit<CNT, MODE, EDGE, VT, MARCH_KS, MARCH_KS, MARCH_K>(rec, lane, x, y, pa, pb, pc0, pc1, pc2, acc0, acc1, acc2, dbg, e_val, sv, sx, p32, psig);
     } else {
-      march_unit<CNT, MODE, EDGE, MARCH_K>(rec, lane, x, y, pa, pb, pc0, pc1, pc2, acc0, acc1, acc2, dbg, e_val, sv, sx);
+      march_unit<CNT, MODE, EDGE, VT, MARCH_K>(rec, lane, x, y, pa, pb, pc0, pc1, pc2, acc0, acc1, acc2, dbg, e_val, sv, sx, p32, psig);
     }
   } else {
-    march_unit<CNT, MODE, EDGE, MARCH_KS>(rec, lane, x, y, pa, pb, pc0, pc1, pc2, acc0, acc1, acc2, dbg, e_val, sv, sx);
-  }
-}
-
-template <int MODE, bool NT, bool DIAG>
+    march_unit<CNT, MODE, EDGE, VT, MARCH_KS>(rec, lane, x, y, pa, pb, pc0, pc1, pc2, acc0, acc1, acc2, dbg, e_val, sv, sx, p32, psig);
+  }
+}
+
+template <int MODE, bool NT, bool DIAG, class VT = VecF64>
 __global__ __launch_bounds__(BLOCK, 4) void k_spmv_s(i64 nslices, const int* __restrict__ srec,
                                                   const double* __restrict__ pval, const int* __restrict__ g_rowid,
                                                   const int* __restrict__ g_rowptr, const int* __restrict__ g_col,
-                                                  const double* __restrict__ g_val, const double* __restrict__ x,
-                                                  double* __restrict__ y, const double* __restrict__ aux,
+                                                  const double* __restrict__ g_val, const typename VT::TX* __restrict__ x,
+                                                  typename VT::TY* __restrict__ y, const double* __restrict__ aux,
                                                   double* __restrict__ partials, const double* __restrict__ sc, int xcd,
                                                   FinArgs fin, int pstride, int accum, const int* __restrict__ mrec,
                                                   i64 nunits, const int* __restrict__ tiles, int tpx,
@@ -538,9 +624,12 @@
   if (sc && sc[S_DONE] != 0.0) return;
   using MI = ModeInfo<MODE>;
   constexpr bool DOTS = MI::DOT0;
-  const double* __restrict__ dx = fin.dotx ? fin.dotx : x;
+  static_assert(MODE == 8 || std::is_same<VT, VecF64>::value, "element types per stream exist for mode 8 only");
+  const double* __restrict__ dx = fin.dotx ? fin.dotx : reinterpret_cast<const double*>(x);
   const double* __restrict__ pa = MODE == 1 ? aux : ((MODE == 2 || MODE == 3) ? dx : nullptr);
-  const double* __restrict__ pb = MODE == 3 ? aux : (MODE == 8 ? fin.base : nullptr);
+  const typename VT::TB* __restrict__ pb = reinterpret_cast<const typename VT::TB*>(MODE == 3 ? aux : (MODE == 8 ? fin.base : nullptr));
+  float* __restrict__ p32 = VT::P32 ? fin.p32 : nullptr;
+  const double psig = fin.psig;
   const int lane = threadIdx.x & 63;
   const int wave = __builtin_amdgcn_readfirstlane(threadIdx.x >> 6);
   double* __restrict__ sv = s_val[wave];
@@ -583,11 +672,11 @@
       if (!(dbg & 16)) {
         const bool edge = rlane(urec, MARCH_EDGE + 1) > 0;
         if (((rlane(urec, 0) >> 8) & 255) == 7) {
-          if (edge) march_dispatch<7, MODE, true>(urec, lane, x, y, pa, pb, fin.pc0, fin.pc1, fin.pc2, acc0, acc1, acc2, dbg, e_val, sv, sx);
-          else march_dispatch<7, MODE, false>(urec, lane, x, y, pa, pb, fin.pc0, fin.pc1, fin.pc2, acc0, acc1, acc2, dbg, e_val, sv, sx);
+          if (edge) march_dispatch<7, MODE, true, VT>(urec, lane, x, y, pa, pb, fin.pc0, fin.pc1, fin.pc2, acc0, acc1, acc2, dbg, e_val, sv, sx, p32, psig);
+          else march_dispatch<7, MODE, false, VT>(urec, lane, x, y, pa, pb, fin.pc0, fin.pc1, fin.pc2, acc0, acc1, acc2, dbg, e_val, sv, sx, p32, psig);
         } else {
-          if (edge) march_dispatch<5, MODE, true>(urec, lane, x, y, pa, pb, fin.pc0, fin.pc1, fin.pc2, acc0, acc1, acc2, dbg, e_val, sv, sx);
-          else march_dispatch<5, MODE, false>(urec, lane, x, y, pa, pb, fin.pc0, fin.pc1, fin.pc2, acc0, acc1, acc2, dbg, e_val, sv, sx);
+          if (edge) march_dispatch<5, MODE, true, VT>(urec, lane, x, y, pa, pb, fin.pc0, fin.pc1, fin.pc2, acc0, acc1, acc2, dbg, e_val, sv, sx, p32, psig);
+          else march_dispatch<5, MODE, false, VT>(urec, lane, x, y, pa, pb, fin.pc0, fin.pc1, fin.pc2, acc0, acc1, acc2, dbg, e_val, sv, sx, p32, psig);
         }
       }
       urec = urec_n;
@@ -610,9 +699,9 @@
     const bool skip = ((dbg & 1) && type == SL_G) || ((dbg & 2) && type != SL_G);
     if (skip) {
     } else if (type == SL_U) {
-      slice_dispatch<false, MODE, NT>(cnt, d, nrows, rec, pval, x, y, pa, pb, lane, acc0, acc1, acc2, dbg, fin.pc0, fin.pc1, fin.pc2);
+      slice_dispatch<false, MODE, NT, VT>(cnt, d, nrows, rec, pval, x, y, pa, pb, lane, acc0, acc1, acc2, dbg, fin.pc0, fin.pc1, fin.pc2, p32, psig);
     } else if (type == SL_P) {
-      slice_dispatch<true, MODE, NT>(cnt, d, nrows, rec, pval, x, y, pa, pb, lane, acc0, acc1, acc2, dbg, fin.pc0, fin.pc1, fin.pc2);
+      slice_dispatch<true, MODE, NT, VT>(cnt, d, nrows, rec, pval, x, y, pa, pb, lane, acc0, acc1, acc2, dbg, fin.pc0, fin.pc1, fin.pc2, p32, psig);
     } else {
       Desc dd;
       dd.r0 = d.r0; dd.base = d.base; dd.r1 = d.r0 + nrows; dd.end = d.aux;
@@ -624,12 +713,13 @@
       const int av = q.ra - basev, ac = q.ra - basec, len = q.rb - q.ra;
 #pragma unroll
       for (int j = 0; j < XV_IT; ++j) sv2[lane + 64 * j] = q.v[j];
-      const double opa = MI::HAS_A ? pa[rid] : 0.0, opb = MI::HAS_B ? pb[rid] : 0.0;
-      const double xown = MI::OWN ? x[rid] : 0.0;
+      const double opa = MI::HAS_A ? pa[rid] : 0.0, opb_ = (MI::HAS_B && !VT::P32) ? (double)pb[rid] : 0.0;
+      const double xown = MI::OWN ? (double)x[rid] : 0.0;
+      const double opb = VT::P32 ? xown : opb_;
       double xg[XC_IT][4];
 #pragma unroll
       for (int j = 0; j < XC_IT; ++j) {
-        xg[j][0] = x[q.c[j].x]; xg[j][1] = x[q.c[j].y]; xg[j][2] = x[q.c[j].z]; xg[j][3] = x[q.c[j].w];
+        xg[j][0] = (double)x[q.c[j].x]; xg[j][1] = (double)x[q.c[j].y]; xg[j][2] = (double)x[q.c[j].z]; xg[j][3] = (double)x[q.c[j].w];
       }
 #pragma unroll
       for (int j = 0; j < XC_IT; ++j) {
@@ -662,7 +752,8 @@
       __builtin_amdgcn_wave_barrier();
       if (live) {
         sum = mode_out<MODE>(sum, xown, opb, fin.pc0, fin.pc1, fin.pc2);
-        y[rid] = sum;
+        store_one_t(y + rid, sum);
+        if (VT::P32) store_one_t(p32 + rid, psig * opb);
         if (MI::DOT0) acc0 += opa * sum;
         if (MI::DOT1) acc1 += sum * sum;
         if (MI::DOT2) acc2 += opb * sum;
@@ -812,6 +903,34 @@
   return false;
 }
 
+template <class VT>
+void launch_typed(const CsrMatrix& A, const void* x, void* y, const double* sc, int grid, hipStream_t st, const FinArgs& fin) {
+  const bool tiled = A.tiles_per_xcd > 0 && A.nslices == A.tile_ns && (xcd_map() & 1) && grid >= 8;
+  hipLaunchKernelGGL(HIP_KERNEL_NAME(k_spmv_s<8, true, false, VT>), dim3(grid), dim3(BLOCK), 0, st, A.nslices, (const int*)A.srec.p,
+                     (const double*)A.pval.p, (const int*)A.g_rowid.p, (const int*)A.g_rowptr.p, (const int*)A.g_col.p,
+                     (const double*)A.g_val.p, static_cast<const typename VT::TX*>(x), static_cast<typename VT::TY*>(y),
+                     (const double*)nullptr, (double*)nullptr, sc, xcd_map(), fin, grid, 0, (const int*)A.mrec.p, A.nunits,
+                     tiled ? (const int*)A.tiles.p : (const int*)nullptr, tiled ? A.tiles_per_xcd : 0, (const double*)A.e_val.p);
+}
+
+}
+
+bool spmv_supports_typed_chain() { return (variant() & 64) != 0 && (variant() & 4) != 0 && xcd_map() < 256; }
+
+void launch_spmv_typed(int kind, const CsrMatrix& A, const void* x, void* y, const double* sc, int grid, hipStream_t st,
+                       const FinArgs& fin) {
+  if (A.n == 0) return;
+  PG_REQUIRE(spmv_supports_typed_chain() && A.srec.p, "typed Horner launches need the slice kernel with the stream hint (PG_SPMV_VARIANT 70)");
+  PG_REQUIRE(!fin.ticket && fin.base, "typed Horner launch: a base operand and no scalar phase");
+  if (kind == TYPED_FIRST) {
+    PG_REQUIRE(fin.p32 && x == (const void*)fin.base, "typed Horner launch (first): x = base and a p32 output");
+    launch_typed<VecTypes<double, double, float, true>>(A, x, y, sc, grid, st, fin);
+  } else if (kind == TYPED_MIDDLE) {
+    launch_typed<VecTypes<float, float, float, false>>(A, x, y, sc, grid, st, fin);
+  } else {
+    PG_REQUIRE(kind == TYPED_HANDOVER, "unknown typed Horner launch");
+    launch_typed<VecTypes<float, double, double, false>>(A, x, y, sc, grid, st, fin);
+  }
 }
 
 
```

New measurement: 1353, median of 6. +3.3%, better.
